# Bardli/RMem_ocu

Hardware: AMD Instinct MI355X
Metric: frames/sec (whole node) 480p VOS, N=8 memory bank (higher is better)
Workload: dtype bf16; 1 GPU; davis17_480p_r50_N8; clip_frames=80, job_clips=64, clip_feeder=static, objects=3, memory_bank=1+7, gap=5, clips_in_flight_per_gpu=24, clips_per_group=8, step_unit=batch, parallelism=clip-parallel x1, weights=synthetic (no checkpoint offline), hipgraphs=True, frames_from=HBM, encoder_lookahead=2

## Files before the change

include/rmem.h:

```cpp
#ifndef RMEM_H_
#define RMEM_H_

#include <stddef.h>

#ifdef __cplusplus
extern "C" {
#endif

#define RMEM_ABI_VERSION 15

int rmem_abi_version(void);
const char* rmem_last_error_string(void);

typedef struct rmem_conv_desc {
  int H, W, Cin;
  int Ho, Wo, Cout;
  int KH, KW, stride, pad;
  int ldo;
  int ldr;
  int ld2;
  int relu;
  int out_f32;
  int res_f32;
  int ldx;
  int batch;
  int act_begin;
  int res_up_h, res_up_w, res_up_align;
} rmem_conv_desc;

size_t rmem_conv_workspace_bytes(const rmem_conv_desc* desc);
int rmem_conv2d_nhwc(const rmem_conv_desc* desc, const void* x, const void* w, const float* bias,
                     const void* residual, void* y, void* y2, void* workspace, void* stream);

enum rmem_gemm_family {
  RMEM_GEMM_GENERAL64 = 0,
  RMEM_GEMM_SCALAR64 = 1,
  RMEM_GEMM_ROWRUN64 = 2,
  RMEM_GEMM_ONE128 = 3,
  RMEM_GEMM_PC128 = 4,
  RMEM_GEMM_ROWRUN128 = 5,
  RMEM_GEMM_DUAL64 = 6,
  RMEM_GEMM_DUAL128 = 7,
  RMEM_GEMM_GROUPED = 8
};
enum rmem_gemm_entry { RMEM_GEMM_ENTRY_CONV2D = 0, RMEM_GEMM_ENTRY_DUAL = 1, RMEM_GEMM_ENTRY_GROUPED = 2 };
typedef struct rmem_gemm_plan {
  int family;
  int tile;
  int ring;
  int is1x1;
  int fast;
  int splits;
  int steps_per_split;
  int xcd_ny;
  int grid_x, grid_y, grid_z, threads;
} rmem_gemm_plan;
int rmem_conv_plan(const rmem_conv_desc* desc, int has_workspace, int entry, int extra, rmem_gemm_plan* plan);

int rmem_linear_grouped(const rmem_conv_desc* desc, int n, const void* const* x, const void* const* w,
                        const float* const* bias, const void* const* residual, void* const* y, void* stream);

int rmem_conv1x1_dual_nhwc(const rmem_conv_desc* desc, const void* x, const void* x2, int H2, int W2, int Cin2, int stride2,
                           const void* w_cat, const float* bias, void* y, void* stream);

typedef struct rmem_bneck_chain_desc { int batch, Ho, Wo, K1, Cout, N2, H2, W2, Cin2, stride2; } rmem_bneck_chain_desc;
int rmem_bneck_chain(const rmem_bneck_chain_desc* desc, const void* b, const void* x2, const void* w3, const float* bias3, const void* res,
                     void* y, const void* w1, const float* bias1, void* a2, void* stream);

typedef struct rmem_attn_chunk {
  int slot;
  int key_begin;
  int key_count;
  int pe_slot;
  int t;
  int reserved[3];
} rmem_attn_chunk;

size_t rmem_attn_workspace_bytes(int Lq, int heads, int nchunks);

int rmem_mem_read_attn(const void* q, int ldq,
                       const void* k_bank, const void* v_bank,
                       long long slot_stride, int ldkv,
                       const rmem_attn_chunk* chunks, int nchunks,
                       int lk_single,
                       const float* pe_cur,
                       const float* pe_mem,
                       int Lq, int heads,
                       void* out, int ldo,
                       float* attn_mass, int T,
                       void* workspace, void* stream);

int rmem_mem_read_attn_clips(const void* q, int ldq, const void* k_bank, const void* v_bank, long long slot_stride, int ldkv,
                             const rmem_attn_chunk* chunks, int nchunks, int lk_single, const float* pe_cur, const float* pe_mem,
                             int Lq, int heads, void* out, int ldo, float* attn_mass, int T, int nclips,
                             long long q_clip_stride, long long kv_clip_stride, long long out_clip_stride,
                             void* workspace, void* stream);

int rmem_lstt_attn_pair_clips(const void* q, int ldq, const void* k_bank, const void* v_bank, long long slot_stride, int ldkv,
                              const rmem_attn_chunk* chunks, int nchunks, int lk_total, const float* pe_cur, const float* pe_mem,
                              int Lq, int heads, void* out_long, int ldo, float* attn_mass, int T, int nclips,
                              long long q_clip_stride, long long out_clip_stride,
                              const void* k_short, const void* v_short, int lk_short, long long kv_short_clip_stride,
                              void* out_short, long long out_short_clip_stride, void* workspace, void* stream);

int rmem_profile_start(int max_launches);
int rmem_profile_stop(double* total_ms, double* total_flops, int* launches);

int rmem_layernorm256(const void* a, int a_is_f32, int lda, const void* b, int b_is_f32, int ldb,
                      const float* gamma, const float* beta, float eps, int M,
                      void* y_bf16, int ldy, const float* pos, void* ypos_bf16, int ldyp,
                      float* y_f32, int ldyf, void* stream);

int rmem_layernorm256_pair(const void* a0, const void* b0, void* y0, const void* a1, const void* b1, void* y1,
                           const float* gamma, const float* beta, float eps, int M, void* stream);

int rmem_lstt_chain_waves(void);
typedef struct rmem_chain_a_desc {
  int L, clips; float eps; int reserved;
  const void* att; float* x;
  const void* w_proj; const float* b_proj; const float* ln2_g; const float* ln2_b; void* curr_v;
  const void* w_q; const float* b_q; void* curr_q;
  const void* short_k; const void* short_v; const float* ln4_g; const float* ln4_b; void* k4; void* v4;
} rmem_chain_a_desc;
int rmem_lstt_chain_a(const rmem_chain_a_desc* d, void* stream);

typedef struct rmem_chain_b_desc {
  int L, clips; float eps; int gn_splits;
  const void* att_long; const void* att_short; float* x;
  const void* w_long; const float* b_long; const void* w_short; const float* b_short; void* tgt3;
  const float* ln3_g; const float* ln3_b; const void* w1; const float* b1; void* h1; float* gn_partial;
} rmem_chain_b_desc;
int rmem_lstt_chain_b(const rmem_chain_b_desc* d, void* stream);

typedef struct rmem_chain_c_desc {
  int L, clips; float eps; int ld_dec;
  float* x;
  const void* h3; const void* w2; const float* b2; const float* dec_g; const float* dec_b; void* dec_out;
  const float* ln1_g; const float* ln1_b; const void* w_qkv; const float* b_qkv; const float* pos_qk; void* qkv;
} rmem_chain_c_desc;
int rmem_lstt_chain_c(const rmem_chain_c_desc* d, void* stream);

int rmem_layernorm(const void* a, int a_is_f32, int lda, const float* gamma, const float* beta, float eps, int M, int C,
                   void* y_bf16, int ldy, float* y_f32, int ldyf, void* stream);

int rmem_patch_merge_ln(const float* x, int H, int W, int C, const float* gamma, const float* beta, float eps,
                        void* y_bf16, void* stream);
int rmem_patch_merge_ln_images(const float* x, int images, int H, int W, int C, const float* gamma, const float* beta, float eps,
                               void* y_bf16, void* stream);

int rmem_window_attn(const void* qkv, const float* qkv_bias, const float* bias_mask_table, void* out, int H, int W,
                     int C, int heads, int shift, void* stream);
int rmem_window_attn_images(const void* qkv, const float* qkv_bias, const float* bias_mask_table, void* out, int images, int H, int W,
                            int C, int heads, int shift, void* stream);

int rmem_add16(const void* a, const void* b, void* y, long long n, void* stream);
int rmem_add16_grouped(int n, const void* const* a, const void* const* b, void* const* y, long long count, void* stream);

size_t rmem_groupnorm_workspace_bytes(int groups);
int rmem_groupnorm_nhwc(const void* x, int M, int C, int groups, const float* gamma, const float* beta,
                        float eps, int act, void* y, float* workspace, void* stream);

int rmem_groupnorm_f32_nhwc(const float* x, int M, int C, int groups, const float* gamma, const float* beta,
                            float eps, int act, void* y, float* workspace, void* stream);

int rmem_groupnorm_nhwc_images(const void* x, int images, int M, int C, int groups, const float* gamma, const float* beta,
                               float eps, int act, void* y, float* workspace, void* stream);
int rmem_groupnorm_head_nhwc_images(const void* x, int images, int M, int C, int groups, const float* gamma, const float* beta,
                                    float eps, int act, const void* w, const float* bias, int N, float* y, int ldy,
                                    float* workspace, void* stream);
int rmem_gn_act_dwconv5x5_nhwc_images(const void* x, int images, int H, int W, int C, int groups, const float* gamma,
                                      const float* beta, float eps, int act, const float* w_t, void* y, float* workspace, void* stream);
int rmem_bilinear_nhwc_images(const void* x, void* y, int images, int Hi, int Wi, int Ho, int Wo, int C, int align_corners, void* stream);
int rmem_gn_act_dwconv5x5_prestats_nhwc_images(const void* x, int images, int H, int W, int C, int groups, const float* gamma,
                                               const float* beta, float eps, int act, const float* w_t, void* y, const float* stats,
                                               void* stream);

int rmem_dwconv5x5_nhwc(const void* x, const float* w_t, void* y, int H, int W, int C, void* stream);

size_t rmem_gated_attn_workspace_bytes(int Lq, int DV, int frames, int keys_per_frame, int nchunks);
int rmem_gated_attn(const void* q, int ldq,
                    const void* k_bank, long long k_slot_stride, int ldk,
                    const void* v_bank, long long v_slot_stride, int ldv,
                    const rmem_attn_chunk* chunks, int nchunks, int frames, int keys_per_frame,
                    const float* pe_cur, const float* pe_mem,
                    int Lq, int DV, const void* u_a, int ldua, const void* u_b, int ldub, int usplit,
                    void* out, int ldo, float* attn_mass,
                    const float* dw_w_t, int H, int W,
                    void* workspace, void* stream);
int rmem_local_gated_attn(const void* q, int ldq, const void* k, int ldk, const void* v, int ldv, const float* rel, int ldrel,
                          int H, int W, int DV, const void* u_a, int ldua, const void* u_b, int ldub, int usplit,
                          void* out, int ldo, const float* dw_w_t, void* workspace, void* stream);

int rmem_gated_attn_clips(const void* q, int ldq, const void* k_bank, long long k_slot_stride, int ldk, const void* v_bank,
                          long long v_slot_stride, int ldv, const rmem_attn_chunk* chunks, int nchunks, int frames, int keys_per_frame,
                          const float* pe_cur, const float* pe_mem, int Lq, int DV, const void* u_a, int ldua, const void* u_b, int ldub,
                          int usplit, void* out, int ldo, float* attn_mass, const float* dw_w_t, int H, int W, int nclips,
                          void* workspace, void* stream);
int rmem_local_gated_attn_clips(const void* q, int ldq, const void* k, int ldk, const void* v, int ldv, const float* rel, int ldrel,
                                int H, int W, int DV, const void* u_a, int ldua, const void* u_b, int ldub, int usplit, void* out, int ldo,
                                const float* dw_w_t, int nclips, void* workspace, void* stream);
int rmem_gated_profile_start(void);
int rmem_gated_profile_stop(double* total_ms, double* total_flops, int* launches);
int rmem_scatter_blocks(const void* src, void* dst, const int* slots_dev, int nclips, long long block_bytes, long long slot_bytes,
                        void* stream);
int rmem_copy2d_async(void* dst, long long dst_pitch, const void* src, long long src_pitch, long long row_bytes, int rows, void* stream);

int rmem_gn_act_dwconv5x5_nhwc(const void* x, int H, int W, int C, int groups, const float* gamma, const float* beta, float eps,
                               int act, const float* w_t, void* y, float* workspace, void* stream);

int rmem_image_to_nhwc8(const float* img_chw, void* out, int H, int W, void* stream);
int rmem_image_to_nhwc8_images(const float* img_chw, void* out, int images, int H, int W, void* stream);
int rmem_image_ptrs_to_nhwc8(const float* const* img_ptrs, void* out, int images, int H, int W, void* stream);
int rmem_stem_padded_size(int H, int W, int* Hp, int* Wp);
int rmem_image_ptrs_to_nhwc4p(const float* const* img_ptrs, void* out_padded, int images, int H, int W, void* stream);
int rmem_stem7x7s2(const void* x_padded, int images, int H, int W, const void* w, const float* bias, void* y, void* stream);
// ... 194 lines not shown
int rmem_mask_iou_counts(const unsigned char* pred, const unsigned char* gt, long long n, int num_ids, int void_label,
                         unsigned long long* counts, void* stream);

size_t rmem_clip_score_workspace_bytes(int frames, int H, int W, int num_ids);
int rmem_boundary_radius(int H, int W, double bound_th);
int rmem_clip_score_counts(const unsigned char* pred, const unsigned char* gt, int frames, int H, int W, int num_ids,
                           int void_label, int radius, void* workspace, unsigned long long* counts, void* stream);

size_t rmem_pair_boundary_workspace_bytes(int frames, int H, int W, int num_a, int num_b);
int rmem_pair_boundary_counts(const unsigned char* a, const unsigned char* b, int frames, int H, int W, int num_a, int num_b,
                              int void_label, int radius, void* workspace, size_t workspace_bytes, int* bnd_a, int* bnd_b,
                              int* match, void* stream);

size_t rmem_png_zlib_bound(int H, int W);
size_t rmem_png_workspace_bytes(int frames, int H, int W);
int rmem_png_encode_labels(const unsigned char* labels, int frames, int H, int W, const unsigned char* lut ,
                           void* workspace, unsigned char* out, long long* offsets, void* stream);

typedef struct RmemPngDesc {
  long long offset;
  long long bytes;
  int bit_depth;
  int colour_type;
} RmemPngDesc;
#define RMEM_PNG_ST_INPUT 1
#define RMEM_PNG_ST_SIZE 2
#define RMEM_PNG_ST_RANGE 4
#define RMEM_PNG_ST_CODE 8
#define RMEM_PNG_ST_HEADER 16
#define RMEM_PNG_ST_ADLER 32
#define RMEM_PNG_ST_FILTER 64
#define RMEM_PNG_ST_DESC 128
size_t rmem_png_decode_workspace_bytes(int frames, int H, int W);
int rmem_png_decode_labels(const unsigned char* bits, const RmemPngDesc* descs , int frames, int H, int W,
                           const unsigned char* lut , void* workspace,
                           unsigned char* out , int* status , void* stream);

#define RMEM_RLE_ST_CAPACITY 1
size_t rmem_rle_workspace_bytes(int frames, int H, int W, int num_ids);
int rmem_rle_encode_labels(const unsigned char* labels, int frames, int H, int W, int num_ids, void* workspace, unsigned char* out,
                           long long capacity, long long* offsets ,
                           int* status , void* stream);

typedef struct RmemRleDesc {
  int frame;
  int value;
  long long offset;
  int length;
} RmemRleDesc;
#define RMEM_RLE_ST_CHAR 1
#define RMEM_RLE_ST_TRUNCATED 2
#define RMEM_RLE_ST_LONG 4
#define RMEM_RLE_ST_NEGATIVE 8
#define RMEM_RLE_ST_SUM 16
#define RMEM_RLE_ST_DESC 32
size_t rmem_rle_decode_workspace_bytes(long long nstrings, long long total_bytes, int frames, int W);
int rmem_rle_decode_labels(const unsigned char* bits, long long total_bytes, const RmemRleDesc* descs , int nstrings, int frames,
                           int H, int W, void* workspace, unsigned char* labels ,
                           int* status , void* stream);

#define RMEM_JPEG_ENC_HEADER_MAX 629
#define RMEM_JPEG_ENC_TABLE_BYTES 4096
int rmem_jpeg_encode_header(int H, int W, int quality, int restart_rows, unsigned char* header, int capacity, int* header_bytes,
                            void* tables );
size_t rmem_jpeg_encode_bound(int H, int W);
size_t rmem_jpeg_encode_workspace_bytes(int frames, int H, int W);
int rmem_jpeg_encode_rgb8(const unsigned char* rgb, const unsigned char* labels ,
                          const unsigned char* palette , int alpha256, int frames,
                          int H, int W, const void* tables ,
                          void* workspace, unsigned char* out, long long* offsets, void* stream);
int rmem_overlay_rgb8(const unsigned char* rgb, const unsigned char* labels, const unsigned char* palette ,
                      int alpha256, int frames, int H, int W, unsigned char* out_rgb, void* stream);

int rmem_graph_begin(void* stream);
int rmem_graph_end(void* stream, void** graph_exec_out);
int rmem_graph_launch(void* graph_exec, void* stream);
int rmem_graph_destroy(void* graph_exec);


int rmem_conv2d_nhwc_f16(const rmem_conv_desc* desc, const void* x, const void* w, const float* bias, const void* residual, void* y, void* y2, void* workspace, void* stream);
int rmem_mem_read_attn_f16(const void* q, int ldq, const void* k_bank, const void* v_bank, long long slot_stride, int ldkv, const rmem_attn_chunk* chunks, int nchunks, int lk_single, const float* pe_cur, const float* pe_mem, int Lq, int heads, void* out, int ldo, float* attn_mass, int T, void* workspace, void* stream);
int rmem_mem_read_attn_clips_f16(const void* q, int ldq, const void* k_bank, const void* v_bank, long long slot_stride, int ldkv, const rmem_attn_chunk* chunks, int nchunks, int lk_single, const float* pe_cur, const float* pe_mem, int Lq, int heads, void* out, int ldo, float* attn_mass, int T, int nclips, long long q_clip_stride, long long kv_clip_stride, long long out_clip_stride, void* workspace, void* stream);
int rmem_lstt_attn_pair_clips_f16(const void* q, int ldq, const void* k_bank, const void* v_bank, long long slot_stride, int ldkv, const rmem_attn_chunk* chunks, int nchunks, int lk_total, const float* pe_cur, const float* pe_mem, int Lq, int heads, void* out_long, int ldo, float* attn_mass, int T, int nclips, long long q_clip_stride, long long out_clip_stride, const void* k_short, const void* v_short, int lk_short, long long kv_short_clip_stride, void* out_short, long long out_short_clip_stride, void* workspace, void* stream);
int rmem_layernorm256_f16(const void* a, int a_is_f32, int lda, const void* b, int b_is_f32, int ldb, const float* gamma, const float* beta, float eps, int M, void* y_bf16, int ldy, const float* pos, void* ypos_bf16, int ldyp, float* y_f32, int ldyf, void* stream);
int rmem_layernorm_f16(const void* a, int a_is_f32, int lda, const float* gamma, const float* beta, float eps, int M, int C, void* y_bf16, int ldy, float* y_f32, int ldyf, void* stream);
int rmem_patch_merge_ln_f16(const float* x, int H, int W, int C, const float* gamma, const float* beta, float eps, void* y_bf16, void* stream);
int rmem_window_attn_f16(const void* qkv, const float* qkv_bias, const float* bias_mask_table, void* out, int H, int W, int C, int heads, int shift, void* stream);
int rmem_window_attn_images_f16(const void* qkv, const float* qkv_bias, const float* bias_mask_table, void* out, int images, int H, int W, int C, int heads, int shift, void* stream);
int rmem_patch_merge_ln_images_f16(const float* x, int images, int H, int W, int C, const float* gamma, const float* beta, float eps, void* y_bf16, void* stream);
int rmem_add16_f16(const void* a, const void* b, void* y, long long n, void* stream);
int rmem_add16_grouped_f16(int n, const void* const* a, const void* const* b, void* const* y, long long count, void* stream);
int rmem_lstt_chain_a_f16(const rmem_chain_a_desc* d, void* stream);
int rmem_lstt_chain_b_f16(const rmem_chain_b_desc* d, void* stream);
int rmem_lstt_chain_c_f16(const rmem_chain_c_desc* d, void* stream);
int rmem_layernorm256_pair_f16(const void* a0, const void* b0, void* y0, const void* a1, const void* b1, void* y1, const float* gamma, const float* beta, float eps, int M, void* stream);
int rmem_bneck_chain_f16(const rmem_bneck_chain_desc* desc, const void* b, const void* x2, const void* w3, const float* bias3, const void* res, void* y, const void* w1, const float* bias1, void* a2, void* stream);
int rmem_conv1x1_dual_nhwc_f16(const rmem_conv_desc* desc, const void* x, const void* x2, int H2, int W2, int Cin2, int stride2, const void* w_cat, const float* bias, void* y, void* stream);
int rmem_linear_grouped_f16(const rmem_conv_desc* desc, int n, const void* const* x, const void* const* w, const float* const* bias, const void* const* residual, void* const* y, void* stream);
int rmem_groupnorm_nhwc_f16(const void* x, int M, int C, int groups, const float* gamma, const float* beta, float eps, int act, void* y, float* workspace, void* stream);
int rmem_groupnorm_f32_nhwc_f16(const float* x, int M, int C, int groups, const float* gamma, const float* beta, float eps, int act, void* y, float* workspace, void* stream);
int rmem_groupnorm_nhwc_images_f16(const void* x, int images, int M, int C, int groups, const float* gamma, const float* beta, float eps, int act, void* y, float* workspace, void* stream);
int rmem_groupnorm_head_nhwc_images_f16(const void* x, int images, int M, int C, int groups, const float* gamma, const float* beta, float eps, int act, const void* w, const float* bias, int N, float* y, int ldy, float* workspace, void* stream);
int rmem_gn_act_dwconv5x5_nhwc_images_f16(const void* x, int images, int H, int W, int C, int groups, const float* gamma, const float* beta, float eps, int act, const float* w_t, void* y, float* workspace, void* stream);
int rmem_gn_act_dwconv5x5_prestats_nhwc_images_f16(const void* x, int images, int H, int W, int C, int groups, const float* gamma, const float* beta, float eps, int act, const float* w_t, void* y, const float* stats, void* stream);
int rmem_gn_act_dwconv5x5_nhwc_f16(const void* x, int H, int W, int C, int groups, const float* gamma, const float* beta, float eps, int act, const float* w_t, void* y, float* workspace, void* stream);
int rmem_dwconv5x5_nhwc_f16(const void* x, const float* w_t, void* y, int H, int W, int C, void* stream);
int rmem_image_ptrs_to_nhwc4p_f16(const float* const* img_ptrs, void* out_padded, int images, int H, int W, void* stream);
int rmem_conv3x3_direct_f16(const void* x, int images, int H, int W, int C, const void* w, const float* bias, int relu, void* y, void* stream);
int rmem_conv3x3_c64_direct_f16(const void* x, int images, int H, int W, const void* w, const float* bias, void* y, void* stream);
int rmem_stem7x7s2_pool_f16(const void* x_padded, int images, int H, int W, const void* w, const float* bias, void* y_pooled, void* stream);
int rmem_stem7x7s2_f16(const void* x_padded, int images, int H, int W, const void* w, const float* bias, void* y, void* stream);
int rmem_image_ptrs_to_nhwc8_f16(const float* const* img_ptrs, void* out, int images, int H, int W, void* stream);
int rmem_image_to_nhwc8_f16(const float* img_chw, void* out, int H, int W, void* stream);
int rmem_image_to_nhwc8_images_f16(const float* img_chw, void* out, int images, int H, int W, void* stream);
int rmem_ingest_rgb8_f16(const unsigned char* rgb_hwc, int Hs, int Ws, int Hd, int Wd, float* out_chw, void* out_nhwc8, void* stream);
int rmem_maxpool3x3s2_nhwc_f16(const void* x, void* y, int H, int W, int C, void* stream);
int rmem_maxpool3x3s2_nhwc_images_f16(const void* x, void* y, int images, int H, int W, int C, void* stream);
int rmem_bilinear_nhwc_f16(const void* x, void* y, int Hi, int Wi, int Ho, int Wo, int C, int align_corners, void* stream);
int rmem_bilinear_nhwc_images_f16(const void* x, void* y, int images, int Hi, int Wi, int Ho, int Wo, int C, int align_corners, void* stream);
int rmem_label_id_embed_f16(const void* label, int label_is_f32, int images, int Hs, int Ws, int H, int W, int KH, int KW, int stride, int pad, int num_classes, const void* w, const float* bias, void* label_scratch_u8, void* out, void* stream);
int rmem_label_to_onehot16_f16(const void* label, int label_is_f32, int Hs, int Ws, int Hd, int Wd, int num_classes, void* out, void* stream);
int rmem_label_to_onehot16_images_f16(const void* label, int label_is_f32, int images, int Hs, int Ws, int Hd, int Wd, int num_classes, void* out, void* stream);
int rmem_gated_attn_f16(const void* q, int ldq, const void* k_bank, long long k_slot_stride, int ldk, const void* v_bank, long long v_slot_stride, int ldv, const rmem_attn_chunk* chunks, int nchunks, int frames, int keys_per_frame, const float* pe_cur, const float* pe_mem, int Lq, int DV, const void* u_a, int ldua, const void* u_b, int ldub, int usplit, void* out, int ldo, float* attn_mass, const float* dw_w_t, int H, int W, void* workspace, void* stream);
int rmem_local_gated_attn_f16(const void* q, int ldq, const void* k, int ldk, const void* v, int ldv, const float* rel, int ldrel, int H, int W, int DV, const void* u_a, int ldua, const void* u_b, int ldub, int usplit, void* out, int ldo, const float* dw_w_t, void* workspace, void* stream);
int rmem_gated_attn_clips_f16(const void* q, int ldq, const void* k_bank, long long k_slot_stride, int ldk, const void* v_bank, long long v_slot_stride, int ldv, const rmem_attn_chunk* chunks, int nchunks, int frames, int keys_per_frame, const float* pe_cur, const float* pe_mem, int Lq, int DV, const void* u_a, int ldua, const void* u_b, int ldub, int usplit, void* out, int ldo, float* attn_mass, const float* dw_w_t, int H, int W, int nclips, void* workspace, void* stream);
int rmem_local_gated_attn_clips_f16(const void* q, int ldq, const void* k, int ldk, const void* v, int ldv, const float* rel, int ldrel, int H, int W, int DV, const void* u_a, int ldua, const void* u_b, int ldub, int usplit, void* out, int ldo, const float* dw_w_t, int nclips, void* workspace, void* stream);

#ifdef __cplusplus
}
#endif
#endif
```

rmem_ocu_amd/_lib.py:

```python
from __future__ import annotations

import ctypes as C
import os
import subprocess

_HERE = os.path.dirname(os.path.abspath(__file__))
LIB_PATH = os.environ.get('RMEM_LIB_PATH') or os.path.join(_HERE, 'librmem_hip.so')
ABI_VERSION = 15


class RmemError(RuntimeError):
    pass


class ConvDesc(C.Structure):
    _fields_ = [(n, C.c_int) for n in ('H', 'W', 'Cin', 'Ho', 'Wo', 'Cout', 'KH', 'KW', 'stride', 'pad',
                                       'ldo', 'ldr', 'ld2', 'relu', 'out_f32', 'res_f32', 'ldx', 'batch', 'act_begin',
                                       'res_up_h', 'res_up_w', 'res_up_align')]


class GemmPlan(C.Structure):
    _fields_ = [(n, C.c_int) for n in ('family', 'tile', 'ring', 'is1x1', 'fast', 'splits', 'steps_per_split', 'xcd_ny',
                                       'grid_x', 'grid_y', 'grid_z', 'threads')]


GEMM_FAMILIES = ('general64', 'scalar64', 'rowrun64', 'one128', 'pc128', 'rowrun128', 'dual64', 'dual128', 'grouped')
GEMM_ENTRIES = ('conv2d', 'conv1x1_dual', 'linear_grouped')


class BneckChainDesc(C.Structure):
    _fields_ = [(n, C.c_int) for n in ('batch', 'Ho', 'Wo', 'K1', 'Cout', 'N2', 'H2', 'W2', 'Cin2', 'stride2')]


class AttnChunk(C.Structure):
    _fields_ = [('slot', C.c_int), ('key_begin', C.c_int), ('key_count', C.c_int), ('pe_slot', C.c_int),
                ('t', C.c_int), ('reserved', C.c_int * 3)]


_vp, _i, _ll, _f = C.c_void_p, C.c_int, C.c_longlong, C.c_float


class JpegInfo(C.Structure):
    _fields_ = [('width', C.c_int), ('height', C.c_int), ('components', C.c_int), ('h_samp', C.c_int * 3), ('v_samp', C.c_int * 3),
                ('quant_id', C.c_int * 3), ('restart_interval', C.c_int), ('quant_mask', C.c_int), ('quant', (C.c_ushort * 64) * 4),
                ('scan_begin', C.c_longlong), ('scan_end', C.c_longlong), ('packed_bound', C.c_longlong)]


class JpegHuff(C.Structure):
    _fields_ = [('lut', C.c_ushort * 512), ('maxcode', C.c_int * 18), ('valoff', C.c_int * 18), ('vals', C.c_ubyte * 256)]


class JpegDesc(C.Structure):
    _fields_ = ([('offset', C.c_longlong), ('bytes', C.c_longlong)]
                + [(n, C.c_int) for n in ('width', 'height', 'ncomp', 'hmax', 'vmax', 'mcus_x', 'mcus_y', 'bpm', 'restart_mcus', 'nunits',
                                          'nsub', 'total_blocks', 'data_off', 'data_bits')]
                + [(n, C.c_int * 3) for n in ('comp_h', 'comp_v', 'comp_bw', 'comp_bh', 'comp_block0', 'comp_dw', 'comp_dh')]
                + [('mcu_comp', C.c_int * 10), ('mcu_sub', C.c_int * 10), ('quant', (C.c_ushort * 64) * 3), ('dc', JpegHuff * 3),
                   ('ac', JpegHuff * 3)])


class JpegPlan(C.Structure):
    _fields_ = ([(n, C.c_int) for n in ('batch', 'max_width', 'max_height', 'max_sub', 'max_blocks', 'max_units', 'sync_rounds', 'flags')]
                + [(n, C.c_longlong) for n in ('slot_bytes', 'off_state', 'off_unit', 'off_dc', 'off_coef', 'off_plane', 'off_misc')])


JPEG_FORCE_FALLBACK = 1
JPEG_ENC_HEADER_MAX, JPEG_ENC_TABLE_BYTES = 629, 4096


class PngDesc(C.Structure):
    _fields_ = [('offset', C.c_longlong), ('bytes', C.c_longlong), ('bit_depth', C.c_int), ('colour_type', C.c_int)]


class RleDesc(C.Structure):
    _fields_ = [('frame', C.c_int), ('value', C.c_int), ('offset', C.c_longlong), ('length', C.c_int)]


class PolyShape(C.Structure):
    _fields_ = [(n, C.c_int) for n in ('frame', 'value', 'x0', 'y0', 'x1', 'y1')] + [('plane', C.c_longlong)]


class PolyPass(C.Structure):
    _fields_ = ([(n, C.c_int) for n in ('frame0', 'frames', 'shape0', 'shapes', 'edge0', 'edges')]
                + [(n, C.c_longlong) for n in ('cross0', 'crossings', 'plane0', 'plane_words')])


class LabelRoute(C.Structure):
    _fields_ = [('dst', C.c_void_p), ('overlay', C.c_void_p), ('feed', C.c_void_p), ('twin', C.c_int), ('mode', C.c_int)]


ROUTE_LIVE, ROUTE_IDLE, ROUTE_SKIP = 0, 1, 2


def _desc(name, ints, ptrs):
    return type(name, (C.Structure,), {'_fields_': [(ints[0], _i), (ints[1], _i), ('eps', _f), (ints[2], _i)] + [(n, _vp) for n in ptrs]})


ChainA = _desc('ChainA', ('L', 'clips', 'reserved'),
               ('att', 'x', 'w_proj', 'b_proj', 'ln2_g', 'ln2_b', 'curr_v', 'w_q', 'b_q', 'curr_q', 'short_k', 'short_v', 'ln4_g', 'ln4_b',
                'k4', 'v4'))
ChainB = _desc('ChainB', ('L', 'clips', 'gn_splits'),
               ('att_long', 'att_short', 'x', 'w_long', 'b_long', 'w_short', 'b_short', 'tgt3', 'ln3_g', 'ln3_b', 'w1', 'b1', 'h1',
                'gn_partial'))
ChainC = _desc('ChainC', ('L', 'clips', 'ld_dec'),
               ('x', 'h3', 'w2', 'b2', 'dec_g', 'dec_b', 'dec_out', 'ln1_g', 'ln1_b', 'w_qkv', 'b_qkv', 'pos_qk', 'qkv'))
SIGNATURES = {
    'rmem_abi_version': (_i, []),
    'rmem_last_error_string': (C.c_char_p, []),
    'rmem_conv_workspace_bytes': (C.c_size_t, [C.POINTER(ConvDesc)]),
    'rmem_conv2d_nhwc': (_i, [C.POINTER(ConvDesc), _vp, _vp, _vp, _vp, _vp, _vp, _vp, _vp]),
    'rmem_conv_plan': (_i, [C.POINTER(ConvDesc), _i, _i, _i, C.POINTER(GemmPlan)]),
    'rmem_attn_workspace_bytes': (C.c_size_t, [_i, _i, _i]),
    'rmem_mem_read_attn': (_i, [_vp, _i, _vp, _vp, _ll, _i, _vp, _i, _i, _vp, _vp, _i, _i, _vp, _i, _vp, _i, _vp, _vp]),
    'rmem_profile_start': (_i, [_i]),
    'rmem_profile_stop': (_i, [C.POINTER(C.c_double), C.POINTER(C.c_double), C.POINTER(_i)]),
    'rmem_layernorm256': (_i, [_vp, _i, _i, _vp, _i, _i, _vp, _vp, _f, _i, _vp, _i, _vp, _vp, _i, _vp, _i, _vp]),
    'rmem_layernorm': (_i, [_vp, _i, _i, _vp, _vp, _f, _i, _i, _vp, _i, _vp, _i, _vp]),
    'rmem_patch_merge_ln': (_i, [_vp, _i, _i, _i, _vp, _vp, _f, _vp, _vp]),
    'rmem_window_attn': (_i, [_vp, _vp, _vp, _vp, _i, _i, _i, _i, _i, _vp]),
    'rmem_window_attn_images': (_i, [_vp, _vp, _vp, _vp, _i, _i, _i, _i, _i, _i, _vp]),
    'rmem_patch_merge_ln_images': (_i, [_vp, _i, _i, _i, _i, _vp, _vp, _f, _vp, _vp]),
    'rmem_add16': (_i, [_vp, _vp, _vp, _ll, _vp]),
    'rmem_add16_grouped': (_i, [_i, C.POINTER(_vp), C.POINTER(_vp), C.POINTER(_vp), _ll, _vp]),
    'rmem_layernorm256_pair': (_i, [_vp, _vp, _vp, _vp, _vp, _vp, _vp, _vp, _f, _i, _vp]),
    'rmem_lstt_chain_waves': (_i, []),
    'rmem_lstt_chain_a': (_i, [C.POINTER(ChainA), _vp]),
    'rmem_lstt_chain_b': (_i, [C.POINTER(ChainB), _vp]),
    'rmem_lstt_chain_c': (_i, [C.POINTER(ChainC), _vp]),
    'rmem_conv1x1_dual_nhwc': (_i, [C.POINTER(ConvDesc), _vp, _vp, _i, _i, _i, _i, _vp, _vp, _vp, _vp]),
    'rmem_bneck_chain': (_i, [C.POINTER(BneckChainDesc), _vp, _vp, _vp, _vp, _vp, _vp, _vp, _vp, _vp, _vp]),
    'rmem_linear_grouped': (_i, [C.POINTER(ConvDesc), _i, C.POINTER(_vp), C.POINTER(_vp), C.POINTER(_vp), C.POINTER(_vp), C.POINTER(_vp), _vp]),
    'rmem_groupnorm_workspace_bytes': (C.c_size_t, [_i]),
    'rmem_groupnorm_nhwc': (_i, [_vp, _i, _i, _i, _vp, _vp, _f, _i, _vp, _vp, _vp]),
    'rmem_groupnorm_f32_nhwc': (_i, [_vp, _i, _i, _i, _vp, _vp, _f, _i, _vp, _vp, _vp]),
    'rmem_groupnorm_nhwc_images': (_i, [_vp, _i, _i, _i, _i, _vp, _vp, _f, _i, _vp, _vp, _vp]),
    'rmem_groupnorm_head_nhwc_images': (_i, [_vp, _i, _i, _i, _i, _vp, _vp, _f, _i, _vp, _vp, _i, _vp, _i, _vp, _vp]),
    'rmem_gn_act_dwconv5x5_nhwc_images': (_i, [_vp, _i, _i, _i, _i, _i, _vp, _vp, _f, _i, _vp, _vp, _vp, _vp]),
    'rmem_gn_act_dwconv5x5_prestats_nhwc_images': (_i, [_vp, _i, _i, _i, _i, _i, _vp, _vp, _f, _i, _vp, _vp, _vp, _vp]),
    'rmem_bilinear_nhwc_images': (_i, [_vp, _vp, _i, _i, _i, _i, _i, _i, _i, _vp]),
    'rmem_mem_read_attn_clips': (_i, [_vp, _i, _vp, _vp, _ll, _i, _vp, _i, _i, _vp, _vp, _i, _i, _vp, _i, _vp, _i, _i, _ll, _ll, _ll, _vp, _vp]),
    'rmem_lstt_attn_pair_clips': (_i, [_vp, _i, _vp, _vp, _ll, _i, _vp, _i, _i, _vp, _vp, _i, _i, _vp, _i, _vp, _i, _i, _ll, _ll,
                                       _vp, _vp, _i, _ll, _vp, _ll, _vp, _vp]),
    'rmem_gn_act_dwconv5x5_nhwc': (_i, [_vp, _i, _i, _i, _i, _vp, _vp, _f, _i, _vp, _vp, _vp, _vp]),
    'rmem_dwconv5x5_nhwc': (_i, [_vp, _vp, _vp, _i, _i, _i, _vp]),
    'rmem_image_to_nhwc8': (_i, [_vp, _vp, _i, _i, _vp]),
    'rmem_image_to_nhwc8_images': (_i, [_vp, _vp, _i, _i, _i, _vp]),
    'rmem_image_ptrs_to_nhwc8': (_i, [_vp, _vp, _i, _i, _i, _vp]),
    'rmem_stem_padded_size': (_i, [_i, _i, C.POINTER(_i), C.POINTER(_i)]),
    'rmem_image_ptrs_to_nhwc4p': (_i, [_vp, _vp, _i, _i, _i, _vp]),
    'rmem_stem7x7s2': (_i, [_vp, _i, _i, _i, _vp, _vp, _vp, _vp]),
    'rmem_stem7x7s2_pool': (_i, [_vp, _i, _i, _i, _vp, _vp, _vp, _vp]),
    'rmem_conv3x3_c64_direct': (_i, [_vp, _i, _i, _i, _vp, _vp, _vp, _vp]),
    'rmem_conv3x3_direct': (_i, [_vp, _i, _i, _i, _i, _vp, _vp, _i, _vp, _vp]),
    'rmem_ingest_rgb8': (_i, [_vp, _i, _i, _i, _i, _vp, _vp, _vp]),
    'rmem_maxpool3x3s2_nhwc': (_i, [_vp, _vp, _i, _i, _i, _vp]),
    'rmem_maxpool3x3s2_nhwc_images': (_i, [_vp, _vp, _i, _i, _i, _i, _vp]),
    'rmem_bilinear_nhwc': (_i, [_vp, _vp, _i, _i, _i, _i, _i, _i, _vp]),
    'rmem_logits_post': (_i, [_vp, _i, _i, _i, _i, _i, _i, _i, _i, _vp, _vp, _vp, _vp]),
    'rmem_logits_post_images': (_i, [_vp, _i, _i, _i, _i, _i, _i, _i, _i, _i, _vp, _vp, _vp, _vp]),
    'rmem_label_to_onehot16': (_i, [_vp, _i, _i, _i, _i, _i, _i, _vp, _vp]),
    'rmem_label_id_embed_scratch_size': (_i, [_i, _i, _i, C.POINTER(_i), C.POINTER(_i)]),
    'rmem_label_id_embed': (_i, [_vp, _i, _i, _i, _i, _i, _i, _i, _i, _i, _i, _i, _vp, _vp, _vp, _vp, _vp]),
    'rmem_label_to_onehot16_images': (_i, [_vp, _i, _i, _i, _i, _i, _i, _i, _vp, _vp]),
    'rmem_evict_scores': (_i, [_vp, _i, _i, _i, _i, _i, _i, _i, _vp, _i, _vp, _vp]),
    'rmem_resize_nearest_flip_f32': (_i, [_vp, _i, _i, _i, _vp, _i, _i, _i, _vp]),
    'rmem_tta_merge': (_i, [C.POINTER(_vp), C.POINTER(_i), _i, _i, _i, _i, _vp, _vp, _vp, _vp]),
    'rmem_logits_post_flip_pairs': (_i, [_vp, _i, _i, _i, _i, _i, _i, _i, _i, _vp, _vp]),
    'rmem_logits_post_ms_merge': (_i, [C.POINTER(_vp), C.POINTER(_i), C.POINTER(_i), C.POINTER(_i), _i, _i, _i, _i, _i, _i, _i, _vp, _vp, _vp]),
    'rmem_route_labels': (_i, [_vp, _i, _i, _i, _vp, _vp]),
    'rmem_label_census': (_i, [_vp, _i, _i, _i, _vp, _vp]),
    'rmem_label_remap': (_i, [_vp, _vp, _i, _ll, _vp, _i, _vp]),
    'rmem_label_pair_census': (_i, [_vp, _vp, _i, _i, _i, _i, _i, _vp, _vp]),
    'rmem_label_pair_census_lds_bins': (_i, []),
    'rmem_label_components_tile': (_i, [C.POINTER(_i), C.POINTER(_i)]),
    'rmem_label_components_workspace_bytes': (_ll, [_i, _i, _i]),
    'rmem_label_components': (_i, [_vp, _i, _i, _i, _i, _vp, _vp, _vp]),
    'rmem_label_component_stats': (_i, [_vp, _vp, _i, _i, _i, _i, _vp, _vp, _vp]),
    'rmem_label_clean': (_i, [_vp, _vp, _vp, _vp, _vp, _i, _i, _i, _i, _i, _i, _vp]),
    'rmem_label_edt_workspace_bytes': (_ll, [_i, _i, _i]),
    'rmem_label_edt': (_i, [_vp, _i, _i, _i, _i, _i, _vp, _vp, _ll, _vp]),
    'rmem_label_edt_peaks_workspace_bytes': (_ll, [_i]),
    'rmem_label_edt_peaks': (_i, [_vp, _vp, _i, _i, _i, _vp, _vp, _ll, _vp]),
    'rmem_label_nearest_workspace_bytes': (_ll, [_i, _i, _i]),
    'rmem_label_nearest': (_i, [_vp, _i, _i, _i, C.POINTER(C.c_uint), C.POINTER(C.c_uint), _i, _vp, _vp, _vp, _vp, _ll, _vp]),
    'rmem_label_surface': (_i, [_vp, _i, _i, _i, _vp, _vp]),
    'rmem_label_edt_at': (_i, [_vp, _vp, _i, _i, _i, _i, _i, _vp, _vp, _ll, _vp]),
    'rmem_surface_census_workspace_bytes': (_ll, [_i, _i]),
    'rmem_surface_census': (_i, [_vp, _vp, _vp, _vp, _i, _i, _i, _i, C.POINTER(_i), _i, _i, _vp, _vp, _ll, _vp]),
    'rmem_label_thin_tile': (_i, [C.POINTER(_i), C.POINTER(_i), C.POINTER(_i)]),
    'rmem_label_thin_table': (_i, [_i, _vp]),
    'rmem_label_thin_workspace_bytes': (_ll, [_i, _i, _i]),
    'rmem_label_thin': (_i, [_vp, _i, _i, _i, _i, _i, _vp, _vp, _vp, _ll, _vp]),
    'rmem_label_pixels_workspace_bytes': (_ll, [_i, _i, _i]),
    'rmem_label_pixels_count': (_i, [_vp, _i, _i, _i, _vp, _vp, _ll, _vp]),
    'rmem_label_pixels_write': (_i, [_vp, _vp, _i, _i, _i, _ll, _vp, _vp, _vp, _ll, _vp]),
    'rmem_label_polygons_unit': (_i, []),
    'rmem_label_polygons_workspace_bytes': (C.c_size_t, [_i, _i, _i, _i]),
    'rmem_label_polygons': (_i, [_vp, _i, _i, _i, _i, _i, _i, _vp, C.c_size_t, _vp, _vp, _vp, _vp]),
    'rmem_polygon_simplify_short_max': (_i, []),
    'rmem_polygon_simplify_workspace_bytes': (C.c_size_t, [_ll, _ll]),
    'rmem_polygon_simplify': (_i, [_vp, _vp, _vp, _ll, _ll, _i, _vp, C.c_size_t, _vp, _vp, _vp, _vp]),
    'rmem_polygon_fill_workspace_bytes': (C.c_size_t, [_ll]),
    'rmem_polygon_fill_labels': (_i, [_vp, _vp, _vp, _i, _vp, _i, _vp, _i, _i, _i, C.POINTER(PolyPass), _vp, C.c_size_t, _vp, _vp, _vp]),
    'rmem_mask_iou_counts': (_i, [_vp, _vp, _ll, _i, _i, _vp, _vp]),
    'rmem_clip_score_workspace_bytes': (C.c_size_t, [_i, _i, _i, _i]),
    'rmem_boundary_radius': (_i, [_i, _i, C.c_double]),
    'rmem_clip_score_counts': (_i, [_vp, _vp, _i, _i, _i, _i, _i, _i, _vp, _vp, _vp]),
    'rmem_pair_boundary_workspace_bytes': (C.c_size_t, [_i, _i, _i, _i, _i]),
    'rmem_pair_boundary_counts': (_i, [_vp, _vp, _i, _i, _i, _i, _i, _i, _i, _vp, C.c_size_t, _vp, _vp, _vp, _vp]),
    'rmem_png_zlib_bound': (C.c_size_t, [_i, _i]),
    'rmem_png_workspace_bytes': (C.c_size_t, [_i, _i, _i]),
    'rmem_png_encode_labels': (_i, [_vp, _i, _i, _i, _vp, _vp, _vp, _vp, _vp]),
    'rmem_png_decode_workspace_bytes': (C.c_size_t, [_i, _i, _i]),
    'rmem_png_decode_labels': (_i, [_vp, _vp, _i, _i, _i, _vp, _vp, _vp, _vp, _vp]),
    'rmem_rle_workspace_bytes': (C.c_size_t, [_i, _i, _i, _i]),
    'rmem_rle_encode_labels': (_i, [_vp, _i, _i, _i, _i, _vp, _vp, _ll, _vp, _vp, _vp]),
    'rmem_rle_decode_workspace_bytes': (C.c_size_t, [_ll, _ll, _i, _i]),
    'rmem_rle_decode_labels': (_i, [_vp, _ll, _vp, _i, _i, _i, _i, _vp, _vp, _vp, _vp]),
    'rmem_split_label': (_i, [_vp, _i, _i, _vp, _ll, _vp]),
    'rmem_soft_logit_aggregate': (_i, [C.POINTER(_vp), _i, _i, _i, _i, _i, _vp, _vp]),
    'rmem_copy_async': (_i, [_vp, _vp, C.c_size_t, _vp]),
    'rmem_scatter_blocks': (_i, [_vp, _vp, _vp, _i, _ll, _ll, _vp]),
    'rmem_copy2d_async': (_i, [_vp, _ll, _vp, _ll, _ll, _i, _vp]),
    'rmem_gated_attn_workspace_bytes': (C.c_size_t, [_i, _i, _i, _i, _i]),
    'rmem_gated_attn': (_i, [_vp, _i, _vp, _ll, _i, _vp, _ll, _i, _vp, _i, _i, _i, _vp, _vp, _i, _i, _vp, _i, _vp, _i, _i, _vp, _i,
                             _vp, _vp, _i, _i, _vp, _vp]),
    'rmem_local_gated_attn': (_i, [_vp, _i, _vp, _i, _vp, _i, _vp, _i, _i, _i, _i, _vp, _i, _vp, _i, _i, _vp, _i, _vp, _vp, _vp]),
    'rmem_gated_attn_clips': (_i, [_vp, _i, _vp, _ll, _i, _vp, _ll, _i, _vp, _i, _i, _i, _vp, _vp, _i, _i, _vp, _i, _vp, _i, _i, _vp, _i,
                                   _vp, _vp, _i, _i, _i, _vp, _vp]),
    'rmem_local_gated_attn_clips': (_i, [_vp, _i, _vp, _i, _vp, _i, _vp, _i, _i, _i, _i, _vp, _i, _vp, _i, _i, _vp, _i, _vp, _i, _vp, _vp]),
    'rmem_gated_profile_start': (_i, []),
    'rmem_gated_profile_stop': (_i, [C.POINTER(C.c_double), C.POINTER(C.c_double), C.POINTER(_i)]),
    'rmem_jpeg_parse': (_i, [_vp, C.c_size_t, C.POINTER(JpegInfo)]),
    'rmem_jpeg_pack': (_i, [_vp, C.c_size_t, _vp, C.c_size_t, C.POINTER(C.c_size_t), C.POINTER(JpegDesc)]),
    'rmem_jpeg_workspace_bytes': (C.c_size_t, [C.POINTER(JpegDesc), _i, _i, C.POINTER(JpegPlan)]),
    'rmem_jpeg_entropy_decode': (_i, [_vp, _vp, _i, _i, C.POINTER(JpegPlan), _vp, _vp, _vp, _vp]),
    'rmem_jpeg_coef_to_rgb': (_i, [_vp, _i, _i, C.POINTER(JpegPlan), _vp, _vp, _vp]),
    'rmem_jpeg_decode_batch': (_i, [_vp, _vp, _i, _i, C.POINTER(JpegPlan), _vp, _vp, _vp, _vp, _vp]),
    'rmem_jpeg_encode_header': (_i, [_i, _i, _i, _i, _vp, _i, C.POINTER(_i), _vp]),
    'rmem_jpeg_encode_bound': (C.c_size_t, [_i, _i]),
    'rmem_jpeg_encode_workspace_bytes': (C.c_size_t, [_i, _i, _i]),
    'rmem_jpeg_encode_rgb8': (_i, [_vp, _vp, _vp, _i, _i, _i, _i, _vp, _vp, _vp, _vp, _vp]),
    'rmem_overlay_rgb8': (_i, [_vp, _vp, _vp, _i, _i, _i, _i, _vp, _vp]),
    'rmem_graph_begin': (_i, [_vp]),
    'rmem_graph_end': (_i, [_vp, C.POINTER(_vp)]),
    'rmem_graph_launch': (_i, [_vp, _vp]),
    'rmem_graph_destroy': (_i, [_vp]),
}

F16_TWINS = ('rmem_conv2d_nhwc', 'rmem_mem_read_attn', 'rmem_mem_read_attn_clips', 'rmem_lstt_attn_pair_clips', 'rmem_layernorm256', 'rmem_layernorm', 'rmem_patch_merge_ln',
             'rmem_window_attn', 'rmem_window_attn_images', 'rmem_patch_merge_ln_images', 'rmem_add16', 'rmem_add16_grouped', 'rmem_layernorm256_pair', 'rmem_lstt_chain_a', 'rmem_lstt_chain_b', 'rmem_lstt_chain_c', 'rmem_conv1x1_dual_nhwc', 'rmem_bneck_chain', 'rmem_label_id_embed', 'rmem_image_ptrs_to_nhwc4p', 'rmem_stem7x7s2', 'rmem_stem7x7s2_pool', 'rmem_conv3x3_c64_direct', 'rmem_conv3x3_direct', 'rmem_linear_grouped',
             'rmem_groupnorm_nhwc', 'rmem_groupnorm_f32_nhwc', 'rmem_groupnorm_nhwc_images', 'rmem_groupnorm_head_nhwc_images',
             'rmem_gn_act_dwconv5x5_nhwc_images', 'rmem_gn_act_dwconv5x5_prestats_nhwc_images', 'rmem_gn_act_dwconv5x5_nhwc', 'rmem_dwconv5x5_nhwc', 'rmem_image_to_nhwc8',
             'rmem_image_to_nhwc8_images', 'rmem_image_ptrs_to_nhwc8', 'rmem_ingest_rgb8', 'rmem_maxpool3x3s2_nhwc', 'rmem_maxpool3x3s2_nhwc_images', 'rmem_bilinear_nhwc',
             'rmem_bilinear_nhwc_images', 'rmem_label_to_onehot16', 'rmem_label_to_onehot16_images', 'rmem_gated_attn', 'rmem_local_gated_attn', 'rmem_gated_attn_clips', 'rmem_local_gated_attn_clips')
SIGNATURES.update({n + '_f16': SIGNATURES[n] for n in F16_TWINS})

_lib = None


def build(force: bool = False) -> str:
    src = os.path.join(_HERE, 'csrc')
    if force:
        subprocess.run(['make', '-C', src, 'clean'], check=True, capture_output=True)
    r = subprocess.run(['make', '-C', src, '-j8'], capture_output=True, text=True)
    if r.returncode != 0:
        raise RmemError('building librmem_hip.so failed:\n' + r.stdout + r.stderr)
    return LIB_PATH


def lib():
    global _lib
    if _lib is None:
        if not os.path.exists(LIB_PATH):
            raise RmemError(f'{LIB_PATH} is missing: run `python -c "import __graft_entry__ as g; g.build()"` '
                            '(there is no CPU fallback for the HIP path)')
        import torch
        L = C.CDLL(LIB_PATH)
        for name, (res, args) in SIGNATURES.items():
            fn = getattr(L, name)
            fn.restype = res
            fn.argtypes = args
        if L.rmem_abi_version() != ABI_VERSION:
            raise RmemError('librmem_hip.so ABI version mismatch; rebuild it')
        _lib = L
    return _lib


def check(rc: int, what: str = ''):
    if rc != 0:
        raise RmemError(f'{what} failed ({rc}): {lib().rmem_last_error_string().decode()}')
```

rmem_ocu_amd/csrc/attention.hip:

```cpp
#include "common.h"
#include "../../include/rmem.h"
#include <type_traits>

namespace {

constexpr int D = 32;
constexpr int KT = 64;
constexpr int NB = 4;
constexpr float NEG_BIG = -1.0e30f;
constexpr float RESCALE_THR = 8.0f;
[[maybe_unused]] constexpr float L_LIMIT = 1.8446744e19f;

typedef __attribute__((ext_vector_type(4))) short s16x4;
typedef __attribute__((address_space(3))) s16x4 lds_s16x4;

struct AttnParams {
  const e16* q; int ldq;
  const e16* k; const e16* v; long slot_stride; int ldkv;
  const rmem_attn_chunk* chunks; int nchunks; int lk; int per_chunk;
  const float* pe_cur; const float* pe_mem;
  int Lq, heads, C, nq;
  int ngroups, rpg;
  float* opart; float* mlg;
  float* ml;
// ... 482 lines not shown
      num += f32x4{(float)o4[0], (float)o4[1], (float)o4[2], (float)o4[3]} * w;
    }
    if (live) {
      const f32x4 o = num * (1.f / den);
      *reinterpret_cast<e16x4*>(p.out + (long)q * p.ldo + head * D + 4 * G) = e16x4{(e16)o[0], (e16)o[1], (e16)o[2], (e16)o[3]};
    }
  }
}

__global__ __launch_bounds__(256) void k_attn_mass(CombineParams pin) {
  CombineParams p = pin;
  p.ml += blockIdx.z * p.ml_cs; p.chunks += blockIdx.z * p.nchunks; p.mass += blockIdx.z * p.mass_cs;
  __shared__ float macc[4][64][33];
  __shared__ int ct[32];
  const int tid = threadIdx.x, ql = tid & 63, hq = tid >> 6;
  const int q = blockIdx.x * 64 + ql;
  const int qc = q < p.Lq ? q : p.Lq - 1;
  if (tid < p.nchunks) ct[tid] = p.chunks[tid].t;
  for (int t = 0; t < 33; ++t) macc[hq][ql][t] = 0.f;
  __syncthreads();
  for (int h = hq; h < p.heads; h += 4) {
    float m = NEG_BIG, den = 0.f;
    for (int c = 0; c < p.nchunks; ++c) {
      const f32x2 mlv = *reinterpret_cast<const f32x2*>(p.ml + (((long)c * p.heads + h) * p.Lq + qc) * 2);
      if (mlv[1] > 0.f) m = fmaxf(m, mlv[0]);
    }
    for (int c = 0; c < p.nchunks; ++c) {
      const f32x2 mlv = *reinterpret_cast<const f32x2*>(p.ml + (((long)c * p.heads + h) * p.Lq + qc) * 2);
      if (mlv[1] > 0.f) den += __builtin_amdgcn_exp2f(mlv[0] - m) * mlv[1];
    }
    const float inv = 1.f / (den * (float)p.heads);
    for (int c = 0; c < p.nchunks; ++c) {
      const f32x2 mlv = *reinterpret_cast<const f32x2*>(p.ml + (((long)c * p.heads + h) * p.Lq + qc) * 2);
      if (mlv[1] > 0.f) macc[hq][ql][ct[c]] += __builtin_amdgcn_exp2f(mlv[0] - m) * mlv[1] * inv;
    }
  }
  __syncthreads();
  for (int i = tid; i < 64 * p.T; i += 256) {
    const int qq = i / p.T, t = i - qq * p.T;
    const int qo = blockIdx.x * 64 + qq;
    if (qo < p.Lq) p.mass[(long)qo * p.T + t] = macc[0][qq][t] + macc[1][qq][t] + macc[2][qq][t] + macc[3][qq][t];
  }
}

}

#ifndef RMEM_F16
extern "C" size_t rmem_attn_workspace_bytes(int Lq, int heads, int nchunks) {
  return (size_t)nchunks * heads * Lq * (D + 4) * sizeof(float);
}
#endif

#if defined(RMEM_ATTN_TIMELINE) && !defined(RMEM_F16)
extern "C" int rmem_attn_timeline_read(double* out, int nwg) {
  static unsigned host[8192 * 8];
  if (nwg > 8192) nwg = 8192;
  if (hipDeviceSynchronize() != hipSuccess) return 1;
  if (hipMemcpyFromSymbol(host, HIP_SYMBOL(g_attn_timeline), sizeof(unsigned) * 8 * nwg) != hipSuccess) return 2;
  double s[5] = {0, 0, 0, 0, 0};
  for (int i = 0; i < nwg; ++i) for (int j = 0; j < 5; ++j) s[j] += host[i * 8 + j];
  for (int j = 0; j < 4; ++j) out[j] = s[4] > 0 ? s[j] / s[4] : 0;
  out[4] = s[4] / nwg;
  return 0;
}
#endif

static unsigned attn_lds_pad() {
  const char* e = getenv("RMEM_ATTN_LDS_PAD");
  const int x = e ? atoi(e) : 0;
  return x > 0 ? (unsigned)x : 0u;
}

static int attn_target_wgs() {
  const char* e = getenv("RMEM_ATTN_WGS");
  const int x = e ? atoi(e) : 0;
  return x > 0 ? x : 1792;
}

static int attn_launch(const void* q, int ldq, const void* k_bank, const void* v_bank, long long slot_stride,
                       int ldkv, const rmem_attn_chunk* chunks, int nchunks, int lk_single,
                       const float* pe_cur, const float* pe_mem, int Lq, int heads, void* out, int ldo,
                       float* attn_mass, int T, int nclips, long long q_clip_stride, long long kv_clip_stride,
                       long long out_clip_stride, void* workspace, void* stream,
                       const void* k2, const void* v2, int lk2, long long kv2_clip_stride, void* out2, long long out2_clip_stride) {
  RMEM_REQUIRE(nclips >= 1 && nclips <= 64, "rmem_mem_read_attn: 1..64 clips");
  RMEM_REQUIRE(q_clip_stride % 8 == 0 && kv_clip_stride % 8 == 0 && out_clip_stride % 8 == 0, "rmem_mem_read_attn: clip strides must be multiples of 8 elements");
  const long long prof_keys = chunks ? (long long)lk_single : 0;
  RMEM_REQUIRE(q && k_bank && v_bank && out && workspace, "rmem_mem_read_attn: null argument");
  RMEM_REQUIRE(heads >= 1 && heads <= 8, "rmem_mem_read_attn: heads must be in 1..8 (head dim is fixed at 32)");
  RMEM_REQUIRE(Lq > 0 && nchunks >= 1 && nchunks <= 32, "rmem_mem_read_attn: need Lq > 0 and 1 <= nchunks <= 32");
  RMEM_REQUIRE(ldq % 8 == 0 && ldkv % 8 == 0 && slot_stride % 8 == 0, "rmem_mem_read_attn: strides must be multiples of 8 elements");
  RMEM_REQUIRE(ldq >= heads * D && ldkv >= heads * D && ldo >= heads * D, "rmem_mem_read_attn: leading dimension < heads*32");
  RMEM_REQUIRE(chunks || lk_single > 0, "rmem_mem_read_attn: lk_single must be > 0 when no chunk table is given");
  RMEM_REQUIRE(lk_single >= 0, "rmem_mem_read_attn: lk_single must be >= 0");
  RMEM_REQUIRE(!attn_mass || (chunks && T >= 1 && T <= 32), "rmem_mem_read_attn: the mass output needs a chunk table and 1 <= T <= 32");
  RMEM_REQUIRE(!pe_mem || chunks, "rmem_mem_read_attn: pe_mem needs a chunk table");
  hipStream_t s = (hipStream_t)stream;
  AttnParams p;
  p.q = (const e16*)q; p.ldq = ldq; p.k = (const e16*)k_bank; p.v = (const e16*)v_bank;
  p.slot_stride = slot_stride; p.ldkv = ldkv; p.chunks = chunks; p.nchunks = nchunks;
  p.lk = lk_single; p.per_chunk = chunks ? 0 : (lk_single + nchunks - 1) / nchunks;
  RMEM_REQUIRE(chunks || (long)p.per_chunk * (nchunks - 1) < lk_single, "rmem_mem_read_attn: too many chunks for lk_single");
  p.pe_cur = pe_cur; p.pe_mem = pe_mem; p.Lq = Lq; p.heads = heads; p.C = heads * D;
  p.nclips = nclips; p.q_cs = q_clip_stride; p.kv_cs = kv_clip_stride; p.out_cs = out_clip_stride;
  p.qscale = 1.4426950408889634f / sqrtf((float)D);
  p.nq = (Lq + 127) / 128;
  {
    const int base = p.nq * heads * nclips;
    int groups = (attn_target_wgs() + base - 1) / base;
    groups = groups < 1 ? 1 : (groups > nchunks ? nchunks : groups);
    p.rpg = (nchunks + groups - 1) / groups;
    p.ngroups = (nchunks + p.rpg - 1) / p.rpg;
  }
  p.opart_cs = (long)p.ngroups * heads * Lq * D; p.mlg_cs = (long)p.ngroups * heads * Lq * 2; p.ml_cs = (long)nchunks * heads * Lq * 2;
  p.opart = (float*)workspace; p.mlg = p.opart + (size_t)nclips * p.opart_cs;
  p.ml = attn_mass ? p.mlg + (size_t)nclips * p.mlg_cs : nullptr;
  p.out = (e16*)out; p.ldo = ldo;
  p.n2 = 0; p.k2 = p.v2 = nullptr; p.lk2 = 0; p.kv2_cs = 0; p.out2 = nullptr; p.out2_cs = 0;
  if (k2) {
    RMEM_REQUIRE(chunks && v2 && out2 && lk2 > 0, "rmem_lstt_attn_pair: the second attention rides on a memory read (chunk table) and needs k2, v2, out2, lk2 > 0");
    RMEM_REQUIRE(kv2_clip_stride % 8 == 0 && out2_clip_stride % 8 == 0 && ((uintptr_t)k2 % 16) == 0 && ((uintptr_t)v2 % 16) == 0,
                 "rmem_lstt_attn_pair: second attention operands must be 16-byte aligned, strides multiples of 8 elements");
    RMEM_REQUIRE(p.nq * heads * nclips >= 8, "rmem_lstt_attn_pair: launch too small for the per-XCD split");
    p.n2 = nclips; p.k2 = (const e16*)k2; p.v2 = (const e16*)v2; p.lk2 = lk2; p.kv2_cs = kv2_clip_stride;
    p.out2 = (e16*)out2; p.out2_cs = out2_clip_stride;
  }
  dim3 grid(p.nq * heads * (p.ngroups * nclips + p.n2));
  if (chunks) {
    const int slot_i = prof_keys > 0 ? rmem_prof_begin(RMEM_PROF_MEM_READ, s, 4.0 * (double)Lq * (double)prof_keys * (double)(heads * D) * nclips)
                                     : -1;
    if (slot_i >= 0) hipLaunchKernelGGL((k_attn_partial<true, true>), grid, dim3(256), attn_lds_pad(), s, p);
    else hipLaunchKernelGGL((k_attn_partial<true, false>), grid, dim3(256), attn_lds_pad(), s, p);
    if (slot_i >= 0) rmem_prof_end(RMEM_PROF_MEM_READ, slot_i, s);
  } else {
    hipLaunchKernelGGL((k_attn_partial<false, false>), grid, dim3(256), 0, s, p);
  }
  CombineParams cp;
  cp.opart = p.opart; cp.mlg = p.mlg; cp.ngroups = p.ngroups; cp.ml = p.ml; cp.chunks = chunks; cp.nchunks = nchunks;
  cp.Lq = Lq; cp.heads = heads; cp.out = (e16*)out; cp.ldo = ldo; cp.mass = attn_mass; cp.T = T;
  cp.out_cs = out_clip_stride; cp.opart_cs = p.opart_cs; cp.mlg_cs = p.mlg_cs; cp.ml_cs = p.ml_cs; cp.mass_cs = (long)Lq * T;
  if (p.ngroups > 1) hipLaunchKernelGGL(k_attn_combine, dim3((Lq + 63) / 64, 16, nclips), dim3(256), 0, s, cp);
  if (attn_mass) hipLaunchKernelGGL(k_attn_mass, dim3((Lq + 63) / 64, 1, nclips), dim3(256), 0, s, cp);
  return rmem_check_launch("rmem_mem_read_attn");
}

extern "C" int RMEM_API(rmem_mem_read_attn_clips)(const void* q, int ldq, const void* k_bank, const void* v_bank, long long slot_stride,
                                        int ldkv, const rmem_attn_chunk* chunks, int nchunks, int lk_single,
                                        const float* pe_cur, const float* pe_mem, int Lq, int heads, void* out, int ldo,
                                        float* attn_mass, int T, int nclips, long long q_clip_stride, long long kv_clip_stride,
                                        long long out_clip_stride, void* workspace, void* stream) {
  return attn_launch(q, ldq, k_bank, v_bank, slot_stride, ldkv, chunks, nchunks, lk_single, pe_cur, pe_mem, Lq, heads, out, ldo, attn_mass, T,
                     nclips, q_clip_stride, kv_clip_stride, out_clip_stride, workspace, stream, nullptr, nullptr, 0, 0, nullptr, 0);
}

extern "C" int RMEM_API(rmem_lstt_attn_pair_clips)(const void* q, int ldq, const void* k_bank, const void* v_bank, long long slot_stride,
                                         int ldkv, const rmem_attn_chunk* chunks, int nchunks, int lk_total,
                                         const float* pe_cur, const float* pe_mem, int Lq, int heads, void* out_long, int ldo,
                                         float* attn_mass, int T, int nclips, long long q_clip_stride, long long out_clip_stride,
                                         const void* k_short, const void* v_short, int lk_short, long long kv_short_clip_stride,
                                         void* out_short, long long out_short_clip_stride, void* workspace, void* stream) {
  RMEM_REQUIRE(chunks && k_short && v_short && out_short, "rmem_lstt_attn_pair: null argument");
  return attn_launch(q, ldq, k_bank, v_bank, slot_stride, ldkv, chunks, nchunks, lk_total, pe_cur, pe_mem, Lq, heads, out_long, ldo, attn_mass, T,
                     nclips, q_clip_stride, 0, out_clip_stride, workspace, stream, k_short, v_short, lk_short, kv_short_clip_stride, out_short,
                     out_short_clip_stride);
}

extern "C" int RMEM_API(rmem_mem_read_attn)(const void* q, int ldq, const void* k_bank, const void* v_bank, long long slot_stride,
                                  int ldkv, const rmem_attn_chunk* chunks, int nchunks, int lk_single,
                                  const float* pe_cur, const float* pe_mem, int Lq, int heads, void* out, int ldo,
                                  float* attn_mass, int T, void* workspace, void* stream) {
  return RMEM_API(rmem_mem_read_attn_clips)(q, ldq, k_bank, v_bank, slot_stride, ldkv, chunks, nchunks, lk_single, pe_cur, pe_mem, Lq, heads, out,
                                  ldo, attn_mass, T, 1, 0, 0, 0, workspace, stream);
}
```

rmem_ocu_amd/csrc/rowchain.hip:

```cpp
#include "common.h"
#include "lds_dma.h"
#include "../../include/rmem.h"

namespace {

#ifndef RMEM_CHAIN_WAVES
#define RMEM_CHAIN_WAVES 8
#endif
constexpr int NW = RMEM_CHAIN_WAVES;
constexpr int NT = 64 * NW;
constexpr int JT = 16 / NW;
constexpr int WC = 256 / NW;
constexpr int RW = 32 / NW;
constexpr int BM = 32;
constexpr int XS = 260;
constexpr int PANEL = BM * 64;
constexpr int PF = 16 / JT;

__device__ __forceinline__ f32x4 ld4(const float* p) { return *reinterpret_cast<const f32x4*>(p); }
__device__ __forceinline__ e16x4 cvt4(f32x4 v) { return e16x4{(e16)v[0], (e16)v[1], (e16)v[2], (e16)v[3]}; }
__device__ __forceinline__ f32x4 up4(e16x4 v) { return f32x4{(float)v[0], (float)v[1], (float)v[2], (float)v[3]}; }

typedef __attribute__((ext_vector_type(2))) unsigned u32x2;
typedef __attribute__((ext_vector_type(4))) unsigned u32x4;
#if defined(__HIP_DEVICE_COMPILE__)
__device__ __forceinline__ void st8(rsrc_t r, int off, e16x4 v) { __builtin_amdgcn_raw_buffer_store_b64(__builtin_bit_cast(u32x2, v), r, off, 0, 0); }
__device__ __forceinline__ void st16(rsrc_t r, int off, f32x4 v) { __builtin_amdgcn_raw_buffer_store_b128(__builtin_bit_cast(u32x4, v), r, off, 0, 0); }
#else
__device__ inline void st8(rsrc_t, int, e16x4) {}
__device__ inline void st16(rsrc_t, int, f32x4) {}
#endif

template <int NP>
__device__ __forceinline__ void stage_tile(e16* A16, int p0, const e16* src, long ld, int nrows) {
  constexpr int PT = NT / 256;
  static_assert(NP % PT == 0, "panels must divide among the thread halves");
  const int t = threadIdx.x & 255, half = threadIdx.x >> 8;
  const int row = t >> 3, ch = t & 7;
  const e16* sr = src + min(row, nrows - 1) * ld + ch * 8;
  e16x8 v[NP / PT];
#pragma unroll
  for (int p = 0; p < NP / PT; ++p) v[p] = *reinterpret_cast<const e16x8*>(sr + (p * PT + half) * 64);
#pragma unroll
  for (int p = 0; p < NP / PT; ++p) *reinterpret_cast<e16x8*>(&A16[(p0 + p * PT + half) * PANEL + swz(row, ch)]) = v[p];
}

__device__ __forceinline__ void put_a(e16* A16, int p0, int row, int lane, e16x4 v) {
  *reinterpret_cast<e16x4*>(&A16[(p0 + (lane >> 4)) * PANEL + swz(row, (lane & 15) >> 1) + (lane & 1) * 4]) = v;
}

struct BRing { e16x8 b[PF][JT]; };

__device__ __forceinline__ const e16* wstream(const e16* w, int nb, int wave, int KC) { return w + (long)(nb * NW + wave) * KC * (JT * 512); }

__device__ __forceinline__ void b_preload(BRing& r, const e16* wp, int lane) {
#pragma unroll
  for (int u = 0; u < PF; ++u)
#pragma unroll
    for (int j = 0; j < JT; ++j) r.b[u][j] = *reinterpret_cast<const e16x8*>(wp + ((u * JT + j) * 64 + lane) * 8);
  __builtin_amdgcn_sched_barrier(0);
}

template <int NP>
__device__ __forceinline__ void gemm32(const e16* A16, int p0, const e16* wp, BRing& r, f32x4 (&acc)[2][JT], int lane) {
  constexpr int KC = NP * 2;
  const int fr = lane & 15, fc = lane >> 4;
#pragma unroll
  for (int kc = 0; kc < KC; ++kc) {
    const e16* Ap = A16 + (p0 + (kc >> 1)) * PANEL;
    const e16x8 a0 = *reinterpret_cast<const e16x8*>(&Ap[swz(fr, 4 * (kc & 1) + fc)]);
    const e16x8 a1 = *reinterpret_cast<const e16x8*>(&Ap[swz(16 + fr, 4 * (kc & 1) + fc)]);
#pragma unroll
    for (int j = 0; j < JT; ++j) {
      acc[0][j] = RMEM_MFMA_16x16x32(a0, r.b[kc % PF][j], acc[0][j], 0, 0, 0);
      acc[1][j] = RMEM_MFMA_16x16x32(a1, r.b[kc % PF][j], acc[1][j], 0, 0, 0);
    }
    if (kc + PF < KC) {
#pragma unroll
      for (int j = 0; j < JT; ++j) r.b[kc % PF][j] = *reinterpret_cast<const e16x8*>(wp + (((kc + PF) * JT + j) * 64 + lane) * 8);
      __builtin_amdgcn_sched_barrier(0);
    }
  }
}

__device__ __forceinline__ void zero_acc(f32x4 (&acc)[2][JT]) {
#pragma unroll
  for (int i = 0; i < 2; ++i)
#pragma unroll
    for (int j = 0; j < JT; ++j) acc[i][j] = f32x4{0.f, 0.f, 0.f, 0.f};
}

__device__ __forceinline__ void dump_acc(float* X, const f32x4 (&acc)[2][JT], int wave, int lane) {
  const int fr = lane & 15, fc = lane >> 4;
#pragma unroll
  for (int i = 0; i < 2; ++i)
#pragma unroll
    for (int j = 0; j < JT; ++j)
#pragma unroll
      for (int q = 0; q < 4; ++q) X[(i * 16 + fc * 4 + q) * XS + wave * WC + j * 16 + fr] = acc[i][j][q];
}

struct Blk { int nrows; long g0; };
__device__ __forceinline__ Blk my_rows(int L) {
  Blk b;
  const int r0 = blockIdx.x * BM;
  b.nrows = min(BM, L - r0);
  b.g0 = (long)blockIdx.y * L + r0;
  return b;
}

template <typename T>
struct Rows8 { T r[RW]; };

__device__ __forceinline__ Rows8<f32x4> load_rows_f32(const float* base, int ld, const Blk& blk, int wave, int c0) {
  Rows8<f32x4> o;
#pragma unroll
  for (int rr = 0; rr < RW; ++rr) {
    const int row = min(wave * RW + rr, blk.nrows - 1);
    o.r[rr] = ld4(base + (blk.g0 + row) * ld + c0);
  }
  return o;
}
__device__ __forceinline__ Rows8<e16x4> load_rows_e16(const e16* base, int ld, const Blk& blk, int wave, int c0) {
  Rows8<e16x4> o;
#pragma unroll
  for (int rr = 0; rr < RW; ++rr) {
    const int row = min(wave * RW + rr, blk.nrows - 1);
    o.r[rr] = *reinterpret_cast<const e16x4*>(base + (blk.g0 + row) * ld + c0);
  }
  return o;
}
__device__ __forceinline__ int row_off(const Blk& blk, int wave, int rr, int ld, int c0, int esz) {
  const int row = wave * RW + rr;
  return row < blk.nrows ? (int)(((blk.g0 + row) * ld + c0) * esz) : OOB;
}

__global__ __launch_bounds__(NT) void k_chain_a(rmem_chain_a_desc d) {
  __shared__ __attribute__((aligned(16))) char smem[4 * PANEL * 2 + BM * XS * 4];
  e16* A16 = reinterpret_cast<e16*>(smem);
  float* X = reinterpret_cast<float*>(smem + 4 * PANEL * 2);
  const int lane = threadIdx.x & 63, wave = __builtin_amdgcn_readfirstlane(threadIdx.x >> 6);
  const Blk blk = my_rows(d.L);
  const int c0 = lane * 4;
  const long rows = (long)d.clips * d.L;
  const rsrc_t rx = make_rsrc(d.x, rows * 1024), rcv = make_rsrc(d.curr_v, rows * 512), rcq = make_rsrc(d.curr_q, rows * 512),
               rk4 = make_rsrc(d.k4, rows * 512), rv4 = make_rsrc(d.v4, rows * 512);
  const f32x4 bp = ld4(d.b_proj + c0), g2 = ld4(d.ln2_g + c0), b2 = ld4(d.ln2_b + c0);
  const f32x4 bq = ld4(d.b_q + c0), g4 = ld4(d.ln4_g + c0), b4 = ld4(d.ln4_b + c0);
  const Rows8<f32x4> xo = load_rows_f32(d.x, 256, blk, wave, c0);
  const Rows8<e16x4> sk = load_rows_e16((const e16*)d.short_k, 256, blk, wave, c0);
  const Rows8<e16x4> sv = load_rows_e16((const e16*)d.short_v, 256, blk, wave, c0);
  BRing ring;
  f32x4 acc[2][JT];
  const e16* wp = wstream((const e16*)d.w_proj, 0, wave, 8);
  stage_tile<4>(A16, 0, (const e16*)d.att + blk.g0 * 256, 256, blk.nrows);
  b_preload(ring, wp, lane);
  __syncthreads();
  zero_acc(acc);
  gemm32<4>(A16, 0, wp, ring, acc, lane);
  dump_acc(X, acc, wave, lane);
  const e16* wq = wstream((const e16*)d.w_q, 0, wave, 8);
  b_preload(ring, wq, lane);
  __syncthreads();
  e16x4 cv[RW];
  {
    f32x4 v[RW];
#pragma unroll
    for (int rr = 0; rr < RW; ++rr) {
      v[rr] = ld4(&X[(wave * RW + rr) * XS + c0]);
      v[rr] += bp;
      v[rr] += xo.r[rr];
      st16(rx, row_off(blk, wave, rr, 256, c0, 4), v[rr]);
    }
    rmem_ln256_rows<RW>(v, g2, b2, d.eps);
#pragma unroll
    for (int rr = 0; rr < RW; ++rr) {
      cv[rr] = cvt4(v[rr]);
      st8(rcv, row_off(blk, wave, rr, 256, c0, 2), cv[rr]);
      put_a(A16, 0, wave * RW + rr, lane, cv[rr]);
    }
  }
  __syncthreads();
  zero_acc(acc);
  gemm32<4>(A16, 0, wq, ring, acc, lane);
  dump_acc(X, acc, wave, lane);
  __syncthreads();
  {
    f32x4 kk[RW], vv[RW];
#pragma unroll
    for (int rr = 0; rr < RW; ++rr) {
      f32x4 q = ld4(&X[(wave * RW + rr) * XS + c0]);
      q += bq;
      const e16x4 cq = cvt4(q);
      st8(rcq, row_off(blk, wave, rr, 256, c0, 2), cq);
      kk[rr] = up4(sk.r[rr]);
      kk[rr] += up4(cq);
      vv[rr] = up4(sv.r[rr]);
      vv[rr] += up4(cv[rr]);
    }
    rmem_ln256_rows<RW>(kk, g4, b4, d.eps);
    rmem_ln256_rows<RW>(vv, g4, b4, d.eps);
#pragma unroll
    for (int rr = 0; rr < RW; ++rr) {
      const int off = row_off(blk, wave, rr, 256, c0, 2);
      st8(rk4, off, cvt4(kk[rr]));
      st8(rv4, off, cvt4(vv[rr]));
    }
  }
}

template <bool STATS>
__global__ __launch_bounds__(NT) void k_chain_b(rmem_chain_b_desc d) {
  __shared__ __attribute__((aligned(16))) char smem[8 * PANEL * 2 + 2 * BM * XS * 4 + 4 * NW * 8 * 2 * 4];
  e16* A16 = reinterpret_cast<e16*>(smem);
  float* Xa = reinterpret_cast<float*>(smem + 8 * PANEL * 2);
  float* Xb = Xa + BM * XS;
  float* gsum = Xb + BM * XS;
  const int lane = threadIdx.x & 63, wave = __builtin_amdgcn_readfirstlane(threadIdx.x >> 6);
  const Blk blk = my_rows(d.L);
  const int c0 = lane * 4;
  const long rows = (long)d.clips * d.L;
  const rsrc_t rx = make_rsrc(d.x, rows * 1024), rt3 = make_rsrc(d.tgt3, rows * 512), rh1 = make_rsrc(d.h1, rows * 2048);
  const f32x4 bl = ld4(d.b_long + c0), bs = ld4(d.b_short + c0), g3 = ld4(d.ln3_g + c0), b3 = ld4(d.ln3_b + c0);
  f32x4 b1[4];
#pragma unroll
  for (int nb = 0; nb < 4; ++nb) b1[nb] = ld4(d.b1 + nb * 256 + c0);
  const Rows8<f32x4> xo = load_rows_f32(d.x, 256, blk, wave, c0);
  BRing ring;
  f32x4 acc[2][JT];
  const e16* wl = wstream((const e16*)d.w_long, 0, wave, 8);
  stage_tile<4>(A16, 0, (const e16*)d.att_long + blk.g0 * 256, 256, blk.nrows);
  stage_tile<4>(A16, 4, (const e16*)d.att_short + blk.g0 * 256, 256, blk.nrows);
  b_preload(ring, wl, lane);
  __syncthreads();
  zero_acc(acc);
  gemm32<4>(A16, 0, wl, ring, acc, lane);
  dump_acc(Xa, acc, wave, lane);
  const e16* ws = wstream((const e16*)d.w_short, 0, wave, 8);
  b_preload(ring, ws, lane);
  zero_acc(acc);
  gemm32<4>(A16, 4, ws, ring, acc, lane);
  dump_acc(Xb, acc, wave, lane);
  const e16* w1 = wstream((const e16*)d.w1, 0, wave, 8);
  b_preload(ring, w1, lane);
  __syncthreads();
  {
    f32x4 t[RW];
#pragma unroll
    for (int rr = 0; rr < RW; ++rr) {
      f32x4 v1 = ld4(&Xa[(wave * RW + rr) * XS + c0]);
      v1 += bl;
      t[rr] = ld4(&Xb[(wave * RW + rr) * XS + c0]);
      t[rr] += bs;
      v1 += xo.r[rr];
      st8(rt3, row_off(blk, wave, rr, 256, c0, 2), cvt4(t[rr]));
      t[rr] += v1;
      st16(rx, row_off(blk, wave, rr, 256, c0, 4), t[rr]);
    }
    rmem_ln256_rows<RW>(t, g3, b3, d.eps);
#pragma unroll
    for (int rr = 0; rr < RW; ++rr) put_a(A16, 0, wave * RW + rr, lane, cvt4(t[rr]));
  }
  __syncthreads();
#pragma unroll
  for (int nb = 0; nb < 4; ++nb) {
    float* X = (nb & 1) ? Xb : Xa;
    zero_acc(acc);
    gemm32<4>(A16, 0, w1, ring, acc, lane);
    dump_acc(X, acc, wave, lane);
    if (nb < 3) { w1 = wstream((const e16*)d.w1, nb + 1, wave, 8); b_preload(ring, w1, lane); }
    __syncthreads();
    float gs = 0.f, gss = 0.f;
#pragma unroll
    for (int rr = 0; rr < RW; ++rr) {
      f32x4 v = ld4(&X[(wave * RW + rr) * XS + c0]);
      v += b1[nb];
      const e16x4 h = cvt4(v);
      st8(rh1, row_off(blk, wave, rr, 1024, nb * 256 + c0, 2), h);
      if (STATS) {
        const f32x4 hf = up4(h);
        const float okf = wave * RW + rr < blk.nrows ? 1.f : 0.f;
        gs += okf * rmem_sum4(hf);
        gss += okf * rmem_sumsq4(hf);
      }
    }
    if (STATS) {
      gs += __shfl_xor(gs, 1); gss += __shfl_xor(gss, 1);
      gs += __shfl_xor(gs, 2); gss += __shfl_xor(gss, 2);
      gs += __shfl_xor(gs, 4); gss += __shfl_xor(gss, 4);
      if ((lane & 7) == 0) { gsum[((nb * NW + wave) * 8 + (lane >> 3)) * 2] = gs; gsum[((nb * NW + wave) * 8 + (lane >> 3)) * 2 + 1] = gss; }
    }
  }
  if (STATS) {
    __syncthreads();
    if (threadIdx.x < 32) {
      const int nb = threadIdx.x >> 3, g = threadIdx.x & 7;
      float a = 0.f, b = 0.f;
#pragma unroll
      for (int w = 0; w < NW; ++w) { a += gsum[((nb * NW + w) * 8 + g) * 2]; b += gsum[((nb * NW + w) * 8 + g) * 2 + 1]; }
      float* o = d.gn_partial + (((long)blockIdx.y * 32 + threadIdx.x) * d.gn_splits + blockIdx.x) * 2;
      o[0] = a; o[1] = b;
    }
  }
}

template <bool FFN2, bool NEXT>
__global__ __launch_bounds__(NT) void k_chain_c(rmem_chain_c_desc d) {
  constexpr int NPA = FFN2 ? 16 : 4;
  static_assert(!FFN2 || 12 * PANEL * 2 >= BM * XS * 4, "the second staging buffer must fit panels 4 .. 15");
  __shared__ __attribute__((aligned(16))) char smem[NPA * PANEL * 2 + (FFN2 ? 1 : 2) * BM * XS * 4];
  e16* A16 = reinterpret_cast<e16*>(smem);
  float* Xa = reinterpret_cast<float*>(smem + NPA * PANEL * 2);
  float* Xb = FFN2 ? reinterpret_cast<float*>(smem + 4 * PANEL * 2) : Xa + BM * XS;
  const int lane = threadIdx.x & 63, wave = __builtin_amdgcn_readfirstlane(threadIdx.x >> 6);
  const Blk blk = my_rows(d.L);
  const int c0 = lane * 4;
  const long rows = (long)d.clips * d.L;
  const rsrc_t rx = make_rsrc(d.x, rows * 1024), rdec = make_rsrc(d.dec_out, FFN2 ? ((rows - 1) * d.ld_dec + 256) * 2 : 0),
               rqkv = make_rsrc(d.qkv, NEXT ? rows * 1536 : 0);
  const f32x4 z4 = {0.f, 0.f, 0.f, 0.f};
  const f32x4 b2 = FFN2 ? ld4(d.b2 + c0) : z4, gd = FFN2 ? ld4(d.dec_g + c0) : z4, bd = FFN2 ? ld4(d.dec_b + c0) : z4;
  const f32x4 g1 = NEXT ? ld4(d.ln1_g + c0) : z4, b1 = NEXT ? ld4(d.ln1_b + c0) : z4;
  f32x4 bq[3] = {z4, z4, z4};
  if (NEXT) {
#pragma unroll
    for (int nb = 0; nb < 3; ++nb) bq[nb] = ld4(d.b_qkv + nb * 256 + c0);
  }
  const Rows8<f32x4> xo = load_rows_f32(d.x, 256, blk, wave, c0);
  BRing ring;
  f32x4 acc[2][JT];
  const e16* wq = NEXT ? wstream((const e16*)d.w_qkv, 0, wave, 8) : nullptr;
  if (FFN2) {
    const e16* w2 = wstream((const e16*)d.w2, 0, wave, 32);
    stage_tile<16>(A16, 0, (const e16*)d.h3 + blk.g0 * 1024, 1024, blk.nrows);
    b_preload(ring, w2, lane);
    __syncthreads();
    zero_acc(acc);
    gemm32<16>(A16, 0, w2, ring, acc, lane);
    dump_acc(Xa, acc, wave, lane);
    if (NEXT) b_preload(ring, wq, lane);
    __syncthreads();
  } else if (NEXT) {
    b_preload(ring, wq, lane);
  }
  {
    f32x4 v[RW];
    if (FFN2) {
      f32x4 vd[RW];
#pragma unroll
      for (int rr = 0; rr < RW; ++rr) {
        v[rr] = ld4(&Xa[(wave * RW + rr) * XS + c0]);
        v[rr] += b2;
        v[rr] += xo.r[rr];
        st16(rx, row_off(blk, wave, rr, 256, c0, 4), v[rr]);
        vd[rr] = v[rr];
      }
      rmem_ln256_rows<RW>(vd, gd, bd, d.eps);
#pragma unroll
      for (int rr = 0; rr < RW; ++rr) st8(rdec, row_off(blk, wave, rr, d.ld_dec, c0, 2), cvt4(vd[rr]));
    } else {
#pragma unroll
      for (int rr = 0; rr < RW; ++rr) v[rr] = xo.r[rr];
    }
    if (NEXT) {
      rmem_ln256_rows<RW>(v, g1, b1, d.eps);
#pragma unroll
      for (int rr = 0; rr < RW; ++rr) put_a(A16, 0, wave * RW + rr, lane, cvt4(v[rr]));
    }
  }
  if (!NEXT) return;
  __syncthreads();
#pragma unroll
  for (int nb = 0; nb < 3; ++nb) {
    float* X = (nb & 1) ? Xb : Xa;
    const Rows8<f32x4> pos = load_rows_f32(d.pos_qk + nb * 256, 768, blk, wave, c0);
    zero_acc(acc);
    gemm32<4>(A16, 0, wq, ring, acc, lane);
    dump_acc(X, acc, wave, lane);
    if (nb < 2) { wq = wstream((const e16*)d.w_qkv, nb + 1, wave, 8); b_preload(ring, wq, lane); }
    __syncthreads();
#pragma unroll
    for (int rr = 0; rr < RW; ++rr) {
      f32x4 v = ld4(&X[(wave * RW + rr) * XS + c0]);
      v += bq[nb];
      v += pos.r[rr];
      st8(rqkv, row_off(blk, wave, rr, 768, nb * 256 + c0, 2), cvt4(v));
    }
  }
}

#ifndef RMEM_F16
}
extern "C" int rmem_lstt_chain_waves(void) { return NW; }
namespace {
#endif
bool al16(const void* p) { return p == nullptr || ((uintptr_t)p % 16) == 0; }

}

extern "C" int RMEM_API(rmem_lstt_chain_a)(const rmem_chain_a_desc* d, void* stream) {
  RMEM_REQUIRE(d && d->L > 0 && d->clips >= 1 && (long)d->L * d->clips < (1L << 20), "rmem_lstt_chain_a: bad geometry (rows must stay below 2^20)");
  RMEM_REQUIRE(d->att && d->x && d->w_proj && d->b_proj && d->ln2_g && d->ln2_b && d->curr_v && d->w_q && d->b_q && d->curr_q && d->short_k &&
               d->short_v && d->ln4_g && d->ln4_b && d->k4 && d->v4, "rmem_lstt_chain_a: null argument");
  RMEM_REQUIRE(al16(d->att) && al16(d->x) && al16(d->w_proj) && al16(d->w_q) && al16(d->curr_v) && al16(d->curr_q) && al16(d->short_k) &&
               al16(d->short_v) && al16(d->k4) && al16(d->v4) && al16(d->b_proj) && al16(d->b_q) && al16(d->ln2_g) && al16(d->ln2_b) &&
               al16(d->ln4_g) && al16(d->ln4_b), "rmem_lstt_chain_a: operands must be 16-byte aligned");
  hipLaunchKernelGGL(k_chain_a, dim3((d->L + BM - 1) / BM, d->clips), dim3(NT), 0, (hipStream_t)stream, *d);
  return rmem_check_launch("rmem_lstt_chain_a");
}

extern "C" int RMEM_API(rmem_lstt_chain_b)(const rmem_chain_b_desc* d, void* stream) {
  RMEM_REQUIRE(d && d->L > 0 && d->clips >= 1 && (long)d->L * d->clips < (1L << 20), "rmem_lstt_chain_b: bad geometry (rows must stay below 2^20)");
  RMEM_REQUIRE(d->att_long && d->att_short && d->x && d->w_long && d->b_long && d->w_short && d->b_short && d->tgt3 && d->ln3_g && d->ln3_b &&
               d->w1 && d->b1 && d->h1, "rmem_lstt_chain_b: null argument");
  RMEM_REQUIRE(al16(d->att_long) && al16(d->att_short) && al16(d->x) && al16(d->w_long) && al16(d->w_short) && al16(d->tgt3) && al16(d->w1) &&
               al16(d->h1) && al16(d->b_long) && al16(d->b_short) && al16(d->b1) && al16(d->ln3_g) && al16(d->ln3_b),
               "rmem_lstt_chain_b: operands must be 16-byte aligned");
  RMEM_REQUIRE(!d->gn_partial || d->gn_splits >= (d->L + BM - 1) / BM, "rmem_lstt_chain_b: gn_splits must cover the row blocks of a clip");
  if (d->gn_partial) hipLaunchKernelGGL(k_chain_b<true>, dim3((d->L + BM - 1) / BM, d->clips), dim3(NT), 0, (hipStream_t)stream, *d);
  else hipLaunchKernelGGL(k_chain_b<false>, dim3((d->L + BM - 1) / BM, d->clips), dim3(NT), 0, (hipStream_t)stream, *d);
  return rmem_check_launch("rmem_lstt_chain_b");
}

extern "C" int RMEM_API(rmem_lstt_chain_c)(const rmem_chain_c_desc* d, void* stream) {
  RMEM_REQUIRE(d && d->L > 0 && d->clips >= 1 && (long)d->L * d->clips < (1L << 20) && d->x, "rmem_lstt_chain_c: bad geometry (rows must stay below 2^20)");
  const bool ffn2 = d->h3 != nullptr, next = d->w_qkv != nullptr;
  RMEM_REQUIRE(ffn2 || next, "rmem_lstt_chain_c: nothing to do (neither h3 nor w_qkv)");
  RMEM_REQUIRE(!ffn2 || (d->w2 && d->b2 && d->dec_g && d->dec_b && d->dec_out && d->ld_dec >= 256 && d->ld_dec % 8 == 0),
               "rmem_lstt_chain_c: the linear2 stage needs w2, b2, the decoder norm and dec_out (ld_dec >= 256, multiple of 8)");
  RMEM_REQUIRE(!next || (d->ln1_g && d->ln1_b && d->b_qkv && d->pos_qk && d->qkv), "rmem_lstt_chain_c: the QKV stage needs ln1, b_qkv, pos_qk, qkv");
  RMEM_REQUIRE(al16(d->x) && al16(d->h3) && al16(d->w2) && al16(d->b2) && al16(d->dec_g) && al16(d->dec_b) && al16(d->dec_out) && al16(d->ln1_g) &&
               al16(d->ln1_b) && al16(d->w_qkv) && al16(d->b_qkv) && al16(d->pos_qk) && al16(d->qkv), "rmem_lstt_chain_c: operands must be 16-byte aligned");
  const dim3 grid((d->L + BM - 1) / BM, d->clips);
  hipStream_t s = (hipStream_t)stream;
  if (ffn2 && next) hipLaunchKernelGGL((k_chain_c<true, true>), grid, dim3(NT), 0, s, *d);
  else if (ffn2) hipLaunchKernelGGL((k_chain_c<true, false>), grid, dim3(NT), 0, s, *d);
  else hipLaunchKernelGGL((k_chain_c<false, true>), grid, dim3(NT), 0, s, *d);
  return rmem_check_launch("rmem_lstt_chain_c");
}
```

rmem_ocu_amd/group_runtime.py:

```python
from __future__ import annotations

from typing import Dict, List, Optional, Tuple

import os

import torch

from . import ops
from .encoder_batch import BatchEncoder, SwinBatchEncoder
from .pack import R50_BLOCKS, R50_STRIDES
from .runtime import BF16, D_MODEL, F32, FFN, HEADS, MAX_CHUNKS, PLAIN_CHUNKS, _out, sine_pos_emb, temporal_slots


class GroupRuntime:
    deaot = False
    max_rows = MAX_CHUNKS
    bank_kw = bank_vw = D_MODEL
    dec_cin = 4 * D_MODEL

    def __init__(self, P: Dict[str, torch.Tensor], in_hw: Tuple[int, int], bank_slots: int, device, clips: int,
                 num_lstt: int = 3, align_corners: bool = True, num_classes: int = 11, lookahead: int = 4):
        if ('g0.qvu.w' in P) != self.deaot:
            raise ops.RmemError('GroupRuntime covers the AOTL paths (ResNet-50 / Swin-B), group_runtime_deaot.GroupRuntimeDeAOT the R50-DeAOTL path')
        self.swin = 'pe.w' in P
        self.chain = not os.environ.get('RMEM_NO_CHAIN')
        self.pair_attn = not os.environ.get('RMEM_NO_PAIR_ATTN')
        self.P, self.dev, self.NL, self.B = P, device, num_lstt, clips
        self.dt = P['proj.w'].dtype
        self.align, self.nc = align_corners, num_classes
        H, W = in_hw
        self.H, self.W = H, W
        B = clips
        if self.swin:
            if H % 4 or W % 4:
                raise ops.RmemError('Swin-B path: network size must be a multiple of 4 (the evaluator makes it a multiple of 16)')
            self.H4, self.W4 = H // 4, W // 4
            self.H8, self.W8 = (self.H4 + 1) // 2, (self.W4 + 1) // 2
            self.H16, self.W16 = (self.H8 + 1) // 2, (self.W8 + 1) // 2
            self.enc_ch = (128, 256, 512)
        else:
            self.H2, self.W2 = _out(H, 7, 2, 3), _out(W, 7, 2, 3)
            self.H4, self.W4 = _out(self.H2, 3, 2, 1), _out(self.W2, 3, 2, 1)
            self.H8, self.W8 = _out(self.H4, 3, 2, 1), _out(self.W4, 3, 2, 1)
            self.H16, self.W16 = _out(self.H8, 3, 2, 1), _out(self.W8, 3, 2, 1)
            self.enc_ch = (256, 512, 1024)
        self.L = self.H16 * self.W16
        L, M4, M8 = self.L, self.H4 * self.W4, self.H8 * self.W8
        self.M4, self.M8 = M4, M8
        e = lambda *shape, dt=None: torch.empty(*shape, dtype=dt or self.dt, device=device)
        self.enc_now = (SwinBatchEncoder if self.swin else BatchEncoder)(P, in_hw, B, device)
        self.lookahead, self.enc_bufs = lookahead, []
        self._prog: Dict[str, list] = {}
        if lookahead > 1:
            self.build_lookahead(2, lookahead)
        R = B * L
        self.dec_in = e(R, self.dec_cin)
        self.id_emb = e(R, D_MODEL)
        self.onehot = e(B * H * W, 16)
        self._alloc_lstt(R, num_lstt)
        self.gn_ws = ops.groupnorm_workspace(32, device, images=B)
        self.ffn_stats = torch.zeros(B * 32 * 64 * 2, dtype=F32, device=device)
        self.chain_stats = self.chain and (self.L + 31) // 32 <= 64 and not os.environ.get('RMEM_NO_CHAIN_STATS')
        self.conv_ws = torch.empty(16 * R * D_MODEL, dtype=F32, device=device)
        self.mass = torch.zeros(B * L * MAX_CHUNKS, dtype=F32, device=device)
        self.scores = torch.zeros(B, 32 + 64 * 32, dtype=F32, device=device)
        self.scores_host = torch.zeros(B, MAX_CHUNKS, dtype=F32).pin_memory()
        self.d16a, self.d16b = e(R, 256), e(R, 256)
        self.d8a, self.d8b = e(B * M8, 256), e(B * M8, 256)
        self.d4a, self.d4b = e(B * M4, 128), e(B * M4, 128)
        self.logits = torch.zeros(B * M4, 16, dtype=F32, device=device)
        self.S = bank_slots
        self.bank_K = [e(B * bank_slots, L, self.bank_kw) for _ in range(num_lstt)]
        self.bank_V = [e(B * bank_slots, L, self.bank_vw) for _ in range(num_lstt)]
        self.slots: List[List[int]] = [[] for _ in range(B)]
        self.free: List[List[int]] = [list(range(bank_slots)) for _ in range(B)]
        self.chunks = torch.zeros(B * self.max_rows, 8, dtype=torch.int32, device=device)
        self.chunks_ring = ops.PinnedRing(4, (B * self.max_rows, 8), torch.int32, device)
        self.append_slots = torch.full((B,), -1, dtype=torch.int32, device=device)
        self.append_ring = ops.PinnedRing(4, (B,), torch.int32, device)

    def build_lookahead(self, buffers: int, frames: int):
        self.lookahead = frames
        self.enc_bufs = [type(self.enc_now)(self.P, (self.H, self.W), self.B * frames, self.dev) for _ in range(buffers)]
        self._prog = {k: v for k, v in self._prog.items() if not k.startswith(('project_', 'decode_'))}

    def _alloc_lstt(self, R: int, num_lstt: int):
        device, L, B = self.dev, self.L, self.B
        e = lambda *shape, dt=None: torch.empty(*shape, dtype=dt or self.dt, device=device)
        self.x = e(R, D_MODEL, dt=F32)
        self.t1b = e(R, D_MODEL)
        self.qkv = e(R, 3 * D_MODEL)
        self.att = e(R, D_MODEL)
        self.att2 = e(R, D_MODEL)
        self.t3 = e(R, D_MODEL)
        self.k4, self.v4 = e(R, D_MODEL), e(R, D_MODEL)
        self.h1, self.h3 = e(R, FFN), e(R, FFN)
        self.curr_Q = [e(R, D_MODEL) for _ in range(num_lstt)]
        self.curr_V = [e(R, D_MODEL) for _ in range(num_lstt)]
        self.new_V = [e(R, D_MODEL) for _ in range(num_lstt)]
        self.tgt3 = [e(R, D_MODEL) for _ in range(num_lstt)]
        self.short_K = [e(R, D_MODEL) for _ in range(num_lstt)]
        self.short_V = [e(R, D_MODEL) for _ in range(num_lstt)]
        self.tmpA = [e(R, D_MODEL) for _ in range(num_lstt)]
        self.tmpB = [e(R, D_MODEL) for _ in range(num_lstt)]
        pos = sine_pos_emb(self.H16, self.W16).to(device)
        self.posb = pos.to(self.dt).repeat(B, 1).contiguous()
        self.pos_qk = [torch.zeros(R, 3 * D_MODEL, dtype=F32, device=device) for _ in range(num_lstt)]
        self._pos_ready = False
        self.attn_ws = ops.attn_workspace(L, HEADS, MAX_CHUNKS, device, nclips=B)
# ... 91 lines not shown

    def prog_project(self, e: Optional[int]) -> list:
        key = f'project_{e}'
        if key not in self._prog:
            self._prog[key] = [ops.conv2d(self._enc(e)[2], self.P['proj.w'], self.P['proj.b'], self.x, H=self.B * self.L, W=1,
                                          Cin=self.enc_ch[2], Cout=D_MODEL, y2=self.dec_in, ld2=4 * D_MODEL, ws=self.conv_ws)]
        return self._prog[key]

    def prog_lstt(self, ref_mode: bool, T: int, want_mass: bool = True) -> list:
        key = 'lstt_ref' if ref_mode else f'lstt_prop{T}{"m" if want_mass else ""}'
        if key in self._prog:
            return self._prog[key]
        P, L, B, o = self.P, self.L, self.B, []
        C = D_MODEL
        R = B * L
        _, nchunks = self.chunk_plan(1 if ref_mode else T)
        if not ref_mode and self.chain:
            self._prog[key] = self._prog_lstt_chained(T, nchunks, want_mass)
            return self._prog[key]
        for i in range(self.NL):
            d = f'l{i}'
            o.append(ops.layernorm256(self.x, P[d + '.ln1.g'], P[d + '.ln1.b'], M=R, y=self.t1b))
            o.append(self._lin(self.t1b, d + '.self_qkv', self.qkv, C, 3 * C, residual=self.pos_qk[i]))
            o.append(self._attn(self.qkv, 3 * C, self.qkv.view(-1)[C:], self.qkv.view(-1)[2 * C:], 3 * C, self.att,
                                nchunks=PLAIN_CHUNKS, lk_single=L, kv_cs=L * 3 * C))
            o.append(self._lin(self.att, d + '.self_proj', self.x, C, C, residual=self.x))
            o.append(ops.layernorm256(self.x, P[d + '.ln2.g'], P[d + '.ln2.b'], M=R, y=self.curr_V[i]))
            cq = self.curr_Q[i]
            o.append(self._lin(self.curr_V[i], d + '.linear_Q', cq, C, C))
            if ref_mode:
                o.append(ops.add16(self.curr_V[i], self.id_emb, self.tmpB[i], R * C))
                o.append(self._lin(self.tmpB[i], d + '.linear_V', self.new_V[i], C, C))
                o.append(self._scatter(cq, self.bank_K[i]))
                o.append(self._scatter(self.new_V[i], self.bank_V[i]))
                sk, sv = cq, self.new_V[i]
            else:
                sk, sv = self.short_K[i], self.short_V[i]
            o.append(self._attn(cq, C, self.bank_K[i], self.bank_V[i], C, self.att, slot_stride=L * C, chunks=self.chunks,
                                nchunks=nchunks, lk_single=(1 if ref_mode else T) * L, pe_cur=P['pe_cur'], pe_mem=P['pe_mem'],
                                mass=self.mass if (i == 0 and not ref_mode and want_mass) else None, T=T))
            o.append(self._lin(self.att, d + '.long_proj', self.x, C, C, residual=self.x))
            o.append(ops.layernorm256_pair(sk, cq, self.k4, sv, self.curr_V[i], self.v4, P[d + '.ln4.g'], P[d + '.ln4.b'], M=R))
            o.append(self._attn(cq, C, self.k4, self.v4, C, self.att, nchunks=PLAIN_CHUNKS, lk_single=L, kv_cs=L * C))
            o.append(self._lin(self.att, d + '.short_proj', self.x, C, C, residual=self.x, y2=self.tgt3[i]))
            if ref_mode:
                o.append(self._lin(self.tgt3[i], d + '.linear_QMem', self.short_K[i], C, C))
                o.append(ops.add16(self.tgt3[i], self.id_emb, self.tmpA[i], R * C))
                o.append(self._lin(self.tmpA[i], d + '.linear_VMem', self.short_V[i], C, C))
            o.append(ops.layernorm256(self.x, P[d + '.ln3.g'], P[d + '.ln3.b'], M=R, y=self.t3))
            o.append(self._lin(self.t3, d + '.linear1', self.h1, C, FFN))
            o.append(ops.gn_act_dwconv5x5(self.h1, P[d + '.gn.g'], P[d + '.gn.b'], P[d + '.dw.w'], self.h3, self.gn_ws, H=self.H16,
                                          W=self.W16, C=FFN, groups=32, act=2, images=B))
            o.append(self._lin(self.h3, d + '.linear2', self.x, FFN, C, residual=self.x))
            o.append(ops.layernorm256(self.x, P[f'dec_norm{i}.g'], P[f'dec_norm{i}.b'], M=R,
                                      y=self.dec_in.view(-1)[(i + 1) * C:], ldy=4 * C))
        self._prog[key] = o
        return o

    def _prog_lstt_chained(self, T: int, nchunks: int, want_mass: bool) -> list:
        P, L, B, C, o = self.P, self.L, self.B, D_MODEL, []
        ln = lambda n: (P[n + '.g'], P[n + '.b'])

        def chain_c(i_done, i_next):
            kw = {}
            if i_done is not None:
                d = f'l{i_done}'
                kw.update(h3=self.h3, w2=P[d + '.linear2.wf'], b2=P[d + '.linear2.b'], dec_norm=ln(f'dec_norm{i_done}'),
                          dec_out=self.dec_in.view(-1)[(i_done + 1) * C:], ld_dec=self.dec_cin)
            if i_next is not None:
                d = f'l{i_next}'
                kw.update(ln1=ln(d + '.ln1'), w_qkv=P[d + '.self_qkv.wf'], b_qkv=P[d + '.self_qkv.b'], pos_qk=self.pos_qk[i_next], qkv=self.qkv)
            return ops.lstt_chain_c(L=L, clips=B, x=self.x, dt=self.dt, **kw)

        o.append(chain_c(None, 0))
        for i in range(self.NL):
            d = f'l{i}'
            cq = self.curr_Q[i]
            o.append(self._attn(self.qkv, 3 * C, self.qkv.view(-1)[C:], self.qkv.view(-1)[2 * C:], 3 * C, self.att,
                                nchunks=PLAIN_CHUNKS, lk_single=L, kv_cs=L * 3 * C))
            o.append(ops.lstt_chain_a(L=L, clips=B, att=self.att, x=self.x, w_proj=P[d + '.self_proj.wf'], b_proj=P[d + '.self_proj.b'],
                                      ln2=ln(d + '.ln2'), curr_v=self.curr_V[i], w_q=P[d + '.linear_Q.wf'], b_q=P[d + '.linear_Q.b'], curr_q=cq,
                                      short_k=self.short_K[i], short_v=self.short_V[i], ln4=ln(d + '.ln4'), k4=self.k4, v4=self.v4))
            mass = self.mass if (i == 0 and want_mass) else None
            if self.pair_attn:
                o.append(ops.lstt_attn_pair(cq, self.bank_K[i], self.bank_V[i], self.att, self.k4, self.v4, self.att2, self.attn_ws, Lq=L,
                                            heads=HEADS, ldq=C, ldkv=C, ldo=C, slot_stride=L * C, chunks=self.chunks, nchunks=nchunks,
                                            lk_total=T * L, pe_cur=P['pe_cur'], pe_mem=P['pe_mem'], mass=mass, T=T, nclips=B, q_cs=L * C,
                                            out_cs=L * C, lk_short=L, kv_short_cs=L * C, out_short_cs=L * C))
            else:
                o.append(self._attn(cq, C, self.bank_K[i], self.bank_V[i], C, self.att, slot_stride=L * C, chunks=self.chunks,
                                    nchunks=nchunks, lk_single=T * L, pe_cur=P['pe_cur'], pe_mem=P['pe_mem'], mass=mass, T=T))
                o.append(self._attn(cq, C, self.k4, self.v4, C, self.att2, nchunks=PLAIN_CHUNKS, lk_single=L, kv_cs=L * C))
            o.append(ops.lstt_chain_b(L=L, clips=B, att_long=self.att, att_short=self.att2, x=self.x, w_long=P[d + '.long_proj.wf'],
                                      b_long=P[d + '.long_proj.b'], w_short=P[d + '.short_proj.wf'], b_short=P[d + '.short_proj.b'],
                                      tgt3=self.tgt3[i], ln3=ln(d + '.ln3'), w1=P[d + '.linear1.wf'], b1=P[d + '.linear1.b'], h1=self.h1,
                                      gn_partial=self.ffn_stats if self.chain_stats else None, gn_splits=64 if self.chain_stats else 0))
            if self.chain_stats:
                o.append(ops.gn_act_dwconv5x5_prestats(self.h1, P[d + '.gn.g'], P[d + '.gn.b'], P[d + '.dw.w'], self.h3, self.ffn_stats,
                                                       H=self.H16, W=self.W16, C=FFN, groups=32, act=2, images=B))
            else:
                o.append(ops.gn_act_dwconv5x5(self.h1, P[d + '.gn.g'], P[d + '.gn.b'], P[d + '.dw.w'], self.h3, self.gn_ws, H=self.H16,
                                              W=self.W16, C=FFN, groups=32, act=2, images=B))
            o.append(chain_c(i, i + 1 if i + 1 < self.NL else None))
        return o

    def prog_decode(self, e: Optional[int]) -> list:
        key = f'decode_{e}'
        if key in self._prog:
            return self._prog[key]
        P, o, L, B = self.P, [], self.L, self.B
        M8, M4 = self.M8, self.M4
        enc1, enc2, enc3 = self._enc(e)
        gn = lambda x, name, y, M, C: ops.groupnorm(x, P[name + '.gn.g'], P[name + '.gn.b'], y, self.gn_ws, M=M, C=C, groups=8, act=1,
                                                    images=B)
        lin = lambda x, name, y, M, K, N, **kw: ops.conv2d(x, P[name + '.w'], P[name + '.b'], y, H=B * M, W=1, Cin=K, Cout=N,
                                                           ws=self.conv_ws, **kw)
        o.append(lin(self.dec_in, 'dec.conv_in', self.d16a, L, self.dec_cin, 256))
        o.append(gn(self.d16a, 'dec.conv_in', self.d16b, L, 256))
        c4, c8, c16 = self.enc_ch
        o.append(lin(enc3, 'dec.adapter_16x', self.d16a, L, c16, 256, residual=self.d16b))
        o.append(self._conv(self.d16a, P['dec.conv_16x.w'], P['dec.conv_16x.b'], self.d16b, H=self.H16, W=self.W16, Cin=256, Cout=256,
                            KH=3, KW=3, pad=1))
        o.append(gn(self.d16b, 'dec.conv_16x', self.d16a, L, 256))
        fuse_up = not os.environ.get('RMEM_NO_UPFUSE')
        if fuse_up:
            o.append(ops.conv2d(enc2, P['dec.adapter_8x.w'], P['dec.adapter_8x.b'], self.d8b, H=self.H8, W=self.W8, Cin=c8, Cout=256,
                                batch=B, residual=self.d16a, res_up=(self.H16, self.W16, self.align)))
        else:
            o.append(ops.bilinear(self.d16a, self.d8a, Hi=self.H16, Wi=self.W16, Ho=self.H8, Wo=self.W8, C=256, align_corners=self.align,
                                  images=B))
            o.append(lin(enc2, 'dec.adapter_8x', self.d8b, M8, c8, 256, residual=self.d8a))
        d8c = self.d8a.view(-1)[: B * M8 * 128]
        o.append(self._conv(self.d8b, P['dec.conv_8x.w'], P['dec.conv_8x.b'], d8c, H=self.H8, W=self.W8, Cin=256, Cout=128, KH=3, KW=3,
                            pad=1))
        d8d = self.d8b.view(-1)[: B * M8 * 128]
        o.append(gn(d8c, 'dec.conv_8x', d8d, M8, 128))
        if fuse_up:
            o.append(ops.conv2d(enc1, P['dec.adapter_4x.w'], P['dec.adapter_4x.b'], self.d4b, H=self.H4, W=self.W4, Cin=c4, Cout=128,
                                batch=B, residual=d8d, res_up=(self.H8, self.W8, self.align)))
        else:
            o.append(ops.bilinear(d8d, self.d4a, Hi=self.H8, Wi=self.W8, Ho=self.H4, Wo=self.W4, C=128, align_corners=self.align, images=B))
            o.append(lin(enc1, 'dec.adapter_4x', self.d4b, M4, c4, 128, residual=self.d4a))
        if os.environ.get('RMEM_DIRECT_CONV3_128') == '1':
            o.append(ops.conv3x3_direct(self.d4b, P['dec.conv_4x.w'], P['dec.conv_4x.b'], self.d4a, H=self.H4, W=self.W4, C=128, images=B))
        else:
            o.append(self._conv(self.d4b, P['dec.conv_4x.w'], P['dec.conv_4x.b'], self.d4a, H=self.H4, W=self.W4, Cin=128, Cout=128, KH=3,
                                KW=3, pad=1))
        if os.environ.get('RMEM_NO_HEADFUSE'):
            o.append(gn(self.d4a, 'dec.conv_4x', self.d4b, M4, 128))
            o.append(lin(self.d4b, 'dec.conv_out', self.logits, M4, 128, self.nc, ldo=16))
        else:
            o.append(ops.groupnorm_head(self.d4a, P['dec.conv_4x.gn.g'], P['dec.conv_4x.gn.b'], P['dec.conv_out.w'], P['dec.conv_out.b'],
                                        self.logits, self.gn_ws, M=M4, C=128, groups=8, N=self.nc, ldy=16, act=1, images=B))
        self._prog[key] = o
        return o

    def prog_id_emb(self, labels: torch.Tensor, hs: int, ws: int) -> list:
        key = f'id_{labels.data_ptr()}_{hs}_{ws}'
        if key in self._prog:
            return self._prog[key]
        P, B = self.P, self.B
        k, s, p = (17, 16, 8) if self.align else (16, 16, 0)
        if os.environ.get('RMEM_NO_LABEL_EMBED', '0') != '1':
            if getattr(self, 'lab_net', None) is None:
                self.lab_net = ops.label_id_embed_scratch(B, self.H, self.W, p, self.dev)
            o = [ops.label_id_embed(labels, P['idbank.w'], P['idbank.b'], self.lab_net, self.id_emb, Hs=hs, Ws=ws, H=self.H, W=self.W, K=k,
                                    stride=s, pad=p, ncls=self.nc, images=B)]
        else:
            o = [ops.label_to_onehot16(labels, self.onehot, Hs=hs, Ws=ws, Hd=self.H, Wd=self.W, ncls=self.nc, images=B)]
            o.append(self._conv(self.onehot, P['idbank.w'], P['idbank.b'], self.id_emb, H=self.H, W=self.W, Cin=16, Cout=D_MODEL,
                                KH=k, KW=k, stride=s, pad=p))
        self._prog[key] = o
        return o

    def prog_update(self, append: bool) -> list:
        key = f'update_{int(append)}'
        if key in self._prog:
            return self._prog[key]
        P, NL, L, C, B = self.P, self.NL, self.L, D_MODEL, self.B
# ... 22 lines not shown
```

rmem_ocu_amd/ops.py:

```python
from __future__ import annotations

import ctypes as C
import os
from typing import Dict, Optional, Sequence

import torch

from . import _lib
from ._lib import AttnChunk, ConvDesc, RmemError

BF16 = torch.bfloat16
F16 = torch.float16
F32 = torch.float32
E16 = (BF16, F16)


def _fn(name: str, dt):
    if dt not in E16:
        raise RmemError(f'{name}: 16-bit operands must be bfloat16 or float16, got {dt}')
    return getattr(_lib.lib(), name + ('_f16' if dt == F16 else ''))


def _first16(*ts):
    for t in ts:
# ... 59 lines not shown
        if ws.numel() * ws.element_size() < _lib.lib().rmem_conv_workspace_bytes(C.byref(d)):
            ws = None
    args = (C.byref(d), _ptr(x), _ptr(w), _ptr(bias), _ptr(residual), _ptr(y), _ptr(y2), _ptr(ws))
    return Op(_fn('rmem_conv2d_nhwc', dt), args, 'rmem_conv2d_nhwc', (d, x, w, bias, residual, y, y2, ws))


def conv_plan(*, H, W, Cin, Cout, KH=1, KW=1, stride=1, pad=0, batch=1, ldx=0, has_ws=False, entry='conv2d', extra=0) -> Dict[str, int]:
    Ho = (H + 2 * pad - KH) // stride + 1
    Wo = (W + 2 * pad - KW) // stride + 1
    d = ConvDesc(H, W, Cin, Ho, Wo, Cout, KH, KW, stride, pad, Cout, Cout, Cout, 0, 0, 0, ldx, batch, 0, 0, 0, 0)
    pl = _lib.GemmPlan()
    _lib.check(_lib.lib().rmem_conv_plan(C.byref(d), int(has_ws), _lib.GEMM_ENTRIES.index(entry), extra, C.byref(pl)), 'rmem_conv_plan')
    return {n: getattr(pl, n) for n, _ in pl._fields_}


def conv1x1_dual(x, x2, w_cat, bias, y, *, H, W, Cin, Cout, H2, W2, Cin2, stride2, relu=False, batch=1) -> Op:
    _dev(x, x2, w_cat, bias, y)
    dt = w_cat.dtype
    assert x.dtype == dt and x2.dtype == dt and w_cat.dtype == dt and w_cat.is_contiguous() and y.dtype == dt
    assert w_cat.numel() == Cout * (Cin + Cin2) and bias.dtype == F32 and bias.numel() == Cout
    assert x.numel() >= batch * H * W * Cin and x2.numel() >= batch * H2 * W2 * Cin2 and y.numel() >= batch * H * W * Cout
    d = ConvDesc(H, W, Cin, H, W, Cout, 1, 1, 1, 0, Cout, Cout, Cout, int(relu), 0, 0, 0, batch, 0, 0, 0, 0)
    args = (C.byref(d), _ptr(x), _ptr(x2), H2, W2, Cin2, stride2, _ptr(w_cat), _ptr(bias), _ptr(y))
    return Op(_fn('rmem_conv1x1_dual_nhwc', dt), args, 'rmem_conv1x1_dual_nhwc', (d, x, x2, w_cat, bias, y))


def bneck_chain(b, w3, bias3, y, w1, bias1, a2, *, H, W, K1, N2, residual=None, x2=None, H2=0, W2=0, Cin2=0, stride2=1, batch=1) -> Op:
    _dev(b, w3, bias3, y, w1, bias1, a2, residual, x2)
    dt = w3.dtype
    M = batch * H * W
    assert (residual is None) != (x2 is None)
    assert all(t.dtype == dt for t in (b, y, w1, a2)) and bias3.dtype == F32 and bias1.dtype == F32
    assert w3.is_contiguous() and w1.is_contiguous() and w3.numel() == 256 * (K1 + (Cin2 if x2 is not None else 0)) and w1.numel() == N2 * 256
    assert b.numel() >= M * K1 and y.numel() >= M * 256 and a2.numel() >= M * N2 and bias3.numel() == 256 and bias1.numel() == N2
    assert residual is None or (residual.dtype == dt and residual.numel() >= M * 256)
    assert x2 is None or (x2.dtype == dt and x2.numel() >= batch * H2 * W2 * Cin2)
    d = _lib.BneckChainDesc(batch, H, W, K1, 256, N2, H2, W2, Cin2, stride2)
    args = (C.byref(d), _ptr(b), _ptr(x2), _ptr(w3), _ptr(bias3), _ptr(residual), _ptr(y), _ptr(w1), _ptr(bias1), _ptr(a2))
    return Op(_fn('rmem_bneck_chain', dt), args, 'rmem_bneck_chain', (d, b, x2, w3, bias3, residual, y, w1, bias1, a2))


def linear(x, w, bias, y, *, M, K, N, residual=None, y2=None, relu=False, ldo=None, ldr=None, ld2=None, ws=None, ldx=0,
           act_begin=0) -> Op:
    return conv2d(x, w, bias, y, H=M, W=1, Cin=K, Cout=N, residual=residual, y2=y2, relu=relu, ldo=ldo, ldr=ldr, ld2=ld2, ws=ws,
                  ldx=ldx, act_begin=act_begin)


def _ptr_array(ts):
    return (C.c_void_p * len(ts))(*[_ptr(t) for t in ts])


def linear_grouped(xs, ws, biases, ys, *, M, K, N, residuals=None, relu=False) -> Op:
    n = len(xs)
    assert 1 <= n <= 4 and len(ws) == n and len(ys) == n and (biases is None or len(biases) == n)
    _dev(*xs, *ws, *ys, *(biases or ()), *(residuals or ()))
    dt = ws[0].dtype
    for x, w, y in zip(xs, ws, ys):
        assert x.dtype == dt and w.dtype == dt and w.numel() == N * K and x.numel() >= M * K and y.numel() >= M * N
    assert len({y.dtype for y in ys}) == 1 and (residuals is None or len({r.dtype for r in residuals}) == 1)
    d = ConvDesc(M, 1, K, M, 1, N, 1, 1, 1, 0, N, N, N, int(relu), int(ys[0].dtype == F32),
                 int(residuals is not None and residuals[0].dtype == F32), 0, 1, 0)
    arrs = (_ptr_array(xs), _ptr_array(ws), _ptr_array(biases) if biases is not None else None,
            _ptr_array(residuals) if residuals is not None else None, _ptr_array(ys))
    args = (C.byref(d), n, arrs[0], arrs[1], arrs[2], arrs[3], arrs[4])
    return Op(_fn('rmem_linear_grouped', dt), args, 'rmem_linear_grouped', (d, arrs, xs, ws, biases, residuals, ys))


def add16_grouped(as_, bs, ys, n: int) -> Op:
    _dev(*as_, *bs, *ys)
    dt = as_[0].dtype
    assert len(as_) == len(bs) == len(ys) <= 8 and all(t.dtype == dt for t in (*as_, *bs, *ys))
    arrs = (_ptr_array(as_), _ptr_array(bs), _ptr_array(ys))
    return Op(_fn('rmem_add16_grouped', dt), (len(as_), arrs[0], arrs[1], arrs[2], n), 'rmem_add16_grouped', (arrs, as_, bs, ys))


def layernorm256_pair(a0, b0, y0, a1, b1, y1, gamma, beta, *, M, eps=1e-5) -> Op:
    _dev(a0, b0, y0, a1, b1, y1, gamma, beta)
    dt = a0.dtype
    assert all(t.dtype == dt and t.numel() >= M * 256 for t in (a0, b0, y0, a1, b1, y1)) and gamma.dtype == F32
    args = (_ptr(a0), _ptr(b0), _ptr(y0), _ptr(a1), _ptr(b1), _ptr(y1), _ptr(gamma), _ptr(beta), eps, M)
    return Op(_fn('rmem_layernorm256_pair', dt), args, 'rmem_layernorm256_pair', (a0, b0, y0, a1, b1, y1, gamma, beta))


def _chain(name, cls, ints, ptrs, dt):
    ts = list(ptrs.values())
    _dev(*ts)
    for k, t in ptrs.items():
        if t is not None and t.data_ptr() % 16:
            raise RmemError(f'{name}: {k} must be 16-byte aligned')
    d = cls(int(ints[0]), int(ints[1]), float(ints[2]), int(ints[3]), *[_ptr(t) for t in ts])
    return Op(_fn(name, dt), (C.byref(d),), name, (d, ts))


def lstt_chain_a(*, L, clips, att, x, w_proj, b_proj, ln2, curr_v, w_q, b_q, curr_q, short_k, short_v, ln4, k4, v4, eps=1e-5) -> Op:
    dt = att.dtype
    R = clips * L
    assert x.dtype == F32 and x.numel() >= R * 256 and all(t.dtype == dt and t.numel() >= R * 256 for t in (att, curr_v, curr_q, short_k, short_v, k4, v4))
    assert w_proj.dtype == dt and w_q.dtype == dt and w_proj.numel() == 65536 and w_q.numel() == 65536
    return _chain('rmem_lstt_chain_a', _lib.ChainA, (L, clips, eps, 0),
                  dict(att=att, x=x, w_proj=w_proj, b_proj=b_proj, ln2_g=ln2[0], ln2_b=ln2[1], curr_v=curr_v, w_q=w_q, b_q=b_q, curr_q=curr_q,
                       short_k=short_k, short_v=short_v, ln4_g=ln4[0], ln4_b=ln4[1], k4=k4, v4=v4), dt)


def lstt_chain_b(*, L, clips, att_long, att_short, x, w_long, b_long, w_short, b_short, tgt3, ln3, w1, b1, h1, gn_partial=None,
                 gn_splits=0, eps=1e-5) -> Op:
    dt = att_long.dtype
    R = clips * L
    assert x.dtype == F32 and all(t.dtype == dt and t.numel() >= R * 256 for t in (att_long, att_short, tgt3)) and h1.dtype == dt and h1.numel() >= R * 1024
    assert w_long.numel() == 65536 and w_short.numel() == 65536 and w1.numel() == 262144 and b1.numel() == 1024
    assert gn_partial is None or (gn_partial.dtype == F32 and gn_splits * 32 >= L and gn_partial.numel() >= clips * 32 * gn_splits * 2)
    return _chain('rmem_lstt_chain_b', _lib.ChainB, (L, clips, eps, gn_splits),
                  dict(att_long=att_long, att_short=att_short, x=x, w_long=w_long, b_long=b_long, w_short=w_short, b_short=b_short, tgt3=tgt3,
                       ln3_g=ln3[0], ln3_b=ln3[1], w1=w1, b1=b1, h1=h1, gn_partial=gn_partial), dt)


def lstt_chain_c(*, L, clips, x, dt, h3=None, w2=None, b2=None, dec_norm=(None, None), dec_out=None, ld_dec=0, ln1=(None, None), w_qkv=None,
                 b_qkv=None, pos_qk=None, qkv=None, eps=1e-5) -> Op:
    R = clips * L
    assert x.dtype == F32 and x.numel() >= R * 256
    assert h3 is None or (h3.dtype == dt and h3.numel() >= R * 1024 and w2.numel() == 262144 and dec_out.numel() >= (R - 1) * ld_dec + 256)
    assert w_qkv is None or (w_qkv.numel() == 196608 and pos_qk.dtype == F32 and pos_qk.numel() >= R * 768 and qkv.dtype == dt and qkv.numel() >= R * 768)
    return _chain('rmem_lstt_chain_c', _lib.ChainC, (L, clips, eps, ld_dec),
                  dict(x=x, h3=h3, w2=w2, b2=b2, dec_g=dec_norm[0], dec_b=dec_norm[1], dec_out=dec_out, ln1_g=ln1[0], ln1_b=ln1[1], w_qkv=w_qkv,
                       b_qkv=b_qkv, pos_qk=pos_qk, qkv=qkv), dt)


def attn_workspace(Lq: int, heads: int, nchunks: int, device, nclips: int = 1) -> torch.Tensor:
    n = nclips * _lib.lib().rmem_attn_workspace_bytes(Lq, heads, nchunks)
    return torch.empty(n // 4, dtype=F32, device=device)


def make_chunk_table(chunks: Sequence[Sequence[int]]) -> torch.Tensor:
    t = torch.zeros(len(chunks), 8, dtype=torch.int32)
    for i, c in enumerate(chunks):
        t[i, :5] = torch.tensor(list(c), dtype=torch.int32)
    return t


def mem_read_attn(q, k_bank, v_bank, out, workspace, *, Lq, heads=8, ldq, ldkv, ldo, slot_stride=0, chunks=None,
                  nchunks=1, lk_single=0, pe_cur=None, pe_mem=None, mass=None, T=0, nclips=1, q_cs=0, kv_cs=0, out_cs=0) -> Op:
    _dev(q, k_bank, v_bank, out, workspace, chunks, pe_cur, pe_mem, mass)
    dt = q.dtype
    assert q.dtype == dt and k_bank.dtype == dt and v_bank.dtype == dt and out.dtype == dt
    assert workspace.numel() * 4 >= nclips * _lib.lib().rmem_attn_workspace_bytes(Lq, heads, nchunks)
    assert chunks is None or (chunks.dtype == torch.int32 and chunks.numel() >= nclips * nchunks * 8)
    assert mass is None or (mass.dtype == F32 and mass.numel() >= nclips * Lq * T)
    args = (_ptr(q), ldq, _ptr(k_bank), _ptr(v_bank), slot_stride, ldkv, _ptr(chunks), nchunks, lk_single,
            _ptr(pe_cur), _ptr(pe_mem), Lq, heads, _ptr(out), ldo, _ptr(mass), T, nclips, q_cs, kv_cs, out_cs, _ptr(workspace))
    return Op(_fn('rmem_mem_read_attn_clips', dt), args, 'rmem_mem_read_attn',
              (q, k_bank, v_bank, out, workspace, chunks, pe_cur, pe_mem, mass))


def lstt_attn_pair(q, k_bank, v_bank, out_long, k_short, v_short, out_short, workspace, *, Lq, heads=8, ldq, ldkv, ldo, slot_stride, chunks,
                   nchunks, lk_total, pe_cur, pe_mem, mass=None, T=0, nclips=1, q_cs=0, out_cs=0, lk_short, kv_short_cs=0, out_short_cs=0) -> Op:
    _dev(q, k_bank, v_bank, out_long, k_short, v_short, out_short, workspace, chunks, pe_cur, pe_mem, mass)
    dt = q.dtype
    assert all(t.dtype == dt for t in (k_bank, v_bank, out_long, k_short, v_short, out_short))
    assert workspace.numel() * 4 >= nclips * _lib.lib().rmem_attn_workspace_bytes(Lq, heads, nchunks)
    assert chunks.dtype == torch.int32 and chunks.numel() >= nclips * nchunks * 8
    assert mass is None or (mass.dtype == F32 and mass.numel() >= nclips * Lq * T)
    assert k_short.numel() >= (nclips - 1) * kv_short_cs + (lk_short - 1) * ldkv + heads * 32
    args = (_ptr(q), ldq, _ptr(k_bank), _ptr(v_bank), slot_stride, ldkv, _ptr(chunks), nchunks, lk_total, _ptr(pe_cur), _ptr(pe_mem), Lq, heads,
            _ptr(out_long), ldo, _ptr(mass), T, nclips, q_cs, out_cs, _ptr(k_short), _ptr(v_short), lk_short, kv_short_cs, _ptr(out_short),
            out_short_cs, _ptr(workspace))
    return Op(_fn('rmem_lstt_attn_pair_clips', dt), args, 'rmem_lstt_attn_pair',
              (q, k_bank, v_bank, out_long, k_short, v_short, out_short, workspace, chunks, pe_cur, pe_mem, mass))


def layernorm256(a, gamma, beta, *, M, lda=256, b=None, ldb=256, y=None, ldy=256, pos=None, ypos=None, ldyp=256,
                 yf=None, ldyf=256, eps=1e-5) -> Op:
    _dev(a, b, gamma, beta, y, pos, ypos, yf)
    dt = _first16(y, ypos, a, b)
    assert a.dtype in (dt, F32) and (b is None or b.dtype in (dt, F32))
    assert gamma.dtype == F32 and beta.dtype == F32 and gamma.numel() == 256
    assert (y is None or y.dtype == dt) and (ypos is None or ypos.dtype == dt) and (yf is None or yf.dtype == F32)
    args = (_ptr(a), int(a.dtype == F32), lda, _ptr(b), int(b is not None and b.dtype == F32), ldb, _ptr(gamma), _ptr(beta),
            eps, M, _ptr(y), ldy, _ptr(pos), _ptr(ypos), ldyp, _ptr(yf), ldyf)
    return Op(_fn('rmem_layernorm256', dt), args, 'rmem_layernorm256', (a, b, gamma, beta, y, pos, ypos, yf))


def layernorm(a, gamma, beta, *, M, C, lda=None, y=None, ldy=None, yf=None, ldyf=None, eps=1e-5) -> Op:
    _dev(a, gamma, beta, y, yf)
    dt = _first16(y, a)
    assert a.dtype in (dt, F32) and gamma.dtype == F32 and gamma.numel() == C
    args = (_ptr(a), int(a.dtype == F32), C if lda is None else lda, _ptr(gamma), _ptr(beta), eps, M, C, _ptr(y),
            C if ldy is None else ldy, _ptr(yf), C if ldyf is None else ldyf)
    return Op(_fn('rmem_layernorm', dt), args, 'rmem_layernorm', (a, gamma, beta, y, yf))


def patch_merge_ln(x, gamma, beta, y, *, H, W, C, eps=1e-5, images=1) -> Op:
    _dev(x, gamma, beta, y)
    dt = y.dtype
    assert x.dtype == F32 and y.dtype == dt and gamma.numel() == 4 * C
    return Op(_fn('rmem_patch_merge_ln_images', dt), (_ptr(x), images, H, W, C, _ptr(gamma), _ptr(beta), eps, _ptr(y)), 'rmem_patch_merge_ln',
              (x, gamma, beta, y))


def window_attn(qkv, qkv_bias, table, out, *, H, W, C, heads, shift, images=1) -> Op:
    _dev(qkv, qkv_bias, table, out)
    dt = qkv.dtype
    assert qkv.dtype == dt and out.dtype == dt and qkv_bias.dtype == F32 and table.dtype == F32
    assert qkv_bias.numel() == 3 * C and table.numel() == 4 * heads * 49 * 49 and table.is_contiguous()
    assert qkv.numel() >= images * H * W * 3 * C and out.numel() >= images * H * W * C
    return Op(_fn('rmem_window_attn_images', dt), (_ptr(qkv), _ptr(qkv_bias), _ptr(table), _ptr(out), images, H, W, C, heads, shift),
              'rmem_window_attn', (qkv, qkv_bias, table, out))


def add16(a, b, y, n: int) -> Op:
    _dev(a, b, y)
    dt = a.dtype
    assert a.dtype == dt and b.dtype == dt and y.dtype == dt
    return Op(_fn('rmem_add16', dt), (_ptr(a), _ptr(b), _ptr(y), n), 'rmem_add16', (a, b, y))


def groupnorm_workspace(groups: int, device, images: int = 1) -> torch.Tensor:
    return torch.empty(images * _lib.lib().rmem_groupnorm_workspace_bytes(groups) // 4, dtype=F32, device=device)


def groupnorm(x, gamma, beta, y, ws, *, M, C, groups, act=0, eps=1e-5, images=1) -> Op:
    _dev(x, gamma, beta, y, ws)
    dt = y.dtype
    assert x.dtype in (dt, F32) and y.dtype == dt and gamma.dtype == F32 and gamma.numel() == C
    assert ws.numel() * 4 >= images * _lib.lib().rmem_groupnorm_workspace_bytes(groups)
    if images > 1:
        assert x.dtype == dt
        args = (_ptr(x), images, M, C, groups, _ptr(gamma), _ptr(beta), eps, act, _ptr(y), _ptr(ws))
        return Op(_fn('rmem_groupnorm_nhwc_images', dt), args, 'rmem_groupnorm_nhwc', (x, gamma, beta, y, ws))
    args = (_ptr(x), M, C, groups, _ptr(gamma), _ptr(beta), eps, act, _ptr(y), _ptr(ws))
    if x.dtype == F32:
        return Op(_fn('rmem_groupnorm_f32_nhwc', dt), args, 'rmem_groupnorm_f32_nhwc', (x, gamma, beta, y, ws))
    return Op(_fn('rmem_groupnorm_nhwc', dt), args, 'rmem_groupnorm_nhwc', (x, gamma, beta, y, ws))


def groupnorm_head(x, gamma, beta, w, bias, y, ws, *, M, C, groups, N, ldy, act=1, eps=1e-5, images=1) -> Op:
    _dev(x, gamma, beta, w, bias, y, ws)
    dt = x.dtype
    assert x.dtype == dt and w.dtype == dt and y.dtype == F32 and gamma.dtype == F32 and gamma.numel() == C
    assert w.numel() == N * C and w.is_contiguous() and (bias is None or (bias.dtype == F32 and bias.numel() == N))
    assert x.numel() >= images * M * C and y.numel() >= (images * M - 1) * ldy + N
    assert ws.numel() * 4 >= images * _lib.lib().rmem_groupnorm_workspace_bytes(groups)
    args = (_ptr(x), images, M, C, groups, _ptr(gamma), _ptr(beta), eps, act, _ptr(w), _ptr(bias), N, _ptr(y), ldy, _ptr(ws))
    return Op(_fn('rmem_groupnorm_head_nhwc_images', dt), args, 'rmem_groupnorm_head_nhwc', (x, gamma, beta, w, bias, y, ws))


def gn_act_dwconv5x5(x, gamma, beta, w_t, y, ws, *, H, W, C, groups, act=2, eps=1e-5, images=1) -> Op:
    _dev(x, gamma, beta, w_t, y, ws)
    dt = x.dtype
    assert x.dtype == dt and y.dtype == dt and w_t.dtype == F32 and w_t.numel() == 25 * C and gamma.numel() == C
    assert ws.numel() * 4 >= images * _lib.lib().rmem_groupnorm_workspace_bytes(groups)
# ... 382 lines not shown
```

Measured before the change: 3368 frames/s.

## Fold split-KV attention combine into LSTT chain_b and template chain row tile

The long-term memory attention can now skip its separate combine kernel. It hands the per-group partial outputs and max/logsumexp values to chain_b, which merges them while staging its A tile. This removes one kernel launch plus a write and read of the combined attention output per LSTT layer. The chain kernels are also templated on the row tile size (32 or 64), picked by a heuristic or an environment override. The trade-off is extra merge arithmetic and scattered partial reads inside chain_b, plus more register and LDS pressure.

Result: faster. 3426 frames/s, median of 6 (+1.7%).

```diff
diff --git a/include/rmem.h b/include/rmem.h
--- a/include/rmem.h
+++ b/include/rmem.h
@@ -103,6 +103,20 @@
                               const void* k_short, const void* v_short, int lk_short, long long kv_short_clip_stride,
                               void* out_short, long long out_short_clip_stride, void* workspace, void* stream);
 
+typedef struct rmem_attn_merge {
+  int ngroups, heads, Lq, reserved;
+  const void* opart;
+  const float* mlg;
+  long long opart_cs, mlg_cs;
+} rmem_attn_merge;
+int rmem_lstt_attn_pair_clips_deferred(const void* q, int ldq, const void* k_bank, const void* v_bank, long long slot_stride, int ldkv,
+                                       const rmem_attn_chunk* chunks, int nchunks, int lk_total, const float* pe_cur, const float* pe_mem,
+                                       int Lq, int heads, void* out_long, int ldo, float* attn_mass, int T, int nclips,
+                                       long long q_clip_stride, long long out_clip_stride,
+                                       const void* k_short, const void* v_short, int lk_short, long long kv_short_clip_stride,
+                                       void* out_short, long long out_short_clip_stride, void* workspace,
+                                       rmem_attn_merge* merge, void* stream);
+
 int rmem_profile_start(int max_launches);
 int rmem_profile_stop(double* total_ms, double* total_flops, int* launches);
 
@@ -115,6 +129,7 @@
                            const float* gamma, const float* beta, float eps, int M, void* stream);
 
 int rmem_lstt_chain_waves(void);
+int rmem_lstt_chain_rows(int L, int clips, int cus);
 typedef struct rmem_chain_a_desc {
   int L, clips; float eps; int reserved;
   const void* att; float* x;
@@ -131,6 +146,7 @@
   const float* ln3_g; const float* ln3_b; const void* w1; const float* b1; void* h1; float* gn_partial;
 } rmem_chain_b_desc;
 int rmem_lstt_chain_b(const rmem_chain_b_desc* d, void* stream);
+int rmem_lstt_chain_b_merged(const rmem_chain_b_desc* d, const rmem_attn_merge* merge, void* stream);
 
 typedef struct rmem_chain_c_desc {
   int L, clips; float eps; int ld_dec;
@@ -491,6 +507,7 @@
 int rmem_mem_read_attn_f16(const void* q, int ldq, const void* k_bank, const void* v_bank, long long slot_stride, int ldkv, const rmem_attn_chunk* chunks, int nchunks, int lk_single, const float* pe_cur, const float* pe_mem, int Lq, int heads, void* out, int ldo, float* attn_mass, int T, void* workspace, void* stream);
 int rmem_mem_read_attn_clips_f16(const void* q, int ldq, const void* k_bank, const void* v_bank, long long slot_stride, int ldkv, const rmem_attn_chunk* chunks, int nchunks, int lk_single, const float* pe_cur, const float* pe_mem, int Lq, int heads, void* out, int ldo, float* attn_mass, int T, int nclips, long long q_clip_stride, long long kv_clip_stride, long long out_clip_stride, void* workspace, void* stream);
 int rmem_lstt_attn_pair_clips_f16(const void* q, int ldq, const void* k_bank, const void* v_bank, long long slot_stride, int ldkv, const rmem_attn_chunk* chunks, int nchunks, int lk_total, const float* pe_cur, const float* pe_mem, int Lq, int heads, void* out_long, int ldo, float* attn_mass, int T, int nclips, long long q_clip_stride, long long out_clip_stride, const void* k_short, const void* v_short, int lk_short, long long kv_short_clip_stride, void* out_short, long long out_short_clip_stride, void* workspace, void* stream);
+int rmem_lstt_attn_pair_clips_deferred_f16(const void* q, int ldq, const void* k_bank, const void* v_bank, long long slot_stride, int ldkv, const rmem_attn_chunk* chunks, int nchunks, int lk_total, const float* pe_cur, const float* pe_mem, int Lq, int heads, void* out_long, int ldo, float* attn_mass, int T, int nclips, long long q_clip_stride, long long out_clip_stride, const void* k_short, const void* v_short, int lk_short, long long kv_short_clip_stride, void* out_short, long long out_short_clip_stride, void* workspace, rmem_attn_merge* merge, void* stream);
 int rmem_layernorm256_f16(const void* a, int a_is_f32, int lda, const void* b, int b_is_f32, int ldb, const float* gamma, const float* beta, float eps, int M, void* y_bf16, int ldy, const float* pos, void* ypos_bf16, int ldyp, float* y_f32, int ldyf, void* stream);
 int rmem_layernorm_f16(const void* a, int a_is_f32, int lda, const float* gamma, const float* beta, float eps, int M, int C, void* y_bf16, int ldy, float* y_f32, int ldyf, void* stream);
 int rmem_patch_merge_ln_f16(const float* x, int H, int W, int C, const float* gamma, const float* beta, float eps, void* y_bf16, void* stream);
@@ -501,6 +518,7 @@
 int rmem_add16_grouped_f16(int n, const void* const* a, const void* const* b, void* const* y, long long count, void* stream);
 int rmem_lstt_chain_a_f16(const rmem_chain_a_desc* d, void* stream);
 int rmem_lstt_chain_b_f16(const rmem_chain_b_desc* d, void* stream);
+int rmem_lstt_chain_b_merged_f16(const rmem_chain_b_desc* d, const rmem_attn_merge* merge, void* stream);
 int rmem_lstt_chain_c_f16(const rmem_chain_c_desc* d, void* stream);
 int rmem_layernorm256_pair_f16(const void* a0, const void* b0, void* y0, const void* a1, const void* b1, void* y1, const float* gamma, const float* beta, float eps, int M, void* stream);
 int rmem_bneck_chain_f16(const rmem_bneck_chain_desc* desc, const void* b, const void* x2, const void* w3, const float* bias3, const void* res, void* y, const void* w1, const float* bias1, void* a2, void* stream);
diff --git a/rmem_ocu_amd/_lib.py b/rmem_ocu_amd/_lib.py
--- a/rmem_ocu_amd/_lib.py
+++ b/rmem_ocu_amd/_lib.py
@@ -90,6 +90,10 @@
 
 
 ROUTE_LIVE, ROUTE_IDLE, ROUTE_SKIP = 0, 1, 2
+
+
+class AttnMerge(C.Structure):
+    _fields_ = [('ngroups', _i), ('heads', _i), ('Lq', _i), ('reserved', _i), ('opart', _vp), ('mlg', _vp), ('opart_cs', _ll), ('mlg_cs', _ll)]
 
 
 def _desc(name, ints, ptrs):
@@ -124,8 +128,10 @@
     'rmem_add16_grouped': (_i, [_i, C.POINTER(_vp), C.POINTER(_vp), C.POINTER(_vp), _ll, _vp]),
     'rmem_layernorm256_pair': (_i, [_vp, _vp, _vp, _vp, _vp, _vp, _vp, _vp, _f, _i, _vp]),
     'rmem_lstt_chain_waves': (_i, []),
+    'rmem_lstt_chain_rows': (_i, [_i, _i, _i]),
     'rmem_lstt_chain_a': (_i, [C.POINTER(ChainA), _vp]),
     'rmem_lstt_chain_b': (_i, [C.POINTER(ChainB), _vp]),
+    'rmem_lstt_chain_b_merged': (_i, [C.POINTER(ChainB), C.POINTER(AttnMerge), _vp]),
     'rmem_lstt_chain_c': (_i, [C.POINTER(ChainC), _vp]),
     'rmem_conv1x1_dual_nhwc': (_i, [C.POINTER(ConvDesc), _vp, _vp, _i, _i, _i, _i, _vp, _vp, _vp, _vp]),
     'rmem_bneck_chain': (_i, [C.POINTER(BneckChainDesc), _vp, _vp, _vp, _vp, _vp, _vp, _vp, _vp, _vp, _vp]),
@@ -141,6 +147,8 @@
     'rmem_mem_read_attn_clips': (_i, [_vp, _i, _vp, _vp, _ll, _i, _vp, _i, _i, _vp, _vp, _i, _i, _vp, _i, _vp, _i, _i, _ll, _ll, _ll, _vp, _vp]),
     'rmem_lstt_attn_pair_clips': (_i, [_vp, _i, _vp, _vp, _ll, _i, _vp, _i, _i, _vp, _vp, _i, _i, _vp, _i, _vp, _i, _i, _ll, _ll,
                                        _vp, _vp, _i, _ll, _vp, _ll, _vp, _vp]),
+    'rmem_lstt_attn_pair_clips_deferred': (_i, [_vp, _i, _vp, _vp, _ll, _i, _vp, _i, _i, _vp, _vp, _i, _i, _vp, _i, _vp, _i, _i, _ll, _ll,
+                                                _vp, _vp, _i, _ll, _vp, _ll, _vp, C.POINTER(AttnMerge), _vp]),
     'rmem_gn_act_dwconv5x5_nhwc': (_i, [_vp, _i, _i, _i, _i, _vp, _vp, _f, _i, _vp, _vp, _vp, _vp]),
     'rmem_dwconv5x5_nhwc': (_i, [_vp, _vp, _vp, _i, _i, _i, _vp]),
     'rmem_image_to_nhwc8': (_i, [_vp, _vp, _i, _i, _vp]),
@@ -248,8 +256,8 @@
     'rmem_graph_destroy': (_i, [_vp]),
 }
 
-F16_TWINS = ('rmem_conv2d_nhwc', 'rmem_mem_read_attn', 'rmem_mem_read_attn_clips', 'rmem_lstt_attn_pair_clips', 'rmem_layernorm256', 'rmem_layernorm', 'rmem_patch_merge_ln',
-             'rmem_window_attn', 'rmem_window_attn_images', 'rmem_patch_merge_ln_images', 'rmem_add16', 'rmem_add16_grouped', 'rmem_layernorm256_pair', 'rmem_lstt_chain_a', 'rmem_lstt_chain_b', 'rmem_lstt_chain_c', 'rmem_conv1x1_dual_nhwc', 'rmem_bneck_chain', 'rmem_label_id_embed', 'rmem_image_ptrs_to_nhwc4p', 'rmem_stem7x7s2', 'rmem_stem7x7s2_pool', 'rmem_conv3x3_c64_direct', 'rmem_conv3x3_direct', 'rmem_linear_grouped',
+F16_TWINS = ('rmem_conv2d_nhwc', 'rmem_mem_read_attn', 'rmem_mem_read_attn_clips', 'rmem_lstt_attn_pair_clips', 'rmem_lstt_attn_pair_clips_deferred', 'rmem_layernorm256', 'rmem_layernorm', 'rmem_patch_merge_ln',
+             'rmem_window_attn', 'rmem_window_attn_images', 'rmem_patch_merge_ln_images', 'rmem_add16', 'rmem_add16_grouped', 'rmem_layernorm256_pair', 'rmem_lstt_chain_a', 'rmem_lstt_chain_b', 'rmem_lstt_chain_b_merged', 'rmem_lstt_chain_c', 'rmem_conv1x1_dual_nhwc', 'rmem_bneck_chain', 'rmem_label_id_embed', 'rmem_image_ptrs_to_nhwc4p', 'rmem_stem7x7s2', 'rmem_stem7x7s2_pool', 'rmem_conv3x3_c64_direct', 'rmem_conv3x3_direct', 'rmem_linear_grouped',
              'rmem_groupnorm_nhwc', 'rmem_groupnorm_f32_nhwc', 'rmem_groupnorm_nhwc_images', 'rmem_groupnorm_head_nhwc_images',
              'rmem_gn_act_dwconv5x5_nhwc_images', 'rmem_gn_act_dwconv5x5_prestats_nhwc_images', 'rmem_gn_act_dwconv5x5_nhwc', 'rmem_dwconv5x5_nhwc', 'rmem_image_to_nhwc8',
              'rmem_image_to_nhwc8_images', 'rmem_image_ptrs_to_nhwc8', 'rmem_ingest_rgb8', 'rmem_maxpool3x3s2_nhwc', 'rmem_maxpool3x3s2_nhwc_images', 'rmem_bilinear_nhwc',
diff --git a/rmem_ocu_amd/csrc/attention.hip b/rmem_ocu_amd/csrc/attention.hip
--- a/rmem_ocu_amd/csrc/attention.hip
+++ b/rmem_ocu_amd/csrc/attention.hip
@@ -588,7 +588,8 @@
                        const float* pe_cur, const float* pe_mem, int Lq, int heads, void* out, int ldo,
                        float* attn_mass, int T, int nclips, long long q_clip_stride, long long kv_clip_stride,
                        long long out_clip_stride, void* workspace, void* stream,
-                       const void* k2, const void* v2, int lk2, long long kv2_clip_stride, void* out2, long long out2_clip_stride) {
+                       const void* k2, const void* v2, int lk2, long long kv2_clip_stride, void* out2, long long out2_clip_stride,
+                       rmem_attn_merge* defer = nullptr) {
   RMEM_REQUIRE(nclips >= 1 && nclips <= 64, "rmem_mem_read_attn: 1..64 clips");
   RMEM_REQUIRE(q_clip_stride % 8 == 0 && kv_clip_stride % 8 == 0 && out_clip_stride % 8 == 0, "rmem_mem_read_attn: clip strides must be multiples of 8 elements");
   const long long prof_keys = chunks ? (long long)lk_single : 0;
@@ -645,7 +646,11 @@
   cp.opart = p.opart; cp.mlg = p.mlg; cp.ngroups = p.ngroups; cp.ml = p.ml; cp.chunks = chunks; cp.nchunks = nchunks;
   cp.Lq = Lq; cp.heads = heads; cp.out = (e16*)out; cp.ldo = ldo; cp.mass = attn_mass; cp.T = T;
   cp.out_cs = out_clip_stride; cp.opart_cs = p.opart_cs; cp.mlg_cs = p.mlg_cs; cp.ml_cs = p.ml_cs; cp.mass_cs = (long)Lq * T;
-  if (p.ngroups > 1) hipLaunchKernelGGL(k_attn_combine, dim3((Lq + 63) / 64, 16, nclips), dim3(256), 0, s, cp);
+  if (defer) {
+    defer->ngroups = p.ngroups; defer->heads = heads; defer->Lq = Lq; defer->reserved = 0;
+    defer->opart = p.opart; defer->mlg = p.mlg; defer->opart_cs = p.opart_cs; defer->mlg_cs = p.mlg_cs;
+  }
+  if (p.ngroups > 1 && !defer) hipLaunchKernelGGL(k_attn_combine, dim3((Lq + 63) / 64, 16, nclips), dim3(256), 0, s, cp);
   if (attn_mass) hipLaunchKernelGGL(k_attn_mass, dim3((Lq + 63) / 64, 1, nclips), dim3(256), 0, s, cp);
   return rmem_check_launch("rmem_mem_read_attn");
 }
@@ -671,6 +676,19 @@
                      out_short_clip_stride);
 }
 
+extern "C" int RMEM_API(rmem_lstt_attn_pair_clips_deferred)(const void* q, int ldq, const void* k_bank, const void* v_bank, long long slot_stride,
+                                                  int ldkv, const rmem_attn_chunk* chunks, int nchunks, int lk_total,
+                                                  const float* pe_cur, const float* pe_mem, int Lq, int heads, void* out_long, int ldo,
+                                                  float* attn_mass, int T, int nclips, long long q_clip_stride, long long out_clip_stride,
+                                                  const void* k_short, const void* v_short, int lk_short, long long kv_short_clip_stride,
+                                                  void* out_short, long long out_short_clip_stride, void* workspace,
+                                                  rmem_attn_merge* merge, void* stream) {
+  RMEM_REQUIRE(chunks && k_short && v_short && out_short && merge, "rmem_lstt_attn_pair_deferred: null argument");
+  return attn_launch(q, ldq, k_bank, v_bank, slot_stride, ldkv, chunks, nchunks, lk_total, pe_cur, pe_mem, Lq, heads, out_long, ldo, attn_mass, T,
+                     nclips, q_clip_stride, 0, out_clip_stride, workspace, stream, k_short, v_short, lk_short, kv_short_clip_stride, out_short,
+                     out_short_clip_stride, merge);
+}
+
 extern "C" int RMEM_API(rmem_mem_read_attn)(const void* q, int ldq, const void* k_bank, const void* v_bank, long long slot_stride,
                                   int ldkv, const rmem_attn_chunk* chunks, int nchunks, int lk_single,
                                   const float* pe_cur, const float* pe_mem, int Lq, int heads, void* out, int ldo,
diff --git a/rmem_ocu_amd/csrc/rowchain.hip b/rmem_ocu_amd/csrc/rowchain.hip
--- a/rmem_ocu_amd/csrc/rowchain.hip
+++ b/rmem_ocu_amd/csrc/rowchain.hip
@@ -1,6 +1,7 @@
 #include "common.h"
 #include "lds_dma.h"
 #include "../../include/rmem.h"
+#include <stdlib.h>
 
 namespace {
 
@@ -12,9 +13,7 @@
 constexpr int JT = 16 / NW;
 constexpr int WC = 256 / NW;
 constexpr int RW = 32 / NW;
-constexpr int BM = 32;
 constexpr int XS = 260;
-constexpr int PANEL = BM * 64;
 constexpr int PF = 16 / JT;
 
 __device__ __forceinline__ f32x4 ld4(const float* p) { return *reinterpret_cast<const f32x4*>(p); }
@@ -31,22 +30,75 @@
 __device__ inline void st16(rsrc_t, int, f32x4) {}
 #endif
 
-template <int NP>
+template <int BM, int NP>
 __device__ __forceinline__ void stage_tile(e16* A16, int p0, const e16* src, long ld, int nrows) {
-  constexpr int PT = NT / 256;
-  static_assert(NP % PT == 0, "panels must divide among the thread halves");
-  const int t = threadIdx.x & 255, half = threadIdx.x >> 8;
-  const int row = t >> 3, ch = t & 7;
-  const e16* sr = src + min(row, nrows - 1) * ld + ch * 8;
-  e16x8 v[NP / PT];
-#pragma unroll
-  for (int p = 0; p < NP / PT; ++p) v[p] = *reinterpret_cast<const e16x8*>(sr + (p * PT + half) * 64);
-#pragma unroll
-  for (int p = 0; p < NP / PT; ++p) *reinterpret_cast<e16x8*>(&A16[(p0 + p * PT + half) * PANEL + swz(row, ch)]) = v[p];
-}
-
+  constexpr int NI = NP * BM * 8 / NT;
+  static_assert(NP * BM * 8 % NT == 0, "the chunks must divide among the threads");
+  const int ch = threadIdx.x & 7;
+  e16x8 v[NI];
+#pragma unroll
+  for (int k = 0; k < NI; ++k) {
+    const int i = (threadIdx.x + k * NT) >> 3, row = i % BM;
+    v[k] = *reinterpret_cast<const e16x8*>(src + min(row, nrows - 1) * ld + ch * 8 + (i / BM) * 64);
+  }
+#pragma unroll
+  for (int k = 0; k < NI; ++k) {
+    const int i = (threadIdx.x + k * NT) >> 3, row = i % BM;
+    *reinterpret_cast<e16x8*>(&A16[(p0 + i / BM) * (BM * 64) + swz(row, ch)]) = v[k];
+  }
+}
+
+template <int BM>
 __device__ __forceinline__ void put_a(e16* A16, int p0, int row, int lane, e16x4 v) {
-  *reinterpret_cast<e16x4*>(&A16[(p0 + (lane >> 4)) * PANEL + swz(row, (lane & 15) >> 1) + (lane & 1) * 4]) = v;
+  *reinterpret_cast<e16x4*>(&A16[(p0 + (lane >> 4)) * (BM * 64) + swz(row, (lane & 15) >> 1) + (lane & 1) * 4]) = v;
+}
+
+constexpr float MERGE_NEG_BIG = -1.0e30f;
+template <int BM>
+__device__ __forceinline__ void stage_merged(e16* A16, const rmem_attn_merge& mg, int nrows, int L) {
+#pragma clang fp contract(off)
+  constexpr int TQ = NT / BM;
+  constexpr int HP = TQ >= 8 ? 1 : 8 / TQ;
+  constexpr int GP = TQ > 8 ? 64 / TQ : 8;
+  const int ql = threadIdx.x % BM, hh = threadIdx.x / BM;
+  const long q = blockIdx.x * BM + min(ql, nrows - 1);
+  const float* mlg = mg.mlg + blockIdx.y * mg.mlg_cs;
+  const e16x4* op = reinterpret_cast<const e16x4*>(reinterpret_cast<const float*>(mg.opart) + blockIdx.y * mg.opart_cs);
+#pragma unroll
+  for (int hp = 0; hp < HP; ++hp) {
+    const int head = TQ > 8 ? hh / (TQ / 8) : hh * HP + hp, G0 = TQ > 8 ? (hh % (TQ / 8)) * GP : 0;
+    float m = MERGE_NEG_BIG;
+    for (int c = 0; c < mg.ngroups; ++c) {
+      const f32x2 mlv = *reinterpret_cast<const f32x2*>(mlg + ((c * 8 + head) * (long)L + q) * 2);
+      m = mlv[1] > 0.f ? fmaxf(m, mlv[0]) : m;
+    }
+    f32x4 num[GP];
+#pragma unroll
+    for (int g = 0; g < GP; ++g) num[g] = f32x4{0.f, 0.f, 0.f, 0.f};
+    float den = 0.f;
+    for (int c = 0; c < mg.ngroups; ++c) {
+      const long ch = c * 8 + head;
+      const f32x2 mlv = *reinterpret_cast<const f32x2*>(mlg + (ch * L + q) * 2);
+      e16x4 o4[GP];
+#pragma unroll
+      for (int g = 0; g < GP; ++g) o4[g] = op[(ch * 8 + G0 + g) * L + q];
+      const bool ok = mlv[1] > 0.f;
+      const float e = __builtin_amdgcn_exp2f(mlv[0] - m);
+      const float w = e * mlv[1];
+      den = ok ? __builtin_fmaf(mlv[1], e, den) : den;
+#pragma unroll
+      for (int g = 0; g < GP; ++g)
+#pragma unroll
+        for (int i = 0; i < 4; ++i) num[g][i] = ok ? __builtin_fmaf(w, (float)o4[g][i], num[g][i]) : num[g][i];
+    }
+    const float inv = 1.f / den;
+#pragma unroll
+    for (int g = 0; g < GP; ++g) {
+      const int G = G0 + g;
+      const f32x4 o = num[g] * inv;
+      *reinterpret_cast<e16x4*>(&A16[(head >> 1) * (BM * 64) + swz(ql, (head & 1) * 4 + (G >> 1)) + (G & 1) * 4]) = cvt4(o);
+    }
+  }
 }
 
 struct BRing { e16x8 b[PF][JT]; };
@@ -61,20 +113,20 @@
   __builtin_amdgcn_sched_barrier(0);
 }
 
-template <int NP>
-__device__ __forceinline__ void gemm32(const e16* A16, int p0, const e16* wp, BRing& r, f32x4 (&acc)[2][JT], int lane) {
-  constexpr int KC = NP * 2;
+template <int BM, int NP>
+__device__ __forceinline__ void gemm_rows(const e16* A16, int p0, const e16* wp, BRing& r, f32x4 (&acc)[BM / 16][JT], int lane) {
+  constexpr int KC = NP * 2, MT = BM / 16;
   const int fr = lane & 15, fc = lane >> 4;
 #pragma unroll
   for (int kc = 0; kc < KC; ++kc) {
-    const e16* Ap = A16 + (p0 + (kc >> 1)) * PANEL;
-    const e16x8 a0 = *reinterpret_cast<const e16x8*>(&Ap[swz(fr, 4 * (kc & 1) + fc)]);
-    const e16x8 a1 = *reinterpret_cast<const e16x8*>(&Ap[swz(16 + fr, 4 * (kc & 1) + fc)]);
-#pragma unroll
-    for (int j = 0; j < JT; ++j) {
-      acc[0][j] = RMEM_MFMA_16x16x32(a0, r.b[kc % PF][j], acc[0][j], 0, 0, 0);
-      acc[1][j] = RMEM_MFMA_16x16x32(a1, r.b[kc % PF][j], acc[1][j], 0, 0, 0);
-    }
+    const e16* Ap = A16 + (p0 + (kc >> 1)) * (BM * 64);
+    e16x8 a[MT];
+#pragma unroll
+    for (int i = 0; i < MT; ++i) a[i] = *reinterpret_cast<const e16x8*>(&Ap[swz(16 * i + fr, 4 * (kc & 1) + fc)]);
+#pragma unroll
+    for (int j = 0; j < JT; ++j)
+#pragma unroll
+      for (int i = 0; i < MT; ++i) acc[i][j] = RMEM_MFMA_16x16x32(a[i], r.b[kc % PF][j], acc[i][j], 0, 0, 0);
     if (kc + PF < KC) {
 #pragma unroll
       for (int j = 0; j < JT; ++j) r.b[kc % PF][j] = *reinterpret_cast<const e16x8*>(wp + (((kc + PF) * JT + j) * 64 + lane) * 8);
@@ -83,17 +135,19 @@
   }
 }
 
-__device__ __forceinline__ void zero_acc(f32x4 (&acc)[2][JT]) {
-#pragma unroll
-  for (int i = 0; i < 2; ++i)
+template <int MT>
+__device__ __forceinline__ void zero_acc(f32x4 (&acc)[MT][JT]) {
+#pragma unroll
+  for (int i = 0; i < MT; ++i)
 #pragma unroll
     for (int j = 0; j < JT; ++j) acc[i][j] = f32x4{0.f, 0.f, 0.f, 0.f};
 }
 
-__device__ __forceinline__ void dump_acc(float* X, const f32x4 (&acc)[2][JT], int wave, int lane) {
+template <int MT>
+__device__ __forceinline__ void dump_acc(float* X, const f32x4 (&acc)[MT][JT], int wave, int lane) {
   const int fr = lane & 15, fc = lane >> 4;
 #pragma unroll
-  for (int i = 0; i < 2; ++i)
+  for (int i = 0; i < MT; ++i)
 #pragma unroll
     for (int j = 0; j < JT; ++j)
 #pragma unroll
@@ -101,6 +155,7 @@
 }
 
 struct Blk { int nrows; long g0; };
+template <int BM>
 __device__ __forceinline__ Blk my_rows(int L) {
   Blk b;
   const int r0 = blockIdx.x * BM;
@@ -112,208 +167,263 @@
 template <typename T>
 struct Rows8 { T r[RW]; };
 
-__device__ __forceinline__ Rows8<f32x4> load_rows_f32(const float* base, int ld, const Blk& blk, int wave, int c0) {
+__device__ __forceinline__ int wrow(int h, int wave, int rr) { return h * 32 + wave * RW + rr; }
+
+__device__ __forceinline__ Rows8<f32x4> load_rows_f32(const float* base, int ld, const Blk& blk, int h, int wave, int c0) {
   Rows8<f32x4> o;
 #pragma unroll
   for (int rr = 0; rr < RW; ++rr) {
-    const int row = min(wave * RW + rr, blk.nrows - 1);
+    const int row = min(wrow(h, wave, rr), blk.nrows - 1);
     o.r[rr] = ld4(base + (blk.g0 + row) * ld + c0);
   }
   return o;
 }
-__device__ __forceinline__ Rows8<e16x4> load_rows_e16(const e16* base, int ld, const Blk& blk, int wave, int c0) {
+__device__ __forceinline__ Rows8<e16x4> load_rows_e16(const e16* base, int ld, const Blk& blk, int h, int wave, int c0) {
   Rows8<e16x4> o;
 #pragma unroll
   for (int rr = 0; rr < RW; ++rr) {
-    const int row = min(wave * RW + rr, blk.nrows - 1);
+    const int row = min(wrow(h, wave, rr), blk.nrows - 1);
     o.r[rr] = *reinterpret_cast<const e16x4*>(base + (blk.g0 + row) * ld + c0);
   }
   return o;
 }
-__device__ __forceinline__ int row_off(const Blk& blk, int wave, int rr, int ld, int c0, int esz) {
-  const int row = wave * RW + rr;
+__device__ __forceinline__ int row_off(const Blk& blk, int h, int wave, int rr, int ld, int c0, int esz) {
+  const int row = wrow(h, wave, rr);
   return row < blk.nrows ? (int)(((blk.g0 + row) * ld + c0) * esz) : OOB;
 }
 
+template <int BM>
 __global__ __launch_bounds__(NT) void k_chain_a(rmem_chain_a_desc d) {
+  constexpr int NH = BM / 32, MT = BM / 16, PANEL = BM * 64;
   __shared__ __attribute__((aligned(16))) char smem[4 * PANEL * 2 + BM * XS * 4];
   e16* A16 = reinterpret_cast<e16*>(smem);
   float* X = reinterpret_cast<float*>(smem + 4 * PANEL * 2);
   const int lane = threadIdx.x & 63, wave = __builtin_amdgcn_readfirstlane(threadIdx.x >> 6);
-  const Blk blk = my_rows(d.L);
+  const Blk blk = my_rows<BM>(d.L);
   const int c0 = lane * 4;
   const long rows = (long)d.clips * d.L;
   const rsrc_t rx = make_rsrc(d.x, rows * 1024), rcv = make_rsrc(d.curr_v, rows * 512), rcq = make_rsrc(d.curr_q, rows * 512),
                rk4 = make_rsrc(d.k4, rows * 512), rv4 = make_rsrc(d.v4, rows * 512);
   const f32x4 bp = ld4(d.b_proj + c0), g2 = ld4(d.ln2_g + c0), b2 = ld4(d.ln2_b + c0);
   const f32x4 bq = ld4(d.b_q + c0), g4 = ld4(d.ln4_g + c0), b4 = ld4(d.ln4_b + c0);
-  const Rows8<f32x4> xo = load_rows_f32(d.x, 256, blk, wave, c0);
-  const Rows8<e16x4> sk = load_rows_e16((const e16*)d.short_k, 256, blk, wave, c0);
-  const Rows8<e16x4> sv = load_rows_e16((const e16*)d.short_v, 256, blk, wave, c0);
+  Rows8<f32x4> xo[NH];
+  Rows8<e16x4> sk[NH], sv[NH];
+#pragma unroll
+  for (int h = 0; h < NH; ++h) xo[h] = load_rows_f32(d.x, 256, blk, h, wave, c0);
+  if (NH == 1) {
+    sk[0] = load_rows_e16((const e16*)d.short_k, 256, blk, 0, wave, c0);
+    sv[0] = load_rows_e16((const e16*)d.short_v, 256, blk, 0, wave, c0);
+  }
   BRing ring;
-  f32x4 acc[2][JT];
+  f32x4 acc[MT][JT];
   const e16* wp = wstream((const e16*)d.w_proj, 0, wave, 8);
-  stage_tile<4>(A16, 0, (const e16*)d.att + blk.g0 * 256, 256, blk.nrows);
+  stage_tile<BM, 4>(A16, 0, (const e16*)d.att + blk.g0 * 256, 256, blk.nrows);
   b_preload(ring, wp, lane);
   __syncthreads();
   zero_acc(acc);
-  gemm32<4>(A16, 0, wp, ring, acc, lane);
+  gemm_rows<BM, 4>(A16, 0, wp, ring, acc, lane);
   dump_acc(X, acc, wave, lane);
   const e16* wq = wstream((const e16*)d.w_q, 0, wave, 8);
   b_preload(ring, wq, lane);
   __syncthreads();
-  e16x4 cv[RW];
-  {
+  e16x4 cv[NH][RW];
+#pragma unroll
+  for (int h = 0; h < NH; ++h) {
     f32x4 v[RW];
 #pragma unroll
     for (int rr = 0; rr < RW; ++rr) {
-      v[rr] = ld4(&X[(wave * RW + rr) * XS + c0]);
+      v[rr] = ld4(&X[wrow(h, wave, rr) * XS + c0]);
       v[rr] += bp;
-      v[rr] += xo.r[rr];
-      st16(rx, row_off(blk, wave, rr, 256, c0, 4), v[rr]);
+      v[rr] += xo[h].r[rr];
+      st16(rx, row_off(blk, h, wave, rr, 256, c0, 4), v[rr]);
     }
     rmem_ln256_rows<RW>(v, g2, b2, d.eps);
 #pragma unroll
     for (int rr = 0; rr < RW; ++rr) {
-      cv[rr] = cvt4(v[rr]);
-      st8(rcv, row_off(blk, wave, rr, 256, c0, 2), cv[rr]);
-      put_a(A16, 0, wave * RW + rr, lane, cv[rr]);
+      cv[h][rr] = cvt4(v[rr]);
+      st8(rcv, row_off(blk, h, wave, rr, 256, c0, 2), cv[h][rr]);
+      put_a<BM>(A16, 0, wrow(h, wave, rr), lane, cv[h][rr]);
+    }
+  }
+  if (NH > 1) {
+#pragma unroll
+    for (int h = 0; h < NH; ++h) {
+      sk[h] = load_rows_e16((const e16*)d.short_k, 256, blk, h, wave, c0);
+      sv[h] = load_rows_e16((const e16*)d.short_v, 256, blk, h, wave, c0);
     }
   }
   __syncthreads();
   zero_acc(acc);
-  gemm32<4>(A16, 0, wq, ring, acc, lane);
+  gemm_rows<BM, 4>(A16, 0, wq, ring, acc, lane);
   dump_acc(X, acc, wave, lane);
   __syncthreads();
-  {
+#pragma unroll
+  for (int h = 0; h < NH; ++h) {
     f32x4 kk[RW], vv[RW];
 #pragma unroll
     for (int rr = 0; rr < RW; ++rr) {
-      f32x4 q = ld4(&X[(wave * RW + rr) * XS + c0]);
+      f32x4 q = ld4(&X[wrow(h, wave, rr) * XS + c0]);
       q += bq;
       const e16x4 cq = cvt4(q);
-      st8(rcq, row_off(blk, wave, rr, 256, c0, 2), cq);
-      kk[rr] = up4(sk.r[rr]);
+      st8(rcq, row_off(blk, h, wave, rr, 256, c0, 2), cq);
+      kk[rr] = up4(sk[h].r[rr]);
       kk[rr] += up4(cq);
-      vv[rr] = up4(sv.r[rr]);
-      vv[rr] += up4(cv[rr]);
+      vv[rr] = up4(sv[h].r[rr]);
+      vv[rr] += up4(cv[h][rr]);
     }
     rmem_ln256_rows<RW>(kk, g4, b4, d.eps);
     rmem_ln256_rows<RW>(vv, g4, b4, d.eps);
 #pragma unroll
     for (int rr = 0; rr < RW; ++rr) {
-      const int off = row_off(blk, wave, rr, 256, c0, 2);
+      const int off = row_off(blk, h, wave, rr, 256, c0, 2);
       st8(rk4, off, cvt4(kk[rr]));
       st8(rv4, off, cvt4(vv[rr]));
     }
   }
 }
 
-template <bool STATS>
-__global__ __launch_bounds__(NT) void k_chain_b(rmem_chain_b_desc d) {
-  __shared__ __attribute__((aligned(16))) char smem[8 * PANEL * 2 + 2 * BM * XS * 4 + 4 * NW * 8 * 2 * 4];
+template <int BM, bool STATS, bool MERGE>
+__global__ __launch_bounds__(NT) void k_chain_b(rmem_chain_b_desc d, rmem_attn_merge mg) {
+  constexpr int NH = BM / 32, MT = BM / 16, PANEL = BM * 64;
+  constexpr bool TWO = BM == 32;
+  __shared__ __attribute__((aligned(16))) char smem[8 * PANEL * 2 + (TWO ? 2 : 1) * BM * XS * 4 + NH * 4 * NW * 8 * 2 * 4];
   e16* A16 = reinterpret_cast<e16*>(smem);
   float* Xa = reinterpret_cast<float*>(smem + 8 * PANEL * 2);
-  float* Xb = Xa + BM * XS;
-  float* gsum = Xb + BM * XS;
+  float* Xb = TWO ? Xa + BM * XS : Xa;
+  float* gsum = Xa + (TWO ? 2 : 1) * BM * XS;
   const int lane = threadIdx.x & 63, wave = __builtin_amdgcn_readfirstlane(threadIdx.x >> 6);
-  const Blk blk = my_rows(d.L);
+  const Blk blk = my_rows<BM>(d.L);
   const int c0 = lane * 4;
   const long rows = (long)d.clips * d.L;
   const rsrc_t rx = make_rsrc(d.x, rows * 1024), rt3 = make_rsrc(d.tgt3, rows * 512), rh1 = make_rsrc(d.h1, rows * 2048);
   const f32x4 bl = ld4(d.b_long + c0), bs = ld4(d.b_short + c0), g3 = ld4(d.ln3_g + c0), b3 = ld4(d.ln3_b + c0);
   f32x4 b1[4];
-#pragma unroll
-  for (int nb = 0; nb < 4; ++nb) b1[nb] = ld4(d.b1 + nb * 256 + c0);
-  const Rows8<f32x4> xo = load_rows_f32(d.x, 256, blk, wave, c0);
+  if (TWO) {
+#pragma unroll
+    for (int nb = 0; nb < 4; ++nb) b1[nb] = ld4(d.b1 + nb * 256 + c0);
+  }
+  Rows8<f32x4> xo[NH];
+#pragma unroll
+  for (int h = 0; h < NH; ++h) xo[h] = load_rows_f32(d.x, 256, blk, h, wave, c0);
   BRing ring;
-  f32x4 acc[2][JT];
+  f32x4 acc[MT][JT];
   const e16* wl = wstream((const e16*)d.w_long, 0, wave, 8);
-  stage_tile<4>(A16, 0, (const e16*)d.att_long + blk.g0 * 256, 256, blk.nrows);
-  stage_tile<4>(A16, 4, (const e16*)d.att_short + blk.g0 * 256, 256, blk.nrows);
+  if (MERGE) stage_merged<BM>(A16, mg, blk.nrows, d.L);
+  else stage_tile<BM, 4>(A16, 0, (const e16*)d.att_long + blk.g0 * 256, 256, blk.nrows);
+  stage_tile<BM, 4>(A16, 4, (const e16*)d.att_short + blk.g0 * 256, 256, blk.nrows);
   b_preload(ring, wl, lane);
   __syncthreads();
   zero_acc(acc);
-  gemm32<4>(A16, 0, wl, ring, acc, lane);
+  gemm_rows<BM, 4>(A16, 0, wl, ring, acc, lane);
   dump_acc(Xa, acc, wave, lane);
   const e16* ws = wstream((const e16*)d.w_short, 0, wave, 8);
   b_preload(ring, ws, lane);
+  if (!TWO) {
+    __syncthreads();
+#pragma unroll
+    for (int h = 0; h < NH; ++h)
+#pragma unroll
+      for (int rr = 0; rr < RW; ++rr) {
+        f32x4 v1 = ld4(&Xa[wrow(h, wave, rr) * XS + c0]);
+        v1 += bl;
+        v1 += xo[h].r[rr];
+        xo[h].r[rr] = v1;
+      }
+  }
   zero_acc(acc);
-  gemm32<4>(A16, 4, ws, ring, acc, lane);
+  gemm_rows<BM, 4>(A16, 4, ws, ring, acc, lane);
+  if (!TWO) __syncthreads();
   dump_acc(Xb, acc, wave, lane);
   const e16* w1 = wstream((const e16*)d.w1, 0, wave, 8);
   b_preload(ring, w1, lane);
   __syncthreads();
-  {
+#pragma unroll
+  for (int h = 0; h < NH; ++h) {
     f32x4 t[RW];
 #pragma unroll
     for (int rr = 0; rr < RW; ++rr) {
-      f32x4 v1 = ld4(&Xa[(wave * RW + rr) * XS + c0]);
-      v1 += bl;
-      t[rr] = ld4(&Xb[(wave * RW + rr) * XS + c0]);
+      f32x4 v1;
+      if (TWO) {
+        v1 = ld4(&Xa[wrow(h, wave, rr) * XS + c0]);
+        v1 += bl;
+      }
+      t[rr] = ld4(&Xb[wrow(h, wave, rr) * XS + c0]);
       t[rr] += bs;
-      v1 += xo.r[rr];
-      st8(rt3, row_off(blk, wave, rr, 256, c0, 2), cvt4(t[rr]));
+      if (TWO) v1 += xo[h].r[rr];
+      else v1 = xo[h].r[rr];
+      st8(rt3, row_off(blk, h, wave, rr, 256, c0, 2), cvt4(t[rr]));
       t[rr] += v1;
-      st16(rx, row_off(blk, wave, rr, 256, c0, 4), t[rr]);
+      st16(rx, row_off(blk, h, wave, rr, 256, c0, 4), t[rr]);
     }
     rmem_ln256_rows<RW>(t, g3, b3, d.eps);
 #pragma unroll
-    for (int rr = 0; rr < RW; ++rr) put_a(A16, 0, wave * RW + rr, lane, cvt4(t[rr]));
+    for (int rr = 0; rr < RW; ++rr) put_a<BM>(A16, 0, wrow(h, wave, rr), lane, cvt4(t[rr]));
   }
   __syncthreads();
 #pragma unroll
   for (int nb = 0; nb < 4; ++nb) {
     float* X = (nb & 1) ? Xb : Xa;
+    if (!TWO) b1[nb] = ld4(d.b1 + nb * 256 + c0);
     zero_acc(acc);
-    gemm32<4>(A16, 0, w1, ring, acc, lane);
+    gemm_rows<BM, 4>(A16, 0, w1, ring, acc, lane);
+    if (!TWO && nb > 0) __syncthreads();
     dump_acc(X, acc, wave, lane);
     if (nb < 3) { w1 = wstream((const e16*)d.w1, nb + 1, wave, 8); b_preload(ring, w1, lane); }
     __syncthreads();
-    float gs = 0.f, gss = 0.f;
-#pragma unroll
-    for (int rr = 0; rr < RW; ++rr) {
-      f32x4 v = ld4(&X[(wave * RW + rr) * XS + c0]);
-      v += b1[nb];
-      const e16x4 h = cvt4(v);
-      st8(rh1, row_off(blk, wave, rr, 1024, nb * 256 + c0, 2), h);
+#pragma unroll
+    for (int h = 0; h < NH; ++h) {
+      float gs = 0.f, gss = 0.f;
+#pragma unroll
+      for (int rr = 0; rr < RW; ++rr) {
+        f32x4 v = ld4(&X[wrow(h, wave, rr) * XS + c0]);
+        v += b1[nb];
+        const e16x4 hh = cvt4(v);
+        st8(rh1, row_off(blk, h, wave, rr, 1024, nb * 256 + c0, 2), hh);
+        if (STATS) {
+          const f32x4 hf = up4(hh);
+          const float okf = wrow(h, wave, rr) < blk.nrows ? 1.f : 0.f;
+          gs += okf * rmem_sum4(hf);
+          gss += okf * rmem_sumsq4(hf);
+        }
+      }
       if (STATS) {
-        const f32x4 hf = up4(h);
-        const float okf = wave * RW + rr < blk.nrows ? 1.f : 0.f;
-        gs += okf * rmem_sum4(hf);
-        gss += okf * rmem_sumsq4(hf);
+        gs += __shfl_xor(gs, 1); gss += __shfl_xor(gss, 1);
+        gs += __shfl_xor(gs, 2); gss += __shfl_xor(gss, 2);
+        gs += __shfl_xor(gs, 4); gss += __shfl_xor(gss, 4);
+        float* go = gsum + (((h * 4 + nb) * NW + wave) * 8 + (lane >> 3)) * 2;
+        if ((lane & 7) == 0) { go[0] = gs; go[1] = gss; }
       }
-    }
-    if (STATS) {
-      gs += __shfl_xor(gs, 1); gss += __shfl_xor(gss, 1);
-      gs += __shfl_xor(gs, 2); gss += __shfl_xor(gss, 2);
-      gs += __shfl_xor(gs, 4); gss += __shfl_xor(gss, 4);
-      if ((lane & 7) == 0) { gsum[((nb * NW + wave) * 8 + (lane >> 3)) * 2] = gs; gsum[((nb * NW + wave) * 8 + (lane >> 3)) * 2 + 1] = gss; }
     }
   }
   if (STATS) {
     __syncthreads();
-    if (threadIdx.x < 32) {
-      const int nb = threadIdx.x >> 3, g = threadIdx.x & 7;
+    const int h = threadIdx.x >> 5, t = threadIdx.x & 31;
+    if (h < NH && h * 32 < blk.nrows) {
+      const int nb = t >> 3, g = t & 7;
+      const float* gi = gsum + ((h * 4 + nb) * NW * 8 + g) * 2;
       float a = 0.f, b = 0.f;
 #pragma unroll
-      for (int w = 0; w < NW; ++w) { a += gsum[((nb * NW + w) * 8 + g) * 2]; b += gsum[((nb * NW + w) * 8 + g) * 2 + 1]; }
-      float* o = d.gn_partial + (((long)blockIdx.y * 32 + threadIdx.x) * d.gn_splits + blockIdx.x) * 2;
+      for (int w = 0; w < NW; ++w) { a += gi[w * 16]; b += gi[w * 16 + 1]; }
+      float* o = d.gn_partial + (((long)blockIdx.y * 32 + t) * d.gn_splits + blockIdx.x * NH + h) * 2;
       o[0] = a; o[1] = b;
     }
   }
 }
 
-template <bool FFN2, bool NEXT>
+template <int BM, bool FFN2, bool NEXT>
 __global__ __launch_bounds__(NT) void k_chain_c(rmem_chain_c_desc d) {
+  constexpr int NH = BM / 32, MT = BM / 16, PANEL = BM * 64;
+  constexpr bool TWO = BM == 32;
   constexpr int NPA = FFN2 ? 16 : 4;
-  static_assert(!FFN2 || 12 * PANEL * 2 >= BM * XS * 4, "the second staging buffer must fit panels 4 .. 15");
-  __shared__ __attribute__((aligned(16))) char smem[NPA * PANEL * 2 + (FFN2 ? 1 : 2) * BM * XS * 4];
+  static_assert(!FFN2 || 12 * PANEL * 2 >= BM * XS * 4, "a staging tile must fit panels 4 .. 15");
+  constexpr int NX = FFN2 ? (TWO ? 1 : 0) : (TWO ? 2 : 1);
+  __shared__ __attribute__((aligned(16))) char smem[NPA * PANEL * 2 + NX * BM * XS * 4];
   e16* A16 = reinterpret_cast<e16*>(smem);
-  float* Xa = reinterpret_cast<float*>(smem + NPA * PANEL * 2);
-  float* Xb = FFN2 ? reinterpret_cast<float*>(smem + 4 * PANEL * 2) : Xa + BM * XS;
+  float* Xp = reinterpret_cast<float*>(smem + 4 * PANEL * 2);
+  float* Xa = NX ? reinterpret_cast<float*>(smem + NPA * PANEL * 2) : Xp;
+  float* Xb = !TWO ? Xa : FFN2 ? Xp : Xa + BM * XS;
   const int lane = threadIdx.x & 63, wave = __builtin_amdgcn_readfirstlane(threadIdx.x >> 6);
-  const Blk blk = my_rows(d.L);
+  const Blk blk = my_rows<BM>(d.L);
   const int c0 = lane * 4;
   const long rows = (long)d.clips * d.L;
   const rsrc_t rx = make_rsrc(d.x, rows * 1024), rdec = make_rsrc(d.dec_out, FFN2 ? ((rows - 1) * d.ld_dec + 256) * 2 : 0),
@@ -326,46 +436,50 @@
 #pragma unroll
     for (int nb = 0; nb < 3; ++nb) bq[nb] = ld4(d.b_qkv + nb * 256 + c0);
   }
-  const Rows8<f32x4> xo = load_rows_f32(d.x, 256, blk, wave, c0);
+  Rows8<f32x4> xo[NH];
+#pragma unroll
+  for (int h = 0; h < NH; ++h) xo[h] = load_rows_f32(d.x, 256, blk, h, wave, c0);
   BRing ring;
-  f32x4 acc[2][JT];
+  f32x4 acc[MT][JT];
   const e16* wq = NEXT ? wstream((const e16*)d.w_qkv, 0, wave, 8) : nullptr;
   if (FFN2) {
     const e16* w2 = wstream((const e16*)d.w2, 0, wave, 32);
-    stage_tile<16>(A16, 0, (const e16*)d.h3 + blk.g0 * 1024, 1024, blk.nrows);
+    stage_tile<BM, 16>(A16, 0, (const e16*)d.h3 + blk.g0 * 1024, 1024, blk.nrows);
     b_preload(ring, w2, lane);
     __syncthreads();
     zero_acc(acc);
-    gemm32<16>(A16, 0, w2, ring, acc, lane);
+    gemm_rows<BM, 16>(A16, 0, w2, ring, acc, lane);
+    if (!TWO) __syncthreads();
     dump_acc(Xa, acc, wave, lane);
     if (NEXT) b_preload(ring, wq, lane);
     __syncthreads();
   } else if (NEXT) {
     b_preload(ring, wq, lane);
   }
-  {
+#pragma unroll
+  for (int h = 0; h < NH; ++h) {
     f32x4 v[RW];
     if (FFN2) {
       f32x4 vd[RW];
 #pragma unroll
       for (int rr = 0; rr < RW; ++rr) {
-        v[rr] = ld4(&Xa[(wave * RW + rr) * XS + c0]);
+        v[rr] = ld4(&Xa[wrow(h, wave, rr) * XS + c0]);
         v[rr] += b2;
-        v[rr] += xo.r[rr];
-        st16(rx, row_off(blk, wave, rr, 256, c0, 4), v[rr]);
+        v[rr] += xo[h].r[rr];
+        st16(rx, row_off(blk, h, wave, rr, 256, c0, 4), v[rr]);
         vd[rr] = v[rr];
       }
       rmem_ln256_rows<RW>(vd, gd, bd, d.eps);
 #pragma unroll
-      for (int rr = 0; rr < RW; ++rr) st8(rdec, row_off(blk, wave, rr, d.ld_dec, c0, 2), cvt4(vd[rr]));
+      for (int rr = 0; rr < RW; ++rr) st8(rdec, row_off(blk, h, wave, rr, d.ld_dec, c0, 2), cvt4(vd[rr]));
     } else {
 #pragma unroll
-      for (int rr = 0; rr < RW; ++rr) v[rr] = xo.r[rr];
+      for (int rr = 0; rr < RW; ++rr) v[rr] = xo[h].r[rr];
     }
     if (NEXT) {
       rmem_ln256_rows<RW>(v, g1, b1, d.eps);
 #pragma unroll
-      for (int rr = 0; rr < RW; ++rr) put_a(A16, 0, wave * RW + rr, lane, cvt4(v[rr]));
+      for (int rr = 0; rr < RW; ++rr) put_a<BM>(A16, 0, wrow(h, wave, rr), lane, cvt4(v[rr]));
     }
   }
   if (!NEXT) return;
@@ -373,28 +487,49 @@
 #pragma unroll
   for (int nb = 0; nb < 3; ++nb) {
     float* X = (nb & 1) ? Xb : Xa;
-    const Rows8<f32x4> pos = load_rows_f32(d.pos_qk + nb * 256, 768, blk, wave, c0);
+    Rows8<f32x4> pos[NH];
+#pragma unroll
+    for (int h = 0; h < NH; ++h) pos[h] = load_rows_f32(d.pos_qk + nb * 256, 768, blk, h, wave, c0);
     zero_acc(acc);
-    gemm32<4>(A16, 0, wq, ring, acc, lane);
+    gemm_rows<BM, 4>(A16, 0, wq, ring, acc, lane);
+    if (!TWO && nb > 0) __syncthreads();
     dump_acc(X, acc, wave, lane);
     if (nb < 2) { wq = wstream((const e16*)d.w_qkv, nb + 1, wave, 8); b_preload(ring, wq, lane); }
     __syncthreads();
 #pragma unroll
-    for (int rr = 0; rr < RW; ++rr) {
-      f32x4 v = ld4(&X[(wave * RW + rr) * XS + c0]);
-      v += bq[nb];
-      v += pos.r[rr];
-      st8(rqkv, row_off(blk, wave, rr, 768, nb * 256 + c0, 2), cvt4(v));
-    }
+    for (int h = 0; h < NH; ++h)
+#pragma unroll
+      for (int rr = 0; rr < RW; ++rr) {
+        f32x4 v = ld4(&X[wrow(h, wave, rr) * XS + c0]);
+        v += bq[nb];
+        v += pos[h].r[rr];
+        st8(rqkv, row_off(blk, h, wave, rr, 768, nb * 256 + c0, 2), cvt4(v));
+      }
   }
 }
 
 #ifndef RMEM_F16
 }
 extern "C" int rmem_lstt_chain_waves(void) { return NW; }
+extern "C" int rmem_lstt_chain_rows(int L, int clips, int cus) { return (long)((L + 31) / 32) * clips > cus ? 64 : 32; }
 namespace {
 #endif
 bool al16(const void* p) { return p == nullptr || ((uintptr_t)p % 16) == 0; }
+
+int chain_rows(int L, int clips) {
+  if (const char* e = getenv("RMEM_CHAIN_ROWS")) {
+    const int x = atoi(e);
+    return x == 32 || x == 64 ? x : 0;
+  }
+  static int cus = 0;
+  if (cus <= 0) {
+    int dev = 0, n = 0;
+    if (hipGetDevice(&dev) != hipSuccess || hipDeviceGetAttribute(&n, hipDeviceAttributeMultiprocessorCount, dev) != hipSuccess || n <= 0)
+      return 32;
+    cus = n;
+  }
+  return rmem_lstt_chain_rows(L, clips, cus);
+}
 
 }
 
@@ -405,21 +540,52 @@
   RMEM_REQUIRE(al16(d->att) && al16(d->x) && al16(d->w_proj) && al16(d->w_q) && al16(d->curr_v) && al16(d->curr_q) && al16(d->short_k) &&
                al16(d->short_v) && al16(d->k4) && al16(d->v4) && al16(d->b_proj) && al16(d->b_q) && al16(d->ln2_g) && al16(d->ln2_b) &&
                al16(d->ln4_g) && al16(d->ln4_b), "rmem_lstt_chain_a: operands must be 16-byte aligned");
-  hipLaunchKernelGGL(k_chain_a, dim3((d->L + BM - 1) / BM, d->clips), dim3(NT), 0, (hipStream_t)stream, *d);
+  const int bm = chain_rows(d->L, d->clips);
+  RMEM_REQUIRE(bm, "rmem_lstt_chain_a: RMEM_CHAIN_ROWS must be 32 or 64");
+  const dim3 grid((d->L + bm - 1) / bm, d->clips);
+  if (bm == 64) hipLaunchKernelGGL(k_chain_a<64>, grid, dim3(NT), 0, (hipStream_t)stream, *d);
+  else hipLaunchKernelGGL(k_chain_a<32>, grid, dim3(NT), 0, (hipStream_t)stream, *d);
   return rmem_check_launch("rmem_lstt_chain_a");
 }
 
-extern "C" int RMEM_API(rmem_lstt_chain_b)(const rmem_chain_b_desc* d, void* stream) {
+namespace {
+template <int BM>
+void launch_chain_b(const rmem_chain_b_desc* d, const rmem_attn_merge* mg, hipStream_t s) {
+  const dim3 grid((d->L + BM - 1) / BM, d->clips);
+  const rmem_attn_merge none = {};
+  if (mg) {
+    if (d->gn_partial) hipLaunchKernelGGL((k_chain_b<BM, true, true>), grid, dim3(NT), 0, s, *d, *mg);
+    else hipLaunchKernelGGL((k_chain_b<BM, false, true>), grid, dim3(NT), 0, s, *d, *mg);
+  } else {
+    if (d->gn_partial) hipLaunchKernelGGL((k_chain_b<BM, true, false>), grid, dim3(NT), 0, s, *d, none);
+    else hipLaunchKernelGGL((k_chain_b<BM, false, false>), grid, dim3(NT), 0, s, *d, none);
+  }
+}
+
+int chain_b(const rmem_chain_b_desc* d, const rmem_attn_merge* mg, void* stream) {
   RMEM_REQUIRE(d && d->L > 0 && d->clips >= 1 && (long)d->L * d->clips < (1L << 20), "rmem_lstt_chain_b: bad geometry (rows must stay below 2^20)");
   RMEM_REQUIRE(d->att_long && d->att_short && d->x && d->w_long && d->b_long && d->w_short && d->b_short && d->tgt3 && d->ln3_g && d->ln3_b &&
                d->w1 && d->b1 && d->h1, "rmem_lstt_chain_b: null argument");
   RMEM_REQUIRE(al16(d->att_long) && al16(d->att_short) && al16(d->x) && al16(d->w_long) && al16(d->w_short) && al16(d->tgt3) && al16(d->w1) &&
                al16(d->h1) && al16(d->b_long) && al16(d->b_short) && al16(d->b1) && al16(d->ln3_g) && al16(d->ln3_b),
                "rmem_lstt_chain_b: operands must be 16-byte aligned");
-  RMEM_REQUIRE(!d->gn_partial || d->gn_splits >= (d->L + BM - 1) / BM, "rmem_lstt_chain_b: gn_splits must cover the row blocks of a clip");
-  if (d->gn_partial) hipLaunchKernelGGL(k_chain_b<true>, dim3((d->L + BM - 1) / BM, d->clips), dim3(NT), 0, (hipStream_t)stream, *d);
-  else hipLaunchKernelGGL(k_chain_b<false>, dim3((d->L + BM - 1) / BM, d->clips), dim3(NT), 0, (hipStream_t)stream, *d);
+  RMEM_REQUIRE(!d->gn_partial || d->gn_splits >= (d->L + 31) / 32, "rmem_lstt_chain_b: gn_splits must cover the 32-row blocks of a clip");
+  RMEM_REQUIRE(!mg || (mg->heads == 8 && mg->Lq == d->L && mg->ngroups <= 32 && mg->opart && mg->mlg && ((uintptr_t)mg->opart % 8) == 0 &&
+                       ((uintptr_t)mg->mlg % 8) == 0 && mg->opart_cs % 2 == 0 && mg->mlg_cs % 2 == 0),
+               "rmem_lstt_chain_b_merged: the merge needs 8 heads, Lq = L, <= 32 groups and 8-byte aligned partials");
+  const int bm = chain_rows(d->L, d->clips);
+  RMEM_REQUIRE(bm, "rmem_lstt_chain_b: RMEM_CHAIN_ROWS must be 32 or 64");
+  if (bm == 64) launch_chain_b<64>(d, mg, (hipStream_t)stream);
+  else launch_chain_b<32>(d, mg, (hipStream_t)stream);
   return rmem_check_launch("rmem_lstt_chain_b");
+}
+}
+
+extern "C" int RMEM_API(rmem_lstt_chain_b)(const rmem_chain_b_desc* d, void* stream) { return chain_b(d, nullptr, stream); }
+
+extern "C" int RMEM_API(rmem_lstt_chain_b_merged)(const rmem_chain_b_desc* d, const rmem_attn_merge* merge, void* stream) {
+  RMEM_REQUIRE(merge, "rmem_lstt_chain_b_merged: null merge");
+  return chain_b(d, merge->ngroups > 1 ? merge : nullptr, stream);
 }
 
 extern "C" int RMEM_API(rmem_lstt_chain_c)(const rmem_chain_c_desc* d, void* stream) {
@@ -431,10 +597,18 @@
   RMEM_REQUIRE(!next || (d->ln1_g && d->ln1_b && d->b_qkv && d->pos_qk && d->qkv), "rmem_lstt_chain_c: the QKV stage needs ln1, b_qkv, pos_qk, qkv");
   RMEM_REQUIRE(al16(d->x) && al16(d->h3) && al16(d->w2) && al16(d->b2) && al16(d->dec_g) && al16(d->dec_b) && al16(d->dec_out) && al16(d->ln1_g) &&
                al16(d->ln1_b) && al16(d->w_qkv) && al16(d->b_qkv) && al16(d->pos_qk) && al16(d->qkv), "rmem_lstt_chain_c: operands must be 16-byte aligned");
-  const dim3 grid((d->L + BM - 1) / BM, d->clips);
+  const int bm = chain_rows(d->L, d->clips);
+  RMEM_REQUIRE(bm, "rmem_lstt_chain_c: RMEM_CHAIN_ROWS must be 32 or 64");
+  const dim3 grid((d->L + bm - 1) / bm, d->clips);
   hipStream_t s = (hipStream_t)stream;
-  if (ffn2 && next) hipLaunchKernelGGL((k_chain_c<true, true>), grid, dim3(NT), 0, s, *d);
-  else if (ffn2) hipLaunchKernelGGL((k_chain_c<true, false>), grid, dim3(NT), 0, s, *d);
-  else hipLaunchKernelGGL((k_chain_c<false, true>), grid, dim3(NT), 0, s, *d);
+  if (bm == 64) {
+    if (ffn2 && next) hipLaunchKernelGGL((k_chain_c<64, true, true>), grid, dim3(NT), 0, s, *d);
+    else if (ffn2) hipLaunchKernelGGL((k_chain_c<64, true, false>), grid, dim3(NT), 0, s, *d);
+    else hipLaunchKernelGGL((k_chain_c<64, false, true>), grid, dim3(NT), 0, s, *d);
+  } else {
+    if (ffn2 && next) hipLaunchKernelGGL((k_chain_c<32, true, true>), grid, dim3(NT), 0, s, *d);
+    else if (ffn2) hipLaunchKernelGGL((k_chain_c<32, true, false>), grid, dim3(NT), 0, s, *d);
+    else hipLaunchKernelGGL((k_chain_c<32, false, true>), grid, dim3(NT), 0, s, *d);
+  }
   return rmem_check_launch("rmem_lstt_chain_c");
 }
diff --git a/rmem_ocu_amd/group_runtime.py b/rmem_ocu_amd/group_runtime.py
--- a/rmem_ocu_amd/group_runtime.py
+++ b/rmem_ocu_amd/group_runtime.py
@@ -25,6 +25,7 @@
         self.swin = 'pe.w' in P
         self.chain = not os.environ.get('RMEM_NO_CHAIN')
         self.pair_attn = not os.environ.get('RMEM_NO_PAIR_ATTN')
+        self.merge_fold = not os.environ.get('RMEM_NO_MERGE_FOLD')
         self.P, self.dev, self.NL, self.B = P, device, num_lstt, clips
         self.dt = P['proj.w'].dtype
         self.align, self.nc = align_corners, num_classes
@@ -282,11 +283,12 @@
                                       ln2=ln(d + '.ln2'), curr_v=self.curr_V[i], w_q=P[d + '.linear_Q.wf'], b_q=P[d + '.linear_Q.b'], curr_q=cq,
                                       short_k=self.short_K[i], short_v=self.short_V[i], ln4=ln(d + '.ln4'), k4=self.k4, v4=self.v4))
             mass = self.mass if (i == 0 and want_mass) else None
+            mg = ops.attn_merge() if (self.pair_attn and self.merge_fold) else None
             if self.pair_attn:
                 o.append(ops.lstt_attn_pair(cq, self.bank_K[i], self.bank_V[i], self.att, self.k4, self.v4, self.att2, self.attn_ws, Lq=L,
                                             heads=HEADS, ldq=C, ldkv=C, ldo=C, slot_stride=L * C, chunks=self.chunks, nchunks=nchunks,
                                             lk_total=T * L, pe_cur=P['pe_cur'], pe_mem=P['pe_mem'], mass=mass, T=T, nclips=B, q_cs=L * C,
-                                            out_cs=L * C, lk_short=L, kv_short_cs=L * C, out_short_cs=L * C))
+                                            out_cs=L * C, lk_short=L, kv_short_cs=L * C, out_short_cs=L * C, merge=mg))
             else:
                 o.append(self._attn(cq, C, self.bank_K[i], self.bank_V[i], C, self.att, slot_stride=L * C, chunks=self.chunks,
                                     nchunks=nchunks, lk_single=T * L, pe_cur=P['pe_cur'], pe_mem=P['pe_mem'], mass=mass, T=T))
@@ -294,7 +296,8 @@
             o.append(ops.lstt_chain_b(L=L, clips=B, att_long=self.att, att_short=self.att2, x=self.x, w_long=P[d + '.long_proj.wf'],
                                       b_long=P[d + '.long_proj.b'], w_short=P[d + '.short_proj.wf'], b_short=P[d + '.short_proj.b'],
                                       tgt3=self.tgt3[i], ln3=ln(d + '.ln3'), w1=P[d + '.linear1.wf'], b1=P[d + '.linear1.b'], h1=self.h1,
-                                      gn_partial=self.ffn_stats if self.chain_stats else None, gn_splits=64 if self.chain_stats else 0))
+                                      gn_partial=self.ffn_stats if self.chain_stats else None, gn_splits=64 if self.chain_stats else 0,
+                                      merge=mg))
             if self.chain_stats:
                 o.append(ops.gn_act_dwconv5x5_prestats(self.h1, P[d + '.gn.g'], P[d + '.gn.b'], P[d + '.dw.w'], self.h3, self.ffn_stats,
                                                        H=self.H16, W=self.W16, C=FFN, groups=32, act=2, images=B))
diff --git a/rmem_ocu_amd/ops.py b/rmem_ocu_amd/ops.py
--- a/rmem_ocu_amd/ops.py
+++ b/rmem_ocu_amd/ops.py
@@ -165,14 +165,22 @@
     return Op(_fn('rmem_layernorm256_pair', dt), args, 'rmem_layernorm256_pair', (a0, b0, y0, a1, b1, y1, gamma, beta))
 
 
-def _chain(name, cls, ints, ptrs, dt):
+def lstt_chain_rows(L: int, clips: int, cus: int) -> int:
+    return int(_lib.lib().rmem_lstt_chain_rows(int(L), int(clips), int(cus)))
+
+
+def attn_merge():
+    return _lib.AttnMerge()
+
+
+def _chain(name, cls, ints, ptrs, dt, extra=()):
     ts = list(ptrs.values())
     _dev(*ts)
     for k, t in ptrs.items():
         if t is not None and t.data_ptr() % 16:
             raise RmemError(f'{name}: {k} must be 16-byte aligned')
     d = cls(int(ints[0]), int(ints[1]), float(ints[2]), int(ints[3]), *[_ptr(t) for t in ts])
-    return Op(_fn(name, dt), (C.byref(d),), name, (d, ts))
+    return Op(_fn(name, dt), (C.byref(d), *[C.byref(e) for e in extra]), name, (d, ts, extra))
 
 
 def lstt_chain_a(*, L, clips, att, x, w_proj, b_proj, ln2, curr_v, w_q, b_q, curr_q, short_k, short_v, ln4, k4, v4, eps=1e-5) -> Op:
@@ -186,15 +194,15 @@
 
 
 def lstt_chain_b(*, L, clips, att_long, att_short, x, w_long, b_long, w_short, b_short, tgt3, ln3, w1, b1, h1, gn_partial=None,
-                 gn_splits=0, eps=1e-5) -> Op:
+                 gn_splits=0, eps=1e-5, merge=None) -> Op:
     dt = att_long.dtype
     R = clips * L
     assert x.dtype == F32 and all(t.dtype == dt and t.numel() >= R * 256 for t in (att_long, att_short, tgt3)) and h1.dtype == dt and h1.numel() >= R * 1024
     assert w_long.numel() == 65536 and w_short.numel() == 65536 and w1.numel() == 262144 and b1.numel() == 1024
     assert gn_partial is None or (gn_partial.dtype == F32 and gn_splits * 32 >= L and gn_partial.numel() >= clips * 32 * gn_splits * 2)
-    return _chain('rmem_lstt_chain_b', _lib.ChainB, (L, clips, eps, gn_splits),
+    return _chain('rmem_lstt_chain_b' if merge is None else 'rmem_lstt_chain_b_merged', _lib.ChainB, (L, clips, eps, gn_splits),
                   dict(att_long=att_long, att_short=att_short, x=x, w_long=w_long, b_long=b_long, w_short=w_short, b_short=b_short, tgt3=tgt3,
-                       ln3_g=ln3[0], ln3_b=ln3[1], w1=w1, b1=b1, h1=h1, gn_partial=gn_partial), dt)
+                       ln3_g=ln3[0], ln3_b=ln3[1], w1=w1, b1=b1, h1=h1, gn_partial=gn_partial), dt, () if merge is None else (merge,))
 
 
 def lstt_chain_c(*, L, clips, x, dt, h3=None, w2=None, b2=None, dec_norm=(None, None), dec_out=None, ld_dec=0, ln1=(None, None), w_qkv=None,
@@ -235,7 +243,8 @@
 
 
 def lstt_attn_pair(q, k_bank, v_bank, out_long, k_short, v_short, out_short, workspace, *, Lq, heads=8, ldq, ldkv, ldo, slot_stride, chunks,
-                   nchunks, lk_total, pe_cur, pe_mem, mass=None, T=0, nclips=1, q_cs=0, out_cs=0, lk_short, kv_short_cs=0, out_short_cs=0) -> Op:
+                   nchunks, lk_total, pe_cur, pe_mem, mass=None, T=0, nclips=1, q_cs=0, out_cs=0, lk_short, kv_short_cs=0, out_short_cs=0,
+                   merge=None) -> Op:
     _dev(q, k_bank, v_bank, out_long, k_short, v_short, out_short, workspace, chunks, pe_cur, pe_mem, mass)
     dt = q.dtype
     assert all(t.dtype == dt for t in (k_bank, v_bank, out_long, k_short, v_short, out_short))
@@ -246,8 +255,10 @@
     args = (_ptr(q), ldq, _ptr(k_bank), _ptr(v_bank), slot_stride, ldkv, _ptr(chunks), nchunks, lk_total, _ptr(pe_cur), _ptr(pe_mem), Lq, heads,
             _ptr(out_long), ldo, _ptr(mass), T, nclips, q_cs, out_cs, _ptr(k_short), _ptr(v_short), lk_short, kv_short_cs, _ptr(out_short),
             out_short_cs, _ptr(workspace))
-    return Op(_fn('rmem_lstt_attn_pair_clips', dt), args, 'rmem_lstt_attn_pair',
-              (q, k_bank, v_bank, out_long, k_short, v_short, out_short, workspace, chunks, pe_cur, pe_mem, mass))
+    if merge is not None:
+        args += (C.byref(merge),)
+    return Op(_fn('rmem_lstt_attn_pair_clips' if merge is None else 'rmem_lstt_attn_pair_clips_deferred', dt), args, 'rmem_lstt_attn_pair',
+              (q, k_bank, v_bank, out_long, k_short, v_short, out_short, workspace, chunks, pe_cur, pe_mem, mass, merge))
 
 
 def layernorm256(a, gamma, beta, *, M, lda=256, b=None, ldb=256, y=None, ldy=256, pos=None, ypos=None, ldyp=256,
```
